# thecasterian/fluca

Measured on AMD Instinct MI355X. Metric: pressure-Poisson Jacobi-PCG iterations/s, 512^3 cells per GPU, higher is better.
Workload: dtype f64

## Files before the change

### fluca_amd/build.py

```python
import hashlib
import json
import os
import subprocess
import sys

HERE = os.path.dirname(os.path.abspath(__file__))
CSRC = os.path.join(HERE, "csrc")
LIBDIR = os.path.join(HERE, "lib")
LIB = os.path.join(LIBDIR, "libflucahip.so")
SOURCES = ["fl_coeff.cpp", "fl_kernels.hip", "fl_api.hip", "fl_knobs.cpp", "fl_place.hip", "fl_halo.hip", "fl_comm.hip", "fl_ksp.hip", "fl_cheb2.hip", "fl_layout.hip", "fl_ibm.hip", "fl_ibm_owner.hip", "fl_ibm_body.hip", "fl_momentum.hip", "fl_mg.hip", "fl_schur_var.hip", "fl_scalar.hip", "fl_buoyancy.hip", "fl_scalar_implicit.hip"]
HEADERS = ["fl_internal.h", "fl_knobs.h", "fl_handle.h", "fl_msg.h", "fl_ibm_device.h", "fl_ibm_handle.h", "fl_ibm_plan.h", "fl_device.h", "fl_stencil.h", "fl_mom_tile.h", "fl_mom_tile3.h", "fl_limiter.h", "fl_scalar_handle.h", os.path.join("..", "..", "include", "fluca_hip.h"),
           os.path.join("..", "..", "include", "fluca_hip_implicit.h"), os.path.join("..", "..", "include", "fluca_hip_implicit_ranks.h"), os.path.join("..", "..", "include", "fluca_hip_ibm_scalar.h")]
HIPCC = os.environ.get("HIPCC", "/opt/rocm/bin/hipcc")
FLAGS = ["--offload-arch=gfx950", "-O3", "-std=c++17", "-fPIC", "-Wall", "-Wno-unused-function", "-Wno-unused-result"]
MANIFEST = os.path.join(LIBDIR, "manifest.json")


def _sha(path):
    h = hashlib.sha256()
    with open(path, "rb") as fh:
        h.update(fh.read())
    return h.hexdigest()


def _load_manifest(path=None):
    try:
        with open(path or MANIFEST) as fh:
            return json.load(fh)
    except (OSError, ValueError):
        return {}


def _fingerprint(deps, cmd_words):
    h = hashlib.sha256()
    for d in deps:
        h.update(os.path.basename(d).encode() + b"\0" + (_sha(d) if os.path.exists(d) else "absent").encode() + b"\0")
    root = os.path.normpath(os.path.join(HERE, ".."))
    real = os.path.realpath(root)
    h.update(" ".join(w.replace(real, "$ROOT").replace(root, "$ROOT") for w in cmd_words).encode())
    return h.hexdigest()


def _stale(target, deps, cmd_words=(), manifest=None):
    if not os.path.exists(target):
        return True
    m = _load_manifest() if manifest is None else manifest
    return m.get(os.path.relpath(target, LIBDIR)) != _fingerprint(deps, cmd_words)


def _record(target, deps, cmd_words=()):
    m = _load_manifest()
    m[os.path.relpath(target, LIBDIR)] = _fingerprint(deps, cmd_words)
    with open(MANIFEST, "w") as fh:
        json.dump(m, fh, indent=0, sort_keys=True)


def _mapped(path):
    try:
        real = os.path.realpath(path)
        with open("/proc/self/maps") as fh:
            return any(line.rstrip().endswith(real) or line.rstrip().endswith(path) for line in fh)
    except OSError:
        return False


def _link(cmd, target):
    if _mapped(target):
        raise RuntimeError(f"{target} is out of date with respect to the sources AND loaded in this process: rebuild it first "
                           "(`python -m fluca_amd.build`, or tests/conftest.py, which builds before anything is loaded); it is not replaced under a live process")
    tmp = target + ".tmp%d" % os.getpid()
    i = cmd.index("-o")
    assert cmd[i + 1] == target
    subprocess.check_call(cmd[:i + 1] + [tmp] + cmd[i + 2:])
    os.replace(tmp, target)


def source_id():
    files = [os.path.join(CSRC, s) for s in SOURCES] + [os.path.normpath(os.path.join(CSRC, h)) for h in HEADERS]
    return _fingerprint(files, FLAGS)[:12]


def build(force=False, verbose=False):
    os.makedirs(LIBDIR, exist_ok=True)
    srcs = [os.path.join(CSRC, s) for s in SOURCES if os.path.exists(os.path.join(CSRC, s))]
    hdrs = [os.path.normpath(os.path.join(CSRC, h)) for h in HEADERS]
    objs = []
    for s in srcs:
        o = os.path.join(LIBDIR, os.path.basename(s) + ".o")
        cmd = [HIPCC] + FLAGS + (["-x", "hip"] if s.endswith(".hip") else []) + ["-c", s, "-o", o]
        if force or _stale(o, [s] + hdrs, cmd):
            if verbose:
                print(" ".join(cmd), flush=True)
            subprocess.check_call(cmd)
            _record(o, [s] + hdrs, cmd)
        objs.append(o)
    sid = source_id()
    idsrc, idobj = os.path.join(LIBDIR, "fl_build_id.cpp"), os.path.join(LIBDIR, "fl_build_id.cpp.o")
    text = f'extern "C" const char *fl_build_id(void) {{ return "{sid}"; }}\n'
    if not os.path.exists(idsrc) or open(idsrc).read() != text:
        with open(idsrc, "w") as fh:
            fh.write(text)
    cmd = [os.environ.get("CXX", "g++"), "-O1", "-fPIC", "-c", idsrc, "-o", idobj]
    if force or _stale(idobj, [idsrc], cmd):
        subprocess.check_call(cmd)
        _record(idobj, [idsrc], cmd)
    objs.append(idobj)
    cmd = [HIPCC, "--offload-arch=gfx950", "-shared", "-fPIC", "-o", LIB] + objs + ["-Wl,-rpath,/opt/rocm/lib", "-ldl"]
    if force or _stale(LIB, objs, cmd):
        if verbose:
            print(" ".join(cmd), flush=True)
        _link(cmd, LIB)
        _record(LIB, objs, cmd)
    build_host(force, verbose)
    return LIB


HOST_LIB = os.path.join(LIBDIR, "libfluca_host.so")


def build_host(force=False, verbose=False):
    src = os.path.join(HERE, "host", "fluca_host.c")
    hdrs = [os.path.normpath(os.path.join(HERE, "..", "include", h)) for h in ("fluca_host.h", "fluca_host_impl.h", "fluca_hip.h", "fluca_hip_implicit.h", "fluca_hip_implicit_ranks.h", "fluca_hip_ibm_scalar.h")]
    cmd = [os.environ.get("CC", "gcc"), "-std=gnu99", "-O2", "-fPIC", "-shared", "-Wall", "-o", HOST_LIB, src,
           "-L" + LIBDIR, "-lflucahip", "-Wl,-rpath,$ORIGIN", "-lm", "-ldl", "-pthread"]
    if force or _stale(HOST_LIB, [src, LIB] + hdrs, cmd):
        if verbose:
            print(" ".join(cmd), flush=True)
        _link(cmd, HOST_LIB)
        _record(HOST_LIB, [src, LIB] + hdrs, cmd)
    build_cgns(force, verbose)
    build_example(force, verbose)
    build_example(force, verbose, name="cavity_flow_3d")
    build_example(force, verbose, name="flow_configs")
    build_example(force, verbose, name="heated_cavity_3d")
    build_example(force, verbose, name="heated_sphere_3d")
    return HOST_LIB


CGNS_LIB = os.path.join(LIBDIR, "libfluca_cgns.so")
HDF5_ROOT = os.environ.get("HDF5_ROOT", "/opt/conda")


def have_hdf5():
    return os.path.exists(os.path.join(HDF5_ROOT, "include", "hdf5.h")) and os.path.exists(os.path.join(HDF5_ROOT, "lib", "libhdf5.so"))


def build_cgns(force=False, verbose=False):
    src = os.path.join(HERE, "host", "fluca_cgns.c")
    if not have_hdf5():
        if verbose:
            print(f"no HDF5 under {HDF5_ROOT}: libfluca_cgns.so not built", flush=True)
        return None
    hdrs = [os.path.normpath(os.path.join(HERE, "..", "include", h)) for h in ("fluca_cgns.h", "fluca_host.h", "fluca_host_impl.h", "fluca_hip.h", "fluca_hip_implicit.h", "fluca_hip_implicit_ranks.h", "fluca_hip_ibm_scalar.h")]
    if True:
        cmd = [os.environ.get("CC", "gcc"), "-std=gnu99", "-O2", "-fPIC", "-shared", "-Wall", "-o", CGNS_LIB, src,
               "-I" + os.path.join(HDF5_ROOT, "include"), "-L" + LIBDIR, "-lfluca_host", "-lflucahip",
               "-L" + os.path.join(HDF5_ROOT, "lib"), "-lhdf5", "-Wl,--enable-new-dtags",
               "-Wl,-rpath,$ORIGIN", "-Wl,-rpath," + os.path.join(HDF5_ROOT, "lib"), "-lm"]
        if force or _stale(CGNS_LIB, [src, HOST_LIB] + hdrs, cmd):
            if verbose:
                print(" ".join(cmd), flush=True)
            _link(cmd, CGNS_LIB)
            _record(CGNS_LIB, [src, HOST_LIB] + hdrs, cmd)
    return CGNS_LIB


EXAMPLE = os.path.join(LIBDIR, "cavity_pressure_step")


def build_example(force=False, verbose=False, name="cavity_pressure_step"):
    root = os.path.normpath(os.path.join(HERE, ".."))
    src = os.path.join(root, "examples", name + ".c")
    EXAMPLE = os.path.join(LIBDIR, name)
    cgns = os.path.exists(CGNS_LIB) and name == "cavity_flow_3d"
    cmd = [os.environ.get("CC", "gcc"), "-std=gnu99", "-O2", "-Wall", "-o", EXAMPLE, src, "-I" + os.path.join(root, "include"),
           "-L" + LIBDIR] + (["-DFLUCA_HAVE_CGNS", "-lfluca_cgns"] if cgns else []) + ["-lfluca_host", "-lflucahip", "-lm",
           "-Wl,-rpath,$ORIGIN", "-Wl,-rpath,/opt/rocm/lib"]
    deps = [src, HOST_LIB, LIB] + ([CGNS_LIB] if cgns else []) + [os.path.join(root, "include", h) for h in ("fluca_host.h", "fluca_hip.h", "fluca_hip_implicit.h", "fluca_hip_implicit_ranks.h", "fluca_hip_ibm_scalar.h", "fluca_cgns.h")]
    if os.path.exists(src) and (force or _stale(EXAMPLE, deps, cmd)):
        if verbose:
            print(" ".join(cmd), flush=True)
        _link(cmd, EXAMPLE)
        _record(EXAMPLE, deps, cmd)
    return EXAMPLE


if __name__ == "__main__":
    print(build(force="--force" in sys.argv, verbose=True))
```

### fluca_amd/capi.py

```python
import ctypes as C
import os

import torch

_HERE = os.path.dirname(os.path.abspath(__file__))
LIB_PATH = os.path.join(os.environ.get("FLUCA_LIB_DIR") or os.path.join(_HERE, "lib"), "libflucahip.so")

if not os.path.exists(LIB_PATH):
    raise ImportError(
        f"{LIB_PATH} is missing: build it with `python -m fluca_amd.build` (hipcc --offload-arch=gfx950). "
        "There is no CPU fallback for the product path.")

lib = C.CDLL(LIB_PATH)

BC_NONE, BC_VELOCITY, BC_PRESSURE_OUTLET, BC_PERIODIC, BC_SYMMETRY = range(5)
KSP_CG, KSP_BCGS, KSP_CHEBYSHEV, KSP_GMRES = range(4)
PC_NONE, PC_JACOBI = range(2)
NORM_PRECONDITIONED, NORM_UNPRECONDITIONED, NORM_NATURAL, NORM_NONE = range(4)
DELTA_PESKIN4, DELTA_ROMA3 = range(2)
SCALAR_DIRICHLET, SCALAR_NEUMANN, SCALAR_PERIODIC = range(3)
LIMITERS = ("superbee", "minmod", "mc", "vanleer", "vanalbada", "barthjesperson", "venkatakrishnan", "koren", "upwind", "sou", "quick")
UNIQUE_ID_BYTES = 128

ERRORS = {0: "FL_SUCCESS", -55: "FL_ERR_MEM", -56: "FL_ERR_SUP", -60: "FL_ERR_ARG_SIZ", -62: "FL_ERR_ARG_WRONG",
          -63: "FL_ERR_ARG_OUTOFRANGE", -73: "FL_ERR_ARG_WRONGSTATE", -76: "FL_ERR_LIB", -85: "FL_ERR_ARG_NULL",
          -91: "FL_ERR_NOT_CONVERGED", -97: "FL_ERR_GPU"}


class FlucaError(RuntimeError):
    def __init__(self, rc, what):
        super().__init__(f"{what} -> {ERRORS.get(rc, rc)} ({rc})")
        self.rc = rc


def check(rc, what="libflucahip"):
    if rc != 0:
        raise FlucaError(rc, what)


class fl_comm_info(C.Structure):
    _fields_ = [("transport", C.c_int), ("rank", C.c_int), ("nranks", C.c_int), ("loopback", C.c_int), ("neighbours", C.c_int), ("messages", C.c_int), ("halo_bytes", C.c_int64)]


class fl_grid(C.Structure):
    _fields_ = [("n", C.c_int64 * 3), ("xf", C.c_void_p * 3), ("xc", C.c_void_p * 3)]


class fl_decomp(C.Structure):
    _fields_ = [("ranks", C.c_int * 3), ("coord", C.c_int * 3), ("lo", C.c_int64 * 3), ("len", C.c_int64 * 3)]


class fl_ksp_opts(C.Structure):
    _fields_ = [("type", C.c_int), ("pc", C.c_int), ("norm_type", C.c_int), ("remove_nullspace", C.c_int),
                ("maxit", C.c_int), ("rtol", C.c_double), ("atol", C.c_double), ("dtol", C.c_double),
                ("emin", C.c_double), ("emax", C.c_double), ("variant", C.c_int), ("check_every", C.c_int),
                ("profile", C.c_int), ("history", C.POINTER(C.c_double)), ("nhistory", C.c_int),
                ("mg_levels", C.c_int), ("mg_smooth_its", C.c_int), ("gmres_restart", C.c_int), ("cg_single_reduction", C.c_int),
                ("initial_guess_nonzero", C.c_int)]


class fl_ksp_stats(C.Structure):
    _fields_ = [("iters", C.c_int), ("reason", C.c_int), ("rnorm0", C.c_double), ("rnorm", C.c_double),
                ("seconds", C.c_double), ("kernel_ms", C.c_double), ("kernel_launches", C.c_int),
                ("kernel2_ms", C.c_double), ("kernel2_launches", C.c_int)]


class fl_dmstag_local(C.Structure):
    _fields_ = [("gstart", C.c_int64 * 3), ("gsize", C.c_int64 * 3), ("start", C.c_int64 * 3), ("entries", C.c_int)]


class fl_scalar_cheb_info(C.Structure):
    _fields_ = [("steps", C.c_int), ("capped", C.c_int), ("emin", C.c_double), ("emax", C.c_double), ("bound", C.c_double)]


class fl_halo_msg(C.Structure):
    _fields_ = [("peer", C.c_int), ("send_boundary", C.c_int), ("recv_boundary", C.c_int), ("sendtag", C.c_int), ("recvtag", C.c_int)]


EXCHANGE_FN = C.CFUNCTYPE(C.c_int, C.c_void_p, C.c_int, C.POINTER(C.c_int), C.POINTER(C.c_int), C.POINTER(C.c_int),
                          C.POINTER(C.c_void_p), C.POINTER(C.c_void_p), C.POINTER(C.c_int64))
ALLREDUCE_FN = C.CFUNCTYPE(C.c_int, C.c_void_p, C.POINTER(C.c_double), C.c_int)

_P = C.c_void_p
PROTOTYPES = {
    "fl_poisson_create": (C.c_int, [C.POINTER(fl_grid), C.POINTER(C.c_int), C.c_double, C.POINTER(fl_decomp), C.c_int, C.POINTER(_P)]),
    "fl_poisson_destroy": (C.c_int, [_P]),
    "fl_poisson_set_stream": (C.c_int, [_P, _P]),
    "fl_poisson_synchronize": (C.c_int, [_P]),
    "fl_poisson_barrier": (C.c_int, [_P]),
    "fl_poisson_sizes": (C.c_int, [_P, C.POINTER(C.c_int64)]),
    "fl_poisson_allreduce_sum": (C.c_int, [_P, C.POINTER(C.c_double), C.c_int]),
    "fl_ksp_opts_default": (None, [C.POINTER(fl_ksp_opts)]),
    "fl_version": (C.c_char_p, []),
    "fl_abi_version": (C.c_int, []),
    "fl_poisson_comm_info": (C.c_int, [_P, C.POINTER(fl_comm_info)]),
    "fl_current_device": (C.c_int, [C.POINTER(C.c_int)]),
    "fl_malloc": (C.c_int, [C.c_int, C.c_size_t, C.POINTER(_P)]),
    "fl_free": (C.c_int, [C.c_int, _P]),
    "fl_memcpy_h2d": (C.c_int, [C.c_int, _P, _P, C.c_size_t]),
    "fl_memcpy_d2h": (C.c_int, [C.c_int, _P, _P, C.c_size_t]),
    "fl_malloc_host": (C.c_int, [C.c_size_t, C.POINTER(C.c_void_p)]),
    "fl_free_host": (C.c_int, [_P]),
    "fl_poisson_upload": (C.c_int, [_P, _P, _P, C.c_size_t]),
    "fl_poisson_upload_fence": (C.c_int, [_P]),
    "fl_tuning_set": (C.c_int, [C.c_char_p, C.c_int]),
    "fl_tuning_get": (C.c_int, [C.c_char_p, C.POINTER(C.c_int)]),
    "fl_poisson_tune_placement": (C.c_int, [_P, C.c_int, C.POINTER(C.c_double)]),
    "fl_poisson_vector_bytes": (C.c_int, [_P, C.POINTER(C.c_int64)]),
    "fl_poisson_apply": (C.c_int, [_P, _P, _P]),
    "fl_poisson_diagonal": (C.c_int, [_P, _P]),
    "fl_poisson_solve": (C.c_int, [_P, _P, _P, C.POINTER(fl_ksp_opts), C.POINTER(fl_ksp_stats)]),
    "fl_poisson_rhs": (C.c_int, [_P, _P, _P, _P, _P, _P]),
    "fl_poisson_project": (C.c_int, [_P, _P, _P, _P, _P, _P, _P, _P]),
    "fl_poisson_gst_bc": (C.c_int, [_P, C.c_int, _P, _P]),
    "fl_pressure_update": (C.c_int, [_P, C.c_int, _P, _P, _P, _P]),
    "fl_layout_from_dmstag_local": (C.c_int, [_P, C.POINTER(fl_dmstag_local), C.c_int, C.c_int, _P, _P]),
    "fl_layout_to_dmstag_local": (C.c_int, [_P, C.POINTER(fl_dmstag_local), C.c_int, C.c_int, _P, _P]),
    "fl_layout_from_dmstag_global": (C.c_int, [_P, C.POINTER(C.c_int), C.c_int, C.c_int, _P, _P]),
    "fl_layout_to_dmstag_global": (C.c_int, [_P, C.POINTER(C.c_int), C.c_int, C.c_int, _P, _P]),
    "fl_dmstag_global_entries": (C.c_int, [_P, C.POINTER(C.c_int), C.POINTER(C.c_int64)]),
    "fl_comm_unique_id": (C.c_int, [_P]),
    "fl_poisson_comm_init_rccl": (C.c_int, [_P, _P, C.c_int, C.c_int]),
    "fl_poisson_comm_init_host": (C.c_int, [_P, EXCHANGE_FN, ALLREDUCE_FN, _P, C.c_int, C.c_int]),
    "fl_poisson_comm_oneshot_handle": (C.c_int, [_P, _P, C.POINTER(_P)]),
    "fl_poisson_comm_oneshot_attach": (C.c_int, [_P, _P, C.POINTER(_P)]),
    "fl_poisson_comm_oneshot_error": (C.c_int, [_P, C.POINTER(C.c_int)]),
    "fl_halo_plan": (C.c_int, [C.POINTER(fl_decomp), C.POINTER(C.c_int), C.POINTER(fl_halo_msg)]),
    "fl_decomp_default": (C.c_int, [C.POINTER(C.c_int64), C.POINTER(C.c_int), C.c_int, C.POINTER(fl_decomp)]),
    "fl_decomp_neighbor": (C.c_int, [C.POINTER(fl_decomp), C.POINTER(C.c_int), C.c_int]),
    "fl_decomp_neighbor_offset": (C.c_int, [C.POINTER(fl_decomp), C.POINTER(C.c_int), C.POINTER(C.c_int)]),
    "fl_momentum_create": (C.c_int, [_P, C.POINTER(_P)]),
    "fl_momentum_destroy": (C.c_int, [_P]),
    "fl_momentum_set_state": (C.c_int, [_P, C.c_double, C.c_double, C.c_double, _P, _P]),
    "fl_momentum_set_state_v0": (C.c_int, [_P, C.c_double, C.c_double, C.c_double, _P, _P, _P]),
    "fl_momentum_set_coefficients": (C.c_int, [_P, C.c_double, C.c_double, C.c_double]),
    "fl_momentum_apply": (C.c_int, [_P, _P, _P]),
    "fl_momentum_diagonal": (C.c_int, [_P, _P]),
    "fl_momentum_rowsum": (C.c_int, [_P, _P]),
    "fl_momentum_gershgorin": (C.c_int, [_P, C.POINTER(C.c_double)]),
    "fl_momentum_chebyshev_interval": (C.c_int, [_P, C.POINTER(C.c_double), C.POINTER(C.c_double)]),
    "fl_abf_set_ainv_types": (C.c_int, [_P, C.c_int, C.c_int]),
    "fl_abf_schur_apply": (C.c_int, [_P, _P, _P]),
    "fl_momentum_solve": (C.c_int, [_P, _P, _P, C.POINTER(fl_ksp_opts), C.POINTER(fl_ksp_stats)]),
    "fl_momentum_face_interp": (C.c_int, [_P, _P, _P, _P]),
    "fl_poisson_gershgorin": (C.c_int, [_P, C.c_int, C.POINTER(C.c_double)]),
    "fl_vec_lincomb": (C.c_int, [_P, C.c_int64, C.c_double, _P, C.c_double, _P, _P]),
    "fl_vec_dot": (C.c_int, [_P, C.c_int64, _P, _P, C.POINTER(C.c_double)]),
    "fl_vec_mdot": (C.c_int, [_P, C.c_int64, _P, C.POINTER(C.c_void_p), C.c_int, C.POINTER(C.c_double)]),
    "fl_vec_maxpy": (C.c_int, [_P, C.c_int64, _P, C.POINTER(C.c_double), C.POINTER(C.c_void_p), C.c_int]),
    "fl_boundary_set_faces": (C.c_int, [_P, C.c_int, C.c_double, _P, _P]),
    "fl_boundary_add_faces": (C.c_int, [_P, C.c_int, C.c_double, _P, _P]),
    "fl_momentum_face_interp_scaled": (C.c_int, [_P, C.c_double, _P, _P, _P]),
    "fl_boundary_add_cells": (C.c_int, [_P, C.c_int, C.c_double, _P, _P]),
    "fl_momentum_rhs": (C.c_int, [_P, C.c_double, C.c_double, C.c_double, _P, _P, _P, _P]),
    "fl_momentum_add_buoyancy": (C.c_int, [_P, C.c_int, C.POINTER(C.c_void_p), C.POINTER(C.c_double), C.POINTER(C.c_double), C.c_double, _P]),
    "fl_momentum_interp_faces": (C.c_int, [_P, _P, _P, _P]),
    "fl_momentum_interp_faces_ends": (C.c_int, [_P, _P, _P, _P]),
    "fl_abf_jacobian_mult": (C.c_int, [_P, _P, _P, _P, _P, _P, _P]),
    "fl_abf_apply": (C.c_int, [_P, C.POINTER(fl_ksp_opts), C.POINTER(fl_ksp_opts), _P, _P, _P, _P, _P, _P, C.POINTER(fl_ksp_stats)]),
    "fl_ibm_create": (C.c_int, [_P, C.c_int, C.c_int64, _P, _P, _P, C.POINTER(_P)]),
    "fl_ibm_update": (C.c_int, [_P, _P, _P, _P]),
    "fl_ibm_interp": (C.c_int, [_P, C.c_int, _P, _P]),
    "fl_ibm_spread": (C.c_int, [_P, C.c_int, _P, _P, _P]),
    "fl_ibm_destroy": (C.c_int, [_P]),
    "fl_ibm_owned_select": (C.c_int, [_P, C.c_int, C.c_int64, _P, _P, _P, _P, C.POINTER(C.c_int64)]),
    "fl_ibm_create_owned": (C.c_int, [_P, C.c_int, C.c_int64, _P, _P, _P, _P, C.POINTER(_P)]),
    "fl_ibm_owned_counts": (C.c_int, [_P, C.POINTER(C.c_int64)]),
    "fl_ibm_migrate": (C.c_int, [_P, _P, _P, _P, C.c_int, _P, C.POINTER(C.c_int64), C.POINTER(C.c_int64)]),
    "fl_ibm_owned_fetch": (C.c_int, [_P, C.c_int64, _P, _P, _P, _P, C.c_int, _P]),
    "fl_ibm_rigid_pose": (C.c_int, [_P, C.c_int64, _P, _P, _P] + [C.POINTER(C.c_double)] * 5 + [_P, _P, _P, _P]),
    "fl_ibm_force": (C.c_int, [_P, _P, _P, _P, C.c_int, C.POINTER(C.c_double), C.POINTER(C.c_double), C.POINTER(C.c_double)]),
    "fl_limiter_from_name": (C.c_int, [C.c_char_p, C.POINTER(C.c_int)]),
    "fl_limiter_eval": (C.c_int, [C.c_int, C.c_double, C.POINTER(C.c_double)]),
    "fl_scalar_create": (C.c_int, [_P, C.POINTER(C.c_int), C.POINTER(_P)]),
    "fl_scalar_create_ranks": (C.c_int, [_P, C.POINTER(C.c_int), C.POINTER(_P)]),
    "fl_scalar_destroy": (C.c_int, [_P]),
    "fl_scalar_set_boundary_value": (C.c_int, [_P, C.c_int, C.c_double]),
    "fl_scalar_set_limiter": (C.c_int, [_P, C.c_int]),
    "fl_scalar_set_diffusivity": (C.c_int, [_P, C.c_double]),
    "fl_scalar_set_velocity": (C.c_int, [_P, _P, _P, _P]),
    "fl_scalar_rhs": (C.c_int, [_P, _P, _P, _P]),
    "fl_scalar_step": (C.c_int, [_P, C.c_double, C.c_int, _P, _P]),
    "fl_scalar_cfl": (C.c_int, [_P, C.c_double, C.POINTER(C.c_double)]),
    "fl_scalar_stats": (C.c_int, [_P, _P, C.POINTER(C.c_double)]),
    "fl_scalar_boundary_flux": (C.c_int, [_P, _P, C.POINTER(C.c_double)]),
}
PROTOTYPES_IMPLICIT = {
    "fl_scalar_cheb_steps": (C.c_int, [C.c_double, C.c_double, C.c_double, C.c_int, C.POINTER(C.c_int), C.POINTER(C.c_double)]),
    "fl_scalar_diffusion_interval": (C.c_int, [_P, C.c_double, C.POINTER(C.c_double), C.POINTER(C.c_double)]),
    "fl_scalar_diffusion_apply": (C.c_int, [_P, C.c_double, _P, _P]),
    "fl_scalar_diffusion_solve": (C.c_int, [_P, C.c_double, C.c_double, C.c_int, _P, _P, C.POINTER(fl_scalar_cheb_info)]),
    "fl_scalar_step_imex": (C.c_int, [_P, C.c_double, C.c_int, C.c_double, C.c_double, C.c_int, _P, _P, C.POINTER(fl_scalar_cheb_info)]),
}
PROTOTYPES_IBM_SCALAR = {
    "fl_ibm_scalar_force": (C.c_int, [_P, C.c_int, _P, _P, C.c_int, C.POINTER(C.c_double), _P, _P, _P]),
    "fl_ibm_scalar_rate": (C.c_int, [_P, _P, _P, _P, C.c_int, C.POINTER(C.c_double)]),
}
PROTOTYPES_IMPLICIT_RANKS = {
    "fl_scalar_diffusion_apply_ranks": PROTOTYPES_IMPLICIT["fl_scalar_diffusion_apply"],
    "fl_scalar_diffusion_solve_ranks": PROTOTYPES_IMPLICIT["fl_scalar_diffusion_solve"],
    "fl_scalar_step_imex_ranks": PROTOTYPES_IMPLICIT["fl_scalar_step_imex"],
}
for _name, (_res, _args) in list(PROTOTYPES.items()) + list(PROTOTYPES_IMPLICIT.items()) + list(PROTOTYPES_IBM_SCALAR.items()) + list(PROTOTYPES_IMPLICIT_RANKS.items()):
    _f = getattr(lib, _name)
    _f.restype = _res
    _f.argtypes = _args
```

### fluca_amd/csrc/fl_momentum.hip

```cpp
#include <new>

#include "fl_handle.h"
#include "fl_device.h"

namespace fl {

struct MomP {
  const double *tab[3];
  const double *stab[3];
  const double *bw[3];
  int           len[3];
  double        cI, cC, cL;
};

struct FaceT {
  const double *w0[3][3], *w1[3][3];
  const int    *c0[3][3];
};

__device__ __forceinline__ double recip(double d)
{
  double r = __builtin_amdgcn_rcp(d);
  r        = fma(r, fma(-d, r, 1.), r);
  r        = fma(r, fma(-d, r, 1.), r);
  return r;
}

}
#include "fl_stencil.h"
#include "fl_mom_tile.h"
#include "fl_mom_tile3.h"
namespace fl {

template <int OP>
__global__ void __launch_bounds__(512) k_mom_pw3(GridP g, int64_t cs, const double *__restrict__ a0, const double *__restrict__ a1, const double *__restrict__ a2, const double *__restrict__ a3, double *__restrict__ w0,
                                                 double *__restrict__ w1, const KspScal *__restrict__ s, double *__restrict__ partial, int pstride, int pairs, int tiles_x, int nchunk, int zc)
{
  __shared__ double red[3 * 8];
  if (OP != 3 && s->reason != 0) return;
  const double alpha = s->alpha, omega = s->omega, beta = s->beta, ob = s->omega_old * s->beta;
  const int    nb = gridDim.x, tiles = nb / nchunk, b = xcd_remap(blockIdx.x, nb), chunk = b / tiles, tile = b % tiles;
  const int    lane = threadIdx.x & 63, w = threadIdx.x >> 6;
  const int    i = (tile % tiles_x) * 128 + 2 * lane, j = (tile / tiles_x) * 8 + w;
  const int    k0 = chunk * zc, k1 = min(k0 + zc, g.nz);
  const int64_t ncell = (int64_t)g.nx * g.ny * g.nz;
  double       acc[3] = {0., 0., 0.};
  if (i < g.nx && j < g.ny) {
    const bool two = i + 1 < g.nx;
    auto       ldp = [&](const double *p, int64_t q) { return two ? ld2<1>(p + q) : make_double2(p[q], 0.); };
    auto       ldk = [&](const double *p, int64_t q) { return two ? ld2<0>(p + q) : make_double2(p[q], 0.); };
    auto       stp = [&](double *p, int64_t q, double2 v) {
      if (two) st2<0>(p + q, v);
      else p[q] = v.x;
    };
    for (int k = k0; k < k1; ++k) {
      const int64_t idx = g.off0 + (int64_t)k * g.sxy + (int64_t)j * g.sx + i, ub = ((int64_t)k * g.ny + j) * g.nx + i;
#pragma unroll
      for (int c = 0; c < 3; ++c) {
        const int64_t q = c * cs + idx;
        if (OP == 0) {
          const double2 r = ldk(a0, q), v = ldp(a1, q), p = ldp(w0, q);
          stp(w0, q, make_double2(r.x - ob * v.x + beta * p.x, r.y - ob * v.y + beta * p.y));
        } else if (OP == 4) {
          stp(w0, q, ldk(a0, q));
        } else if (OP == 1) {
          const double2 r = ldp(a0, q), v = ldp(a1, q);
          stp(w0, q, make_double2(r.x - alpha * v.x, r.y - alpha * v.y));
        } else if (OP == 6) {
          const double2 xk = ldp(a0, q), ax = ldp(a1, q), bb = ldp(a2, q), xo = ldp(w0, q);
          const double2 rr = make_double2(bb.x - ax.x, bb.y - ax.y);
          double2       zz = rr;
          if (a3) {
            const double2 d = ldk(a3, q);
            zz.x = rr.x * recip(d.x);
            zz.y = two ? rr.y * recip(d.y) : 0.;
          }
          stp(w0, q, make_double2(fma(s->cheb_c, zz.x, fma(s->cheb_rho, xk.x - xo.x, xk.x)), fma(s->cheb_c, zz.y, fma(s->cheb_rho, xk.y - xo.y, xk.y))));
          acc[0] += zz.x + (two ? zz.y : 0.);
          acc[1] += zz.x * zz.x + (two ? zz.y * zz.y : 0.);
          acc[2] += rr.x * rr.x + (two ? rr.y * rr.y : 0.);
        } else if (OP == 2 || OP == 5) {
          const double2 P = ldp(a0, q), S = ldp(a1, q), T = ldp(a2, q), RP = ldk(a3, q), X = OP == 5 ? make_double2(0., 0.) : ldp(w0, q);
          const double2 rn = make_double2(S.x - omega * T.x, S.y - omega * T.y);
          double2       xn = X;
          xn.x += alpha * P.x + omega * S.x;
          xn.y += alpha * P.y + omega * S.y;
          if (two) st2<1>(w0 + q, xn);
          else w0[q] = xn.x;
          stp(w1, q, rn);
          acc[0] += rn.x * rn.x + (two ? rn.y * rn.y : 0.);
          acc[1] += rn.x * RP.x + (two ? rn.y * RP.y : 0.);
          acc[2] += rn.x + (two ? rn.y : 0.);
        } else {
          const int64_t u = c * ncell + ub;
          double2       bb;
          if (two && pairs) bb = ld2<1>(a0 + u);
          else bb = make_double2(a0[u], two ? a0[u + 1] : 0.);
          double2 r = bb;
          if (a1) {
            const double2 d = ldp(a1, q);
            r.x = bb.x / d.x;
            if (two) r.y = bb.y / d.y;
          }
          stp(w0, q, r);
          stp(w1, q, r);
          acc[0] += r.x + (two ? r.y : 0.);
          acc[1] += r.x * r.x + (two ? r.y * r.y : 0.);
        }
      }
    }
  }
  if (OP == 2 || OP == 3 || OP == 5 || OP == 6) {
#pragma unroll
    for (int a = 0; a < 3; ++a) {
      const double v = wave_sum(acc[a]);
      if (lane == 0) red[a * 8 + w] = v;
    }
    __syncthreads();
    if (threadIdx.x < 3) {
      double v = 0.;
#pragma unroll
      for (int q = 0; q < 8; ++q) v += red[threadIdx.x * 8 + q];
      partial[(int64_t)threadIdx.x * pstride + blockIdx.x] = v;
    }
  }
}

__global__ void __launch_bounds__(256) k_fill(int64_t n, double v, double *__restrict__ out)
{
  for (int64_t q = (int64_t)blockIdx.x * blockDim.x + threadIdx.x; q < n; q += (int64_t)gridDim.x * blockDim.x) out[q] = v;
}
__global__ void __launch_bounds__(256) k_recip(int64_t n, const double *__restrict__ in, double *__restrict__ out)
{
  for (int64_t q = (int64_t)blockIdx.x * blockDim.x + threadIdx.x; q < n; q += (int64_t)gridDim.x * blockDim.x) out[q] = 1. / in[q];
}
__global__ void __launch_bounds__(256) k_scale_by(int64_t n, const double *__restrict__ w, double shift, const double *x, double *y, int add)
{
  for (int64_t q = (int64_t)blockIdx.x * blockDim.x + threadIdx.x; q < n; q += (int64_t)gridDim.x * blockDim.x) {
    const double t = (w[q] - shift) * x[q];
    y[q]           = add ? y[q] + t : t;
  }
}
__global__ void __launch_bounds__(256) k_max_sum_owned(GridP g, int64_t cs, const double *__restrict__ a, const double *__restrict__ b, double *__restrict__ partial)
{
  __shared__ double red[2][4];
  const int64_t plane = (int64_t)g.nz * g.ny, rows = 3 * plane;
  double        mx = 0., sm = 0.;
  for (int64_t r0 = (int64_t)blockIdx.x * 4; r0 < rows; r0 += (int64_t)gridDim.x * 4) {
    int64_t base[4];
#pragma unroll
    for (int u = 0; u < 4; ++u) {
      const int64_t r = min(r0 + u, rows - 1);
      const int     c = (int)(r / plane), kj = (int)(r % plane), k = kj / g.ny, j = kj % g.ny;
      base[u] = (int64_t)c * cs + g.off0 + (int64_t)k * g.sxy + (int64_t)j * g.sx;
    }
    for (int i = 2 * threadIdx.x; i < g.nx; i += 512) {
      const bool two = i + 1 < g.nx;
      double2    va[4], vb[4];
#pragma unroll
      for (int u = 0; u < 4; ++u) {
        va[u] = a ? (two ? *reinterpret_cast<const double2 *>(a + base[u] + i) : make_double2(a[base[u] + i], 0.)) : make_double2(0., 0.);
        vb[u] = b ? (two ? *reinterpret_cast<const double2 *>(b + base[u] + i) : make_double2(b[base[u] + i], 0.)) : make_double2(0., 0.);
      }
#pragma unroll
      for (int u = 0; u < 4; ++u) {
        mx = fmax(mx, fmax(va[u].x, va[u].y));
        if (r0 + u < rows) sm += vb[u].x + vb[u].y;
      }
    }
  }
  for (int off = 32; off > 0; off >>= 1) {
    mx = fmax(mx, __shfl_down(mx, off, 64));
    sm += __shfl_down(sm, off, 64);
  }
  if ((threadIdx.x & 63) == 0) {
    red[0][threadIdx.x >> 6] = mx;
    red[1][threadIdx.x >> 6] = sm;
  }
  __syncthreads();
  if (threadIdx.x == 0) {
    partial[2 * blockIdx.x]     = fmax(fmax(red[0][0], red[0][1]), fmax(red[0][2], red[0][3]));
    partial[2 * blockIdx.x + 1] = (red[1][0] + red[1][1]) + (red[1][2] + red[1][3]);
  }
}

struct Vec8 {
  const double *p[8];
};
struct Coef8 {
  double a[8];
};
__global__ void __launch_bounds__(256) k_mdot8(int64_t n, const double *__restrict__ x, Vec8 Y, int k, double *__restrict__ partial, int stride)
{
  __shared__ double red[8 * 4];
  double            acc[8] = {0., 0., 0., 0., 0., 0., 0., 0.};
  for (int64_t q = (int64_t)blockIdx.x * blockDim.x + threadIdx.x; q < n; q += (int64_t)gridDim.x * blockDim.x) {
    const double xv = x[q];
#pragma unroll
    for (int i = 0; i < 8; ++i)
      if (i < k) acc[i] += xv * Y.p[i][q];
  }
  block_sum<8>(acc, red);
  if (threadIdx.x == 0)
#pragma unroll
    for (int i = 0; i < 8; ++i) partial[(int64_t)i * stride + blockIdx.x] = acc[i];
}
__global__ void __launch_bounds__(256) k_maxpy8(int64_t n, double *__restrict__ x, Coef8 A, Vec8 Y, int k)
{
  for (int64_t q = (int64_t)blockIdx.x * blockDim.x + threadIdx.x; q < n; q += (int64_t)gridDim.x * blockDim.x) {
    double t = x[q];
#pragma unroll
    for (int i = 0; i < 8; ++i)
      if (i < k) t += A.a[i] * Y.p[i][q];
    x[q] = t;
  }
}
__global__ void __launch_bounds__(256) k_lincomb(int64_t n, double a, const double *x, double b, const double *z, double *y)
{
  const bool ux = a != 0., uz = z && b != 0.;
  for (int64_t q = (int64_t)blockIdx.x * blockDim.x + threadIdx.x; q < n; q += (int64_t)gridDim.x * blockDim.x) y[q] = (ux ? a * x[q] : 0.) + (uz ? b * z[q] : 0.);
}

__global__ void __launch_bounds__(256) k_dot(int64_t n, const double *__restrict__ x, const double *__restrict__ y, double *__restrict__ partial)
{
  __shared__ double red[4];
  double            v[1] = {0.};
  for (int64_t q = (int64_t)blockIdx.x * blockDim.x + threadIdx.x; q < n; q += (int64_t)gridDim.x * blockDim.x) v[0] += x[q] * y[q];
  block_sum<1>(v, red);
  if (threadIdx.x == 0) partial[blockIdx.x] = v[0];
}

__global__ void __launch_bounds__(256) k_pad_copy_ext(GridP g, const double *__restrict__ src, double *__restrict__ dst, int ex, int ey, int ez)
{
  const int64_t n = (int64_t)ex * ey * ez;
  for (int64_t q = (int64_t)blockIdx.x * blockDim.x + threadIdx.x; q < n; q += (int64_t)gridDim.x * blockDim.x) {
    const int     i = (int)(q % ex);
    const int64_t r = q / ex;
    const int     j = (int)(r % ey), k = (int)(r / ey);
    dst[g.off0 + (int64_t)k * g.sxy + (int64_t)j * g.sx + i] = src[q];
  }
}

__global__ void __launch_bounds__(256) k_pad_copy_ends(GridP g, const double *__restrict__ src, double *__restrict__ dst, int ex, int ey, int ez, int d)
{
  const int     nd = d == 0 ? g.nx : (d == 1 ? g.ny : g.nz), ed = d == 0 ? ex : (d == 1 ? ey : ez);
  const int     na = d == 0 ? ey : ex, nb = d == 2 ? ey : ez;
  const int     nend = ed > nd ? 2 : 1;
  const int64_t n = (int64_t)na * nb * nend;
  for (int64_t q = (int64_t)blockIdx.x * blockDim.x + threadIdx.x; q < n; q += (int64_t)gridDim.x * blockDim.x) {
    const int a = (int)(q % na), b = (int)((q / na) % nb), f = (q / ((int64_t)na * nb)) ? nd : 0;
    const int i = d == 0 ? f : a, j = d == 1 ? f : (d == 0 ? a : b), k = d == 2 ? f : b;
    dst[g.off0 + (int64_t)k * g.sxy + (int64_t)j * g.sx + i] = src[((int64_t)k * ey + j) * ex + i];
  }
}

__global__ void __launch_bounds__(256) k_face_interp(GridP g, FaceT t, int kind, int d, double alpha, const double *__restrict__ vpad, const double *rhs, double *V)
{
  const int     ex = d == 0 ? g.fx : g.nx, ey = d == 1 ? g.fy : g.ny, ez = d == 2 ? g.fz : g.nz;
  const int64_t str = d == 0 ? 1 : (d == 1 ? (int64_t)g.sx : g.sxy);
  const int     lane = threadIdx.x & 63, w = __builtin_amdgcn_readfirstlane(threadIdx.x >> 6), nw = blockDim.x >> 6;
  const int     nseg = (ex + 63) / 64;
  const int64_t nitem = (int64_t)nseg * ey * ez;
  for (int64_t it = (int64_t)blockIdx.x * nw + w; it < nitem; it += (int64_t)gridDim.x * nw) {
    const int seg = (int)(it % nseg), row = (int)(it / nseg);
    const int j = row % ey, k = row / ey, i = seg * 64 + lane;
    if (i >= ex) continue;
    const int     f = d == 0 ? i : (d == 1 ? j : k);
    const int     c0 = t.c0[kind][d][f];
    const int64_t q = ((int64_t)k * ey + j) * ex + i;
    const int64_t base = g.off0 + (int64_t)k * g.sxy + (int64_t)j * g.sx + i + (int64_t)(c0 - f) * str;
    const double  w0 = alpha * t.w0[kind][d][f], w1 = alpha * t.w1[kind][d][f];
    double        s = rhs ? rhs[q] : 0.;
    if (w0 != 0.) s += w0 * vpad[base];
    if (w1 != 0.) s += w1 * vpad[base + str];
    V[q] = s;
  }
}

__global__ void __launch_bounds__(256) k_face_interp_ends(GridP g, FaceT t, int kind, int d, const double *__restrict__ vpad, const double *rhs, double *V)
{
  const int     ex = d == 0 ? g.fx : g.nx, ey = d == 1 ? g.fy : g.ny, ez = d == 2 ? g.fz : g.nz;
  const int     nd = d == 0 ? g.nx : (d == 1 ? g.ny : g.nz), ed = d == 0 ? ex : (d == 1 ? ey : ez);
  const int     na = d == 0 ? ey : ex, nb = d == 2 ? ey : ez;
  const int64_t n = (int64_t)na * nb * (ed > nd ? 2 : 1);
  const int64_t str = d == 0 ? 1 : (d == 1 ? (int64_t)g.sx : g.sxy);
  for (int64_t q = (int64_t)blockIdx.x * blockDim.x + threadIdx.x; q < n; q += (int64_t)gridDim.x * blockDim.x) {
    const int     a = (int)(q % na), b = (int)((q / na) % nb), f = (q / ((int64_t)na * nb)) ? nd : 0;
    const int     i = d == 0 ? f : a, j = d == 1 ? f : (d == 0 ? a : b), k = d == 2 ? f : b;
    const int64_t u = ((int64_t)k * ey + j) * ex + i;
    const int     c0 = t.c0[kind][d][f];
    const int64_t base = g.off0 + (int64_t)k * g.sxy + (int64_t)j * g.sx + i + (int64_t)(c0 - f) * str;
    const double  w0 = t.w0[kind][d][f], w1 = t.w1[kind][d][f];
    double        s = rhs ? rhs[u] : 0.;
    if (w0 != 0.) s += w0 * vpad[base];
    if (w1 != 0.) s += w1 * vpad[base + str];
    V[u] = s;
  }
}

}

using namespace fl;


struct fl_momentum {
  fl_poisson *p = nullptr;
  MomP        mp;
  FaceT       ft;
  void       *tabs[3] = {nullptr, nullptr, nullptr};
  double     *bws[3] = {nullptr, nullptr, nullptr};
  double     *stabs[2][3] = {{nullptr, nullptr, nullptr}, {nullptr, nullptr, nullptr}};
  std::vector<void *> ttabs;
  double     *srhs = nullptr;
  double     *gr = nullptr, *gd = nullptr;
  double     *tmpv = nullptr;
  double     *F = nullptr;
  double     *dg = nullptr;
  double     *v0p = nullptr;
  bool        fly = false;
  double     *vec[8] = {nullptr, nullptr, nullptr, nullptr, nullptr, nullptr, nullptr, nullptr};
  int                   schur_ainv = FL_ABF_AINV_ID, upper_ainv = FL_ABF_AINV_ID;
  double               *ainv[2] = {nullptr, nullptr}, *zV[3] = {nullptr, nullptr, nullptr}, *gv = nullptr;
  std::vector<double *> gm;
  std::vector<double *> kb;
  bool        have_state = false;
  double      dmean = 1.;
  double      gersh = -1.;
  int         t2x = 1, t2chunk = 1, t2zc = 1, t2blocks = 1;
};

namespace {

int mom_vec(fl_momentum *m, int slot)
{
  if (m->vec[slot]) return 0;
  return fl_dev_alloc(m->p, (void **)&m->vec[slot], sizeof(double) * 3 * m->p->padlen, true);
}

int mom_ghosts(fl_momentum *m, double *v3)
{
  fl_poisson *h = m->p;
  if (!fl_any_ghost_exchange(h)) return 0;
  if (!h->multi) {
    for (int d = 0; d < 3; ++d)
      if (h->wrap_local[d]) launch_wrap(h->stream, h->g, v3, d, 3, (int64_t)h->padlen);
    return 0;
  }
  for (int c = 0; c < 3; ++c) FL_CHK(fl_fill_ghosts(h, v3 + (size_t)c * h->padlen));
  return 0;
}

constexpr int MOM_XCD_ORDER = 1;

bool mom3_grid(const GridP &g) { return g.ny > 8; }

template <int DOT, bool JAC, int OUT>
void mom_apply_t(fl_momentum *m, const double *x, double *y, const double *o, const KspScal *s, const MomP *coeffs = nullptr)
{
  fl_poisson *h = m->p;
  int         flags = MOM_XCD_ORDER;
  if (OUT == 1 && (h->g.nx & 1) == 0 && (reinterpret_cast<uintptr_t>(y) & 15) == 0) flags |= 2;
  if (m->fly && mom3_grid(h->g))
    hipLaunchKernelGGL((k_mom3<8, DOT, JAC, OUT, 1>), dim3(m->t2blocks), dim3(512), 0, h->stream, h->g, coeffs ? *coeffs : m->mp, x, y, m->F, (const double *)m->v0p, (int64_t)h->padlen, o, s, h->partial,
                       h->partial_stride, m->t2x, m->t2chunk, m->t2zc, flags);
  else
    hipLaunchKernelGGL((k_mom2<8, DOT, JAC, OUT, 1>), dim3(m->t2blocks), dim3(512), 0, h->stream, h->g, coeffs ? *coeffs : m->mp, x, y, m->F, (int64_t)h->padlen, o, s, h->partial, h->partial_stride, m->t2x, m->t2chunk,
                       m->t2zc, flags);
}
int mom_scale_tables(fl_momentum *m, int slot, MomP &p)
{
  fl_poisson *h = m->p;
  for (int d = 0; d < 3; ++d) {
    const int len = m->mp.len[d], n = len * MOM_STAB;
    hipLaunchKernelGGL(k_mom_scale_tab, dim3((n + 255) / 256), dim3(256), 0, h->stream, (const double *)m->tabs[d], len, p.cC, p.cL, m->stabs[slot][d]);
    p.stab[d] = m->stabs[slot][d];
  }
  FL_HIP(hipGetLastError());
  return 0;
}

template <int OP>
void mom_pw(fl_momentum *m, const double *a0, const double *a1, const double *a2, const double *a3, double *w0, double *w1)
{
  fl_poisson *h = m->p;
  const int   pairs = (h->g.nx & 1) == 0 && (reinterpret_cast<uintptr_t>(a0) & 15) == 0;
  hipLaunchKernelGGL((k_mom_pw3<OP>), dim3(m->t2blocks), dim3(512), 0, h->stream, h->g, (int64_t)h->padlen, a0, a1, a2, a3, w0, w1, h->scal, h->partial, h->partial_stride, pairs, m->t2x, m->t2chunk, m->t2zc);
}

}

MomPlan fl::mom_plan(const GridP &g)
{
  MomPlan p;
  p.t2x           = (g.nx + 127) / 128;
  const int tiles = p.t2x * ((g.ny + 7) / 8);
  int       nc    = z_chunk_count(tiles, g.nz, 1024);
  if (tiles * nc > MAX_PARTIAL_BLOCKS) nc = std::max(1, MAX_PARTIAL_BLOCKS / tiles);
  const ZChunks z = z_chunks(g.nz, nc);
  p.t2zc     = z.zc;
  p.t2chunk  = z.nchunk;
  p.t2blocks = tiles * p.t2chunk;
  return p;
}

namespace {

int mom_init(fl_momentum *m, fl_poisson *h)
{
  m->p = h;
  const GridP &g = h->g;
  if (g.nx < 2 || g.ny < 2 || g.nz < 2) return FL_ERR_SUP;
  const int64_t lo[3] = {h->dec.lo[0], h->dec.lo[1], h->dec.lo[2]};
  const int     len[3] = {g.nx, g.ny, g.nz};
  for (int d = 0; d < 3; ++d) {
    std::vector<double> tab, loc;
    FL_CHK(build_axis_momentum(h->ax[d], tab));
    const int64_t n = h->ax[d].n;
    loc.resize((size_t)MOM_NTAB * len[d]);
    for (int a = 0; a < MOM_NTAB; ++a)
      for (int i = 0; i < len[d]; ++i) loc[(size_t)a * len[d] + i] = tab[(size_t)a * n + (size_t)(lo[d] + i)];
    FL_HIP(hipMalloc(&m->tabs[d], sizeof(double) * loc.size()));
    FL_HIP(hipMemcpy(m->tabs[d], loc.data(), sizeof(double) * loc.size(), hipMemcpyHostToDevice));
    m->mp.tab[d] = (const double *)m->tabs[d];
    m->mp.len[d] = len[d];
    for (int slot = 0; slot < 2; ++slot) FL_HIP(hipMalloc((void **)&m->stabs[slot][d], sizeof(double) * (size_t)MOM_STAB * len[d]));
    m->mp.stab[d] = m->stabs[0][d];
    const int nfl = d == 0 ? g.fx : (d == 1 ? g.fy : g.fz);
    std::vector<double> bw((size_t)4 * nfl, 0.);
    for (int kind = 0; kind < 3; ++kind) {
      std::vector<double> w0, w1;
      std::vector<int>    c0;
      FL_CHK(build_axis_faceinterp(h->ax[d], kind, w0, w1, c0));
      std::vector<double> l0(nfl), l1(nfl);
      std::vector<int>    lc(nfl);
      for (int f = 0; f < nfl; ++f) {
        l0[f] = w0[(size_t)(lo[d] + f)];
        l1[f] = w1[(size_t)(lo[d] + f)];
        lc[f] = (int)(c0[(size_t)(lo[d] + f)] - lo[d]);
        if (kind >= 1) {
          bw[(size_t)4 * f + 2 * (kind - 1)]     = l0[f];
          bw[(size_t)4 * f + 2 * (kind - 1) + 1] = l1[f];
        }
      }
      const void  *src[3] = {l0.data(), l1.data(), lc.data()};
      const size_t by[3] = {sizeof(double) * nfl, sizeof(double) * nfl, sizeof(int) * nfl};
      void        *dv[3];
      for (int a = 0; a < 3; ++a) {
        FL_HIP(hipMalloc(&dv[a], std::max<size_t>(by[a], 8)));
        m->ttabs.push_back(dv[a]);
        FL_HIP(hipMemcpy(dv[a], src[a], by[a], hipMemcpyHostToDevice));
      }
      m->ft.w0[kind][d] = (const double *)dv[0];
      m->ft.w1[kind][d] = (const double *)dv[1];
      m->ft.c0[kind][d] = (const int *)dv[2];
    }
    FL_HIP(hipMalloc((void **)&m->bws[d], sizeof(double) * std::max<size_t>(bw.size(), 4)));
    FL_HIP(hipMemcpy(m->bws[d], bw.data(), sizeof(double) * bw.size(), hipMemcpyHostToDevice));
    m->mp.bw[d] = m->bws[d];
  }
  m->mp.cI = 1.;
  m->mp.cC = 0.;
  m->mp.cL = 0.;
  const MomPlan pl = mom_plan(g);
  if (pl.t2blocks > MAX_PARTIAL_BLOCKS) return FL_ERR_SUP;
  m->t2x      = pl.t2x;
  m->t2chunk  = pl.t2chunk;
  m->t2zc     = pl.t2zc;
  m->t2blocks = pl.t2blocks;
  FL_CHK(fl_ensure_partials(h, m->t2blocks));
  FL_CHK(fl_dev_alloc(h, (void **)&m->F, sizeof(double) * 12 * h->padlen, true));
  FL_CHK(fl_dev_alloc(h, (void **)&m->dg, sizeof(double) * 3 * h->padlen, true));
  return fl_momentum_set_coefficients(m, 1., 0., 0.);
}

}

extern "C" int fl_momentum_create(fl_poisson *grid_from, fl_momentum **out)
{
  if (!grid_from || !out) return FL_ERR_ARG_NULL;
  *out = nullptr;
  FL_HIP(hipSetDevice(grid_from->device));
  fl_momentum *m = new (std::nothrow) fl_momentum;
  if (!m) return FL_ERR_MEM;
  const int rc = mom_init(m, grid_from);
  if (rc != 0) {
    fl_momentum_destroy(m);
    return rc;
  }
  *out = m;
  return FL_SUCCESS;
}

extern "C" int fl_momentum_destroy(fl_momentum *m)
{
  if (!m) return FL_SUCCESS;
  if (m->p) {
    (void)hipSetDevice(m->p->device);
    (void)hipStreamSynchronize(m->p->stream);
  }
  for (void *t : m->tabs)
    if (t) (void)hipFree(t);
  for (void *t : m->ttabs)
    if (t) (void)hipFree(t);
  for (double *t : m->bws)
    if (t) (void)hipFree(t);
  for (auto &sl : m->stabs)
    for (double *t : sl)
      if (t) (void)hipFree(t);
  if (m->srhs) (void)hipFree(m->srhs);
  if (m->gr) (void)hipFree(m->gr);
  if (m->gd) (void)hipFree(m->gd);
  if (m->tmpv) (void)hipFree(m->tmpv);
  if (m->F) (void)hipFree(m->F);
  if (m->dg) (void)hipFree(m->dg);
  if (m->v0p) (void)hipFree(m->v0p);
  for (double *v : m->vec)
    if (v) (void)hipFree(v);
  for (double *v : {m->ainv[0], m->ainv[1], m->zV[0], m->zV[1], m->zV[2], m->gv})
    if (v) (void)hipFree(v);
  for (double *v : m->gm)
    if (v) (void)hipFree(v);
  for (double *v : m->kb)
    if (v) (void)hipFree(v);
  delete m;
  return FL_SUCCESS;
}

extern "C" int fl_momentum_set_coefficients(fl_momentum *m, double cI, double cC, double cL)
{
  if (!m) return FL_ERR_ARG_NULL;
  m->mp.cI = cI;
  m->mp.cC = cC;
  m->mp.cL = cL;
  m->gersh = -1.;
  fl_poisson *h = m->p;
  FL_HIP(hipSetDevice(h->device));
  FL_CHK(mom_scale_tables(m, 0, m->mp));
  mom_apply_t<0, false, 2>(m, m->F, m->dg, nullptr, nullptr);
  FL_HIP(hipGetLastError());
  return FL_SUCCESS;
}

namespace {
int mom_set_state(fl_momentum *m, double dt, double rho, double mu, const double *const V0_dev[3], const double *const v0interp_dev[9], const double *v0_dev)
{
  if (!m || !V0_dev || !v0interp_dev) return FL_ERR_ARG_NULL;
  if (!(rho > 0.)) return FL_ERR_ARG_OUTOFRANGE;
  fl_poisson  *h = m->p;
  const GridP &g = h->g;
  FL_HIP(hipSetDevice(h->device));
  for (int d = 0; d < 3; ++d) {
    if (!V0_dev[d]) return FL_ERR_ARG_NULL;
    for (int c = 0; c < 3; ++c)
      if (!v0interp_dev[c * 3 + d]) return FL_ERR_ARG_NULL;
  }
  const int ext[3][3] = {{g.fx, g.ny, g.nz}, {g.nx, g.fy, g.nz}, {g.nx, g.ny, g.fz}};
  const bool ends_only = v0_dev && mom3_grid(g);
  for (int f = 0; f < 12; ++f) {
    const int     d = f < 3 ? f : (f - 3) % 3;
    const double *src = f < 3 ? V0_dev[f] : v0interp_dev[f - 3];
    double       *dst = m->F + (size_t)f * h->padlen;
    const int64_t n = (int64_t)ext[d][0] * ext[d][1] * ext[d][2];
    const int     nb = (int)std::min<int64_t>((n + 255) / 256, 8192);
    if (f >= 3 && ends_only) {
      const int64_t ne = 2 * n / std::max(ext[d][d], 1);
      hipLaunchKernelGGL(k_pad_copy_ends, dim3((unsigned)std::max<int64_t>(1, std::min<int64_t>((ne + 255) / 256, 8192))), dim3(256), 0, h->stream, g, src, dst, ext[d][0], ext[d][1], ext[d][2], d);
    } else hipLaunchKernelGGL(k_pad_copy_ext, dim3(std::max(nb, 1)), dim3(256), 0, h->stream, g, src, dst, ext[d][0], ext[d][1], ext[d][2]);
    if (fl_any_ghost_exchange(h)) FL_CHK(fl_fill_ghosts(h, dst));
  }
  m->fly = false;
  if (v0_dev) {
    if (!m->v0p) FL_CHK(fl_dev_alloc(h, (void **)&m->v0p, sizeof(double) * 3 * h->padlen, true));
    for (int c = 0; c < 3; ++c) launch_pad_copy(h->stream, g, v0_dev + (size_t)c * h->ncell, m->v0p + (size_t)c * h->padlen);
    FL_CHK(mom_ghosts(m, m->v0p));
    m->fly = true;
  }
  m->have_state = true;
  return fl_momentum_set_coefficients(m, 1., dt, -0.5 * mu * dt / rho);
}
}

extern "C" int fl_momentum_set_state(fl_momentum *m, double dt, double rho, double mu, const double *const V0_dev[3], const double *const v0interp_dev[9])
{
  return mom_set_state(m, dt, rho, mu, V0_dev, v0interp_dev, nullptr);
}

extern "C" int fl_momentum_set_state_v0(fl_momentum *m, double dt, double rho, double mu, const double *const V0_dev[3], const double *const v0interp_dev[9], const double *v0_dev)
{
  if (!v0_dev) return FL_ERR_ARG_NULL;
  return mom_set_state(m, dt, rho, mu, V0_dev, v0interp_dev, v0_dev);
}

extern "C" int fl_momentum_apply(fl_momentum *m, const double *v_dev, double *y_dev)
{
  if (!m || !v_dev || !y_dev) return FL_ERR_ARG_NULL;
  if (!m->have_state && m->mp.cC != 0.) return FL_ERR_ARG_WRONGSTATE;
  fl_poisson *h = m->p;
  FL_HIP(hipSetDevice(h->device));
  FL_CHK(mom_vec(m, 7));
  for (int c = 0; c < 3; ++c) launch_pad_copy(h->stream, h->g, v_dev + (size_t)c * h->ncell, m->vec[7] + (size_t)c * h->padlen);
  FL_CHK(mom_ghosts(m, m->vec[7]));
  mom_apply_t<0, false, 1>(m, m->vec[7], y_dev, nullptr, nullptr);
  FL_HIP(hipGetLastError());
  return FL_SUCCESS;
}

extern "C" int fl_momentum_diagonal(fl_momentum *m, double *d_dev)
{
  if (!m || !d_dev) return FL_ERR_ARG_NULL;
  if (!m->have_state && m->mp.cC != 0.) return FL_ERR_ARG_WRONGSTATE;
  fl_poisson *h = m->p;
  FL_HIP(hipSetDevice(h->device));
  mom_apply_t<0, false, 2>(m, m->F, m->dg, nullptr, nullptr);
  for (int c = 0; c < 3; ++c) launch_unpad_copy(h->stream, h->g, m->dg + (size_t)c * h->padlen, d_dev + (size_t)c * h->ncell, nullptr);
  FL_HIP(hipGetLastError());
  return FL_SUCCESS;
}

static int max_sum_owned(fl_momentum *m, const double *a3, const double *b3, double *mx_out, double *sum_out)
{
  fl_poisson   *h = m->p;
  const int64_t rows = (int64_t)3 * h->g.nz * h->g.ny;
  const int     nb = (int)std::max<int64_t>(1, std::min<int64_t>((rows + 3) / 4, 2048));
  FL_CHK(fl_ensure_partials(h, 2 * nb));
  hipLaunchKernelGGL(k_max_sum_owned, dim3(nb), dim3(256), 0, h->stream, h->g, (int64_t)h->padlen, a3, b3, h->partial);
  FL_HIP(hipGetLastError());
  std::vector<double> part((size_t)(2 * nb));
  FL_HIP(hipMemcpyAsync(part.data(), h->partial, sizeof(double) * (size_t)(2 * nb), hipMemcpyDeviceToHost, h->stream));
  FL_HIP(hipStreamSynchronize(h->stream));
  double mx = 0., sm = 0.;
  for (int q = 0; q < nb; ++q) {
    mx = std::max(mx, part[(size_t)(2 * q)]);
    sm += part[(size_t)(2 * q + 1)];
  }
  FL_CHK(fl_allreduce_max(h, &mx));
  FL_CHK(fl_allreduce_sum(h, &sm));
  if (mx_out) *mx_out = mx;
  if (sum_out) *sum_out = sm;
  return 0;
}

extern "C" int fl_momentum_gershgorin(fl_momentum *m, double *radius)
{
  if (!m || !radius) return FL_ERR_ARG_NULL;
  if (!m->have_state && m->mp.cC != 0.) return FL_ERR_ARG_WRONGSTATE;
  fl_poisson *h = m->p;
  FL_HIP(hipSetDevice(h->device));
  if (m->gersh < 0.) {
    FL_CHK(mom_vec(m, 7));
    mom_apply_t<0, false, 3>(m, m->F, m->vec[7], nullptr, nullptr);
    double dsum = 0.;
    FL_CHK(max_sum_owned(m, m->vec[7], m->dg, &m->gersh, &dsum));
    m->dmean = dsum / (3. * (double)h->ax[0].n * (double)h->ax[1].n * (double)h->ax[2].n);
  }
  *radius = m->gersh;
  return FL_SUCCESS;
}

extern "C" int fl_momentum_chebyshev_interval(fl_momentum *m, double *emin, double *emax)
{
  if (!m || !emin || !emax) return FL_ERR_ARG_NULL;
  double g = 0.;
  FL_CHK(fl_momentum_gershgorin(m, &g));
  *emax = 1. + g;
  *emin = std::max(1. - g, 0.9 / m->dmean);
  return FL_SUCCESS;
}

static int momentum_cheb(fl_momentum *m, const double *b_dev, double *x_dev, const fl_ksp_opts *opts, fl_ksp_stats *stats, bool from_guess = false)
{
  if (opts->pc != FL_PC_JACOBI && opts->pc != FL_PC_NONE) return FL_ERR_SUP;
  if (opts->norm_type == FL_NORM_NATURAL) return FL_ERR_SUP;
  if (opts->maxit < 0) return FL_ERR_ARG_OUTOFRANGE;
  fl_poisson *h = m->p;
  FL_HIP(hipSetDevice(h->device));
  std::memset(stats, 0, sizeof(*stats));
  const bool jac = opts->pc == FL_PC_JACOBI;
  double     emin = opts->emin, emax = opts->emax;
  bool       default_interval = false;
  if (emin == 0. && emax == 0.) {
    if (!jac) return FL_ERR_SUP;
    FL_CHK(fl_momentum_chebyshev_interval(m, &emin, &emax));
    default_interval = true;
  }
  if (!(emax > emin) || !(emin > 0.)) return FL_ERR_ARG_OUTOFRANGE;
  const bool fused = m->fly && mom3_grid(h->g);
  for (int a : {0, 2, 4}) FL_CHK(mom_vec(m, a));
  if (!fused) FL_CHK(mom_vec(m, 3));
  double *B = m->vec[0], *X0 = m->vec[4], *X1 = m->vec[2], *AX = m->vec[3];
  const int nhist = opts->maxit + 2;
  FL_CHK(fl_ensure_hist(h, nhist));
  FL_CHK(fl_ensure_partials(h, m->t2blocks));
  fl_ksp_opts o = *opts;
  o.remove_nullspace = 0;
  const bool watched = default_interval && o.norm_type == FL_NORM_NONE;
  if (watched) {
    o.norm_type = FL_NORM_PRECONDITIONED;
    o.rtol      = 0.;
    o.atol      = 0.;
  }
  FL_CHK(fl_cheb_begin(h, &o, emin, emax));
  const size_t bytes = sizeof(double) * 3 * h->padlen;
  for (double *v : {X0, X1}) FL_HIP(hipMemsetAsync(v, 0, bytes, h->stream));
  for (int c = 0; c < 3; ++c) launch_pad_copy(h->stream, h->g, b_dev + (size_t)c * h->ncell, B + (size_t)c * h->padlen);
  if (from_guess)
    for (int c = 0; c < 3; ++c) launch_pad_copy(h->stream, h->g, x_dev + (size_t)c * h->ncell, X0 + (size_t)c * h->padlen);
  const int every = o.check_every > 0 ? o.check_every : 8;
  const int total = o.norm_type == FL_NORM_NONE ? o.maxit : o.maxit + 1;
  int       j = 0, hostcur = 0;
  bool      done = total <= 0;
  const int flags = MOM_XCD_ORDER;
  while (!done) {
    const int stop = std::min(total, j + every);
    for (; j < stop; ++j) {
      double *xin = hostcur ? X1 : X0, *xout = hostcur ? X0 : X1;
      if (j > 0 || from_guess) FL_CHK(mom_ghosts(m, xin));
      if (fused) {
        if (jac) hipLaunchKernelGGL((k_mom3<8, 0, true, 4, 1>), dim3(m->t2blocks), dim3(512), 0, h->stream, h->g, m->mp, (const double *)xin, xout, m->F, (const double *)m->v0p, (int64_t)h->padlen, (const double *)B,
                                    (const KspScal *)h->scal, h->partial, h->partial_stride, m->t2x, m->t2chunk, m->t2zc, flags);
        else hipLaunchKernelGGL((k_mom3<8, 0, false, 4, 1>), dim3(m->t2blocks), dim3(512), 0, h->stream, h->g, m->mp, (const double *)xin, xout, m->F, (const double *)m->v0p, (int64_t)h->padlen, (const double *)B,
                                (const KspScal *)h->scal, h->partial, h->partial_stride, m->t2x, m->t2chunk, m->t2zc, flags);
        FL_CHK(fl_cheb_fin_step(h, m->t2blocks, nhist));
      } else {
        mom_apply_t<0, false, 0>(m, xin, AX, nullptr, h->scal);
        mom_pw<6>(m, xin, AX, B, jac ? m->dg : nullptr, xout, nullptr);
        FL_CHK(fl_cheb_fin_step(h, m->t2blocks, nhist));
      }
      hostcur ^= 1;
    }
    FL_HIP(hipGetLastError());
    FL_CHK(fl_poll_scal(h));
    if (h->scal_host->reason != 0 || j >= total) done = true;
  }
  FL_CHK(fl_poll_scal(h));
  const double *ans = h->scal_host->cur ? X1 : X0;
  for (int c = 0; c < 3; ++c) launch_unpad_copy(h->stream, h->g, ans + (size_t)c * h->padlen, x_dev + (size_t)c * h->ncell, nullptr);
  FL_CHK(fl_ksp_finish(h, &o, stats));
  if (watched && stats->reason == FL_DIVERGED_ITS) stats->reason = FL_CONVERGED_ITS;
  return 0;
}

static int momentum_gmres(fl_momentum *m, const double *b_dev, double *x_dev, const fl_ksp_opts *opts, fl_ksp_stats *stats);

namespace {
void lincomb(fl_poisson *h, int64_t n, double a, const double *x, double b, const double *z, double *y);
}
static int momentum_solve_from_guess(fl_momentum *m, const double *b_dev, double *x_dev, const fl_ksp_opts *opts, fl_ksp_stats *stats)
{
  fl_poisson *h = m->p;
  FL_HIP(hipSetDevice(h->device));
  const int64_t n3 = 3 * h->ncell;
  const bool scaled = opts->pc == FL_PC_JACOBI && opts->norm_type != FL_NORM_UNPRECONDITIONED;
  for (int a = 0; a < 2; ++a) FL_CHK(mom_vec(m, a));
  FL_CHK(fl_ensure_partials(h, m->t2blocks));
  mom_pw<3>(m, b_dev, scaled ? m->dg : nullptr, nullptr, nullptr, m->vec[0], m->vec[1]);
  launch_reduce(h->stream, h->partial, m->t2blocks, h->partial_stride, 3, h->sums);
  if (h->multi) FL_CHK(h->comm.allreduce(h->stream, h->sums, NSLOT));
  double sums[NSLOT];
  FL_HIP(hipMemcpyAsync(sums, h->sums, sizeof(sums), hipMemcpyDeviceToHost, h->stream));
  FL_HIP(hipStreamSynchronize(h->stream));
  const double bnorm = std::sqrt(sums[1] > 0. ? sums[1] : 0.);
  if (opts->type == FL_KSP_CHEBYSHEV) {
    fl_ksp_opts o = *opts;
    o.initial_guess_nonzero = 0;
    o.rtol = 0.;
    o.atol = std::max(opts->rtol * bnorm, opts->atol);
    FL_CHK(momentum_cheb(m, b_dev, x_dev, &o, stats, true));
    if (stats->reason == FL_CONVERGED_ATOL && !(stats->rnorm < opts->atol)) stats->reason = FL_CONVERGED_RTOL;
    stats->rnorm0 = bnorm;
    return FL_SUCCESS;
  }
  if (!m->gr) FL_CHK(fl_dev_alloc(h, (void **)&m->gr, sizeof(double) * (size_t)n3, false));
  if (!m->gd) FL_CHK(fl_dev_alloc(h, (void **)&m->gd, sizeof(double) * (size_t)n3, false));
  FL_CHK(fl_momentum_apply(m, x_dev, m->gr));
  lincomb(h, n3, 1., b_dev, -1., m->gr, m->gr);
  fl_ksp_opts o = *opts;
  o.initial_guess_nonzero = 0;
  o.rtol = 0.;
  o.atol = std::max(opts->rtol * bnorm, opts->atol);
  FL_CHK(fl_momentum_solve(m, m->gr, m->gd, &o, stats));
  lincomb(h, n3, 1., x_dev, 1., m->gd, x_dev);
  FL_HIP(hipGetLastError());
  if (stats->reason == FL_CONVERGED_ATOL && !(stats->rnorm < opts->atol)) stats->reason = FL_CONVERGED_RTOL;
  stats->rnorm0 = bnorm;
  return FL_SUCCESS;
}

extern "C" int fl_momentum_solve(fl_momentum *m, const double *b_dev, double *x_dev, const fl_ksp_opts *opts, fl_ksp_stats *stats)
{
  if (!m || !b_dev || !x_dev || !opts || !stats) return FL_ERR_ARG_NULL;
  if (!m->have_state && m->mp.cC != 0.) return FL_ERR_ARG_WRONGSTATE;
  if (opts->initial_guess_nonzero) return momentum_solve_from_guess(m, b_dev, x_dev, opts, stats);
  if (opts->type == FL_KSP_GMRES) return momentum_gmres(m, b_dev, x_dev, opts, stats);
  if (opts->type == FL_KSP_CHEBYSHEV) return momentum_cheb(m, b_dev, x_dev, opts, stats);
  if (opts->type != FL_KSP_BCGS) return FL_ERR_SUP;
  if (opts->pc != FL_PC_JACOBI && opts->pc != FL_PC_NONE) return FL_ERR_SUP;
  if (opts->norm_type != FL_NORM_PRECONDITIONED) return FL_ERR_SUP;
  if (opts->maxit < 0) return FL_ERR_ARG_OUTOFRANGE;
  fl_poisson *h = m->p;
  FL_HIP(hipSetDevice(h->device));
  std::memset(stats, 0, sizeof(*stats));
  const bool jac = opts->pc == FL_PC_JACOBI;
  for (int a = 0; a < 7; ++a) FL_CHK(mom_vec(m, a));
  double *R = m->vec[0], *RP = m->vec[1], *P = m->vec[2], *V = m->vec[3], *X = m->vec[4], *S = m->vec[5], *T = m->vec[6];
  const int nhist = opts->maxit + 1;
  FL_CHK(fl_ensure_hist(h, nhist));
  FL_CHK(fl_ensure_partials(h, m->t2blocks));
  fl_ksp_opts o = *opts;
  o.remove_nullspace = 0;
  FL_CHK(fl_ksp_begin(h, &o));
  const size_t bytes = sizeof(double) * 3 * h->padlen;
  mom_pw<3>(m, b_dev, jac ? m->dg : nullptr, nullptr, nullptr, R, RP);
  FL_CHK(fl_bcgs_fin_step(h, 0, m->t2blocks, 3, nhist));
  const int every = o.check_every > 0 ? o.check_every : 4;
  int       it = 0;
  bool      done = false;
  while (!done) {
    const int stop = std::min(o.maxit, it + every);
    for (; it < stop; ++it) {
      if (it == 0) mom_pw<4>(m, R, nullptr, nullptr, nullptr, P, nullptr);
      else mom_pw<0>(m, R, V, nullptr, nullptr, P, nullptr);
      FL_CHK(mom_ghosts(m, P));
      if (jac) mom_apply_t<1, true, 0>(m, P, V, RP, h->scal);
      else mom_apply_t<1, false, 0>(m, P, V, RP, h->scal);
      FL_CHK(fl_bcgs_fin_step(h, 1, m->t2blocks, 4, nhist));
      mom_pw<1>(m, R, V, nullptr, nullptr, S, nullptr);
      FL_CHK(mom_ghosts(m, S));
      if (jac) mom_apply_t<2, true, 0>(m, S, T, nullptr, h->scal);
      else mom_apply_t<2, false, 0>(m, S, T, nullptr, h->scal);
      FL_CHK(fl_bcgs_fin_step(h, 3, m->t2blocks, 4, nhist));
      if (it == 0) mom_pw<5>(m, P, S, T, RP, X, R);
      else mom_pw<2>(m, P, S, T, RP, X, R);
      FL_CHK(fl_bcgs_fin_step(h, 4, m->t2blocks, 3, nhist));
    }
    FL_CHK(fl_poll_scal(h));
    if (h->scal_host->reason != 0 || it >= o.maxit) done = true;
  }
  if (h->scal_host->it == 0) FL_HIP(hipMemsetAsync(X, 0, bytes, h->stream));
  for (int c = 0; c < 3; ++c) launch_unpad_copy(h->stream, h->g, X + (size_t)c * h->padlen, x_dev + (size_t)c * h->ncell, nullptr);
  return fl_ksp_finish(h, &o, stats);
}

namespace {
int face_interp(fl_momentum *m, double alpha, const double *v_dev, const double *const rhs_dev[3], double *const V_dev[3])
{
  fl_poisson *h = m->p;
  FL_CHK(mom_vec(m, 7));
  for (int c = 0; c < 3; ++c) launch_pad_copy(h->stream, h->g, v_dev + (size_t)c * h->ncell, m->vec[7] + (size_t)c * h->padlen);
  FL_CHK(mom_ghosts(m, m->vec[7]));
  for (int d = 0; d < 3; ++d) {
    if (!V_dev[d]) return FL_ERR_ARG_NULL;
    const int64_t n = h->nface[d];
    const int     nb = (int)std::min<int64_t>((n + 255) / 256, 8192);
    hipLaunchKernelGGL(k_face_interp, dim3(std::max(nb, 1)), dim3(256), 0, h->stream, h->g, m->ft, 0, d, alpha, m->vec[7] + (size_t)d * h->padlen, rhs_dev ? rhs_dev[d] : nullptr, V_dev[d]);
  }
  FL_HIP(hipGetLastError());
  return 0;
}
void lincomb(fl_poisson *h, int64_t n, double a, const double *x, double b, const double *z, double *y)
{
  const int nb = (int)std::min<int64_t>((n + 255) / 256, 8192);
  hipLaunchKernelGGL(k_lincomb, dim3(std::max(nb, 1)), dim3(256), 0, h->stream, n, a, x, b, z, y);
}
}

extern "C" int fl_momentum_face_interp(fl_momentum *m, const double *v_dev, const double *const rhs_dev[3], double *const V_dev[3])
{
  if (!m || !v_dev || !V_dev) return FL_ERR_ARG_NULL;
  FL_HIP(hipSetDevice(m->p->device));
  return face_interp(m, 1., v_dev, rhs_dev, V_dev);
}

extern "C" int fl_momentum_face_interp_scaled(fl_momentum *m, double alpha, const double *v_dev, const double *const rhs_dev[3], double *const V_dev[3])
{
  if (!m || !v_dev || !V_dev) return FL_ERR_ARG_NULL;
  FL_HIP(hipSetDevice(m->p->device));
  return face_interp(m, alpha, v_dev, rhs_dev, V_dev);
}

extern "C" int fl_momentum_rhs(fl_momentum *m, double dt, double rho, double mu, const double *v0_dev, const double *p_dev, const double *vbc_dev, double *momrhs_dev)
{
  if (!m || !v0_dev || !momrhs_dev) return FL_ERR_ARG_NULL;
  if (!(rho > 0.)) return FL_ERR_ARG_OUTOFRANGE;
  fl_poisson *h = m->p;
  FL_HIP(hipSetDevice(h->device));
  const size_t N = (size_t)h->ncell;
  FL_CHK(mom_vec(m, 7));
  for (int c = 0; c < 3; ++c) launch_pad_copy(h->stream, h->g, v0_dev + c * N, m->vec[7] + (size_t)c * h->padlen);
  FL_CHK(mom_ghosts(m, m->vec[7]));
  MomP co = m->mp;
  co.cI   = 1.;
  co.cC   = 0.;
  co.cL   = 0.5 * mu * dt / rho;
  FL_CHK(mom_scale_tables(m, 1, co));
  mom_apply_t<0, false, 1>(m, m->vec[7], momrhs_dev, nullptr, nullptr, &co);
  if (p_dev) FL_CHK(fl_poisson_project(h, p_dev, momrhs_dev, momrhs_dev + N, momrhs_dev + 2 * N, nullptr, nullptr, nullptr));
  if (vbc_dev) lincomb(h, (int64_t)(3 * N), 1., momrhs_dev, 1., vbc_dev, momrhs_dev);
  FL_HIP(hipGetLastError());
  return FL_SUCCESS;
}

extern "C" int fl_momentum_interp_faces(fl_momentum *m, const double *v_dev, const double *const vbc_dev[9], double *const out_dev[9])
{
  if (!m || !v_dev || !out_dev) return FL_ERR_ARG_NULL;
  fl_poisson *h = m->p;
  FL_HIP(hipSetDevice(h->device));
  FL_CHK(mom_vec(m, 7));
  for (int c = 0; c < 3; ++c) launch_pad_copy(h->stream, h->g, v_dev + (size_t)c * h->ncell, m->vec[7] + (size_t)c * h->padlen);
  FL_CHK(mom_ghosts(m, m->vec[7]));
  for (int c = 0; c < 3; ++c)
    for (int d = 0; d < 3; ++d) {
      if (!out_dev[c * 3 + d]) return FL_ERR_ARG_NULL;
      const int64_t n = h->nface[d];
      const int     nb = (int)std::min<int64_t>((n + 255) / 256, 8192);
      hipLaunchKernelGGL(k_face_interp, dim3(std::max(nb, 1)), dim3(256), 0, h->stream, h->g, m->ft, c == d ? 1 : 2, d, 1., m->vec[7] + (size_t)c * h->padlen, vbc_dev ? vbc_dev[c * 3 + d] : nullptr,
                         out_dev[c * 3 + d]);
    }
  FL_HIP(hipGetLastError());
  return FL_SUCCESS;
}

extern "C" int fl_momentum_interp_faces_ends(fl_momentum *m, const double *v_dev, const double *const vbc_dev[9], double *const out_dev[9])
{
  if (!m || !v_dev || !out_dev) return FL_ERR_ARG_NULL;
  fl_poisson *h = m->p;
  const GridP &g = h->g;
  if (!mom3_grid(g)) return fl_momentum_interp_faces(m, v_dev, vbc_dev, out_dev);
  FL_HIP(hipSetDevice(h->device));
  FL_CHK(mom_vec(m, 7));
  for (int c = 0; c < 3; ++c) launch_pad_copy(h->stream, h->g, v_dev + (size_t)c * h->ncell, m->vec[7] + (size_t)c * h->padlen);
  FL_CHK(mom_ghosts(m, m->vec[7]));
  for (int c = 0; c < 3; ++c)
    for (int d = 0; d < 3; ++d) {
      if (!out_dev[c * 3 + d]) return FL_ERR_ARG_NULL;
      const int64_t n = 2 * h->nface[d] / std::max(d == 0 ? g.fx : (d == 1 ? g.fy : g.fz), 1);
      const int     nb = (int)std::max<int64_t>(1, std::min<int64_t>((n + 255) / 256, 8192));
      hipLaunchKernelGGL(k_face_interp_ends, dim3(nb), dim3(256), 0, h->stream, g, m->ft, c == d ? 1 : 2, d, m->vec[7] + (size_t)c * h->padlen, vbc_dev ? vbc_dev[c * 3 + d] : nullptr, out_dev[c * 3 + d]);
    }
  FL_HIP(hipGetLastError());
  return FL_SUCCESS;
}

extern "C" int fl_abf_jacobian_mult(fl_momentum *m, const double *v_dev, const double *const V_dev[3], const double *p_dev, double *fv_dev, double *const fV_dev[3], double *fp_dev)
{
  if (!m || !v_dev || !V_dev || !p_dev || !fv_dev || !fV_dev || !fp_dev) return FL_ERR_ARG_NULL;
  fl_poisson *h = m->p;
  FL_HIP(hipSetDevice(h->device));
  const int64_t N = h->ncell;
  if (!m->tmpv) FL_CHK(fl_dev_alloc(h, (void **)&m->tmpv, sizeof(double) * 3 * (size_t)N, true));
  if (!m->srhs) FL_CHK(fl_dev_alloc(h, (void **)&m->srhs, sizeof(double) * (size_t)N, true));
  for (int d = 0; d < 3; ++d)
    if (!V_dev[d] || !fV_dev[d]) return FL_ERR_ARG_NULL;
  FL_CHK(fl_momentum_apply(m, v_dev, fv_dev));
  lincomb(h, N, -1., p_dev, 0., nullptr, m->srhs);
  lincomb(h, 3 * N, 1., v_dev, 0., nullptr, m->tmpv);
  for (int d = 0; d < 3; ++d) lincomb(h, h->nface[d], 1., V_dev[d], 0., nullptr, fV_dev[d]);
  FL_CHK(fl_poisson_project(h, m->srhs, m->tmpv, m->tmpv + N, m->tmpv + 2 * N, fV_dev[0], fV_dev[1], fV_dev[2]));
  lincomb(h, 3 * N, 1., fv_dev, 1., m->tmpv, fv_dev);
  lincomb(h, 3 * N, 1., fv_dev, -1., v_dev, fv_dev);
  FL_CHK(face_interp(m, -1., m->tmpv, fV_dev, fV_dev));
  FL_CHK(fl_poisson_rhs(h, V_dev[0], V_dev[1], V_dev[2], nullptr, fp_dev));
  lincomb(h, N, -1., fp_dev, 0., nullptr, fp_dev);
  FL_HIP(hipGetLastError());
  return FL_SUCCESS;
}

namespace {

int nblk_flat(int64_t n) { return (int)std::max<int64_t>(1, std::min<int64_t>((n + 255) / 256, 8192)); }

int compute_ainv(fl_momentum *m, int type, double **out)
{
  fl_poisson   *h = m->p;
  const int64_t n3 = 3 * h->ncell;
  if (!*out) FL_CHK(fl_dev_alloc(h, (void **)out, sizeof(double) * (size_t)n3, true));
  if (type == FL_ABF_AINV_DIAG) FL_CHK(fl_momentum_diagonal(m, *out));
  else FL_CHK(fl_momentum_rowsum(m, *out));
  hipLaunchKernelGGL(k_recip, dim3(nblk_flat(n3)), dim3(256), 0, h->stream, n3, (const double *)*out, *out);
  return 0;
}

int ensure_ainv_scratch(fl_momentum *m)
{
  fl_poisson *h = m->p;
  if (!m->gv) FL_CHK(fl_dev_alloc(h, (void **)&m->gv, sizeof(double) * 3 * (size_t)h->ncell, true));
  for (int d = 0; d < 3; ++d)
    if (!m->zV[d]) FL_CHK(fl_dev_alloc(h, (void **)&m->zV[d], sizeof(double) * (size_t)std::max<int64_t>(h->nface[d], 1), true));
  return 0;
}

int schur_apply_var(fl_momentum *m, const double *p, double *y)
{
  fl_poisson   *h = m->p;
  const int64_t N = h->ncell, n3 = 3 * N;
  if (knob(K_schur_var_fused) != 0 && fl_schur_var_usable(h)) {
    FL_CHK(fl_ensure_vec(h, &h->w0));
    launch_pad_copy(h->stream, h->g, p, h->w0);
    FL_CHK(fl_schur_var_fill_ghosts(h, h->w0));
    SchurVarT t;
    for (int d = 0; d < 3; ++d) {
      t.w0[d] = m->ft.w0[0][d];
      t.w1[d] = m->ft.w1[0][d];
      t.c0[d] = m->ft.c0[0][d];
    }
    return fl_schur_var_apply_fused(h, t, m->ainv[0], h->w0, y);
  }
  FL_CHK(ensure_ainv_scratch(m));
  FL_HIP(hipMemsetAsync(m->gv, 0, sizeof(double) * (size_t)n3, h->stream));
  for (int d = 0; d < 3; ++d) FL_HIP(hipMemsetAsync(m->zV[d], 0, sizeof(double) * (size_t)h->nface[d], h->stream));
  FL_CHK(fl_poisson_project(h, p, m->gv, m->gv + N, m->gv + 2 * N, m->zV[0], m->zV[1], m->zV[2]));
  hipLaunchKernelGGL(k_scale_by, dim3(nblk_flat(n3)), dim3(256), 0, h->stream, n3, (const double *)m->ainv[0], 1., (const double *)m->gv, m->gv, 0);
  FL_CHK(face_interp(m, 1., m->gv, m->zV, m->zV));
  FL_CHK(fl_poisson_rhs(h, m->zV[0], m->zV[1], m->zV[2], nullptr, y));
  lincomb(h, N, -1., y, 0., nullptr, y);
  return 0;
}

int dot_cells(fl_poisson *h, const double *x, const double *y, double *out)
{
  const int64_t n = h->ncell;
  FL_CHK(fl_ensure_partials(h, 1024));
  const int nb = (int)std::max<int64_t>(1, std::min<int64_t>((n + 255) / 256, 1024));
  hipLaunchKernelGGL(k_dot, dim3(nb), dim3(256), 0, h->stream, n, x, y, h->partial);
  launch_reduce(h->stream, h->partial, nb, h->partial_stride, 1, h->sums);
  if (h->multi) FL_CHK(h->comm.allreduce(h->stream, h->sums, NSLOT));
  FL_HIP(hipMemcpyAsync(out, h->sums, sizeof(double), hipMemcpyDeviceToHost, h->stream));
  FL_HIP(hipStreamSynchronize(h->stream));
  return 0;
}

int schur_solve_var(fl_momentum *m, const double *b, double *x, const fl_ksp_opts *o, fl_ksp_stats *st)
{
  fl_poisson   *h = m->p;
  const int64_t N = h->ncell;
  constexpr int M = 20;
  while ((int)m->gm.size() < 2 * M + 2) {
    double *v = nullptr;
    FL_CHK(fl_dev_alloc(h, (void **)&v, sizeof(double) * (size_t)N, true));
    m->gm.push_back(v);
  }
  double **V = m->gm.data(), **Z = m->gm.data() + M + 1, *w = m->gm[2 * M + 1];
  fl_ksp_opts inner = *o;
  inner.rtol        = std::max(o->rtol, 1e-2);
  inner.history     = nullptr;
  inner.nhistory    = 0;
  fl_ksp_stats ist;
  struct Events {
    hipEvent_t a = nullptr, b = nullptr;
    ~Events()
    {
      if (a) (void)hipEventDestroy(a);
      if (b) (void)hipEventDestroy(b);
    }
  } ev;
  FL_HIP(hipEventCreate(&ev.a));
  FL_HIP(hipEventCreate(&ev.b));
  hipEvent_t e0 = ev.a, e1 = ev.b;
  FL_HIP(hipEventRecord(e0, h->stream));
  double H[(M + 1) * M], cs[M], sn[M], g[M + 1], y[M];
  double bnorm = 0., beta = 0.;
  FL_CHK(dot_cells(h, b, b, &bnorm));
  bnorm = std::sqrt(bnorm);
  const double ttol = std::max(o->rtol * bnorm, o->atol);
  FL_HIP(hipMemsetAsync(x, 0, sizeof(double) * (size_t)N, h->stream));
  int    its = 0, reason = 0, nh = 0;
  double rnorm = bnorm;
  if (o->history && o->nhistory > 0) o->history[nh++] = bnorm;
  bool first = true;
  while (!reason) {
    if (first) lincomb(h, N, 1., b, 0., nullptr, w);
    else {
      FL_CHK(schur_apply_var(m, x, w));
      lincomb(h, N, -1., w, 1., b, w);
    }
    first = false;
    FL_CHK(dot_cells(h, w, w, &beta));
    beta  = std::sqrt(beta);
    rnorm = beta;
    if (std::isnan(beta)) { reason = FL_DIVERGED_NANORINF; break; }
    if (beta <= ttol) { reason = beta < o->atol ? FL_CONVERGED_ATOL : FL_CONVERGED_RTOL; break; }
    if (its >= o->maxit) { reason = FL_DIVERGED_ITS; break; }
    lincomb(h, N, 1. / beta, w, 0., nullptr, V[0]);
    std::fill(g, g + M + 1, 0.);
    g[0] = beta;
    int j = 0;
    for (; j < M && its < o->maxit; ++j) {
      FL_CHK(fl_poisson_solve(h, V[j], Z[j], &inner, &ist));
      if (ist.reason < 0 && ist.reason != FL_DIVERGED_ITS) { reason = ist.reason; break; }
      FL_CHK(schur_apply_var(m, Z[j], w));
      for (int i = 0; i <= j; ++i) {
        double hij;
        FL_CHK(dot_cells(h, w, V[i], &hij));
        H[i * M + j] = hij;
        lincomb(h, N, 1., w, -hij, V[i], w);
      }
      double hn;
      FL_CHK(dot_cells(h, w, w, &hn));
      hn = std::sqrt(hn);
      H[(j + 1) * M + j] = hn;
      for (int i = 0; i < j; ++i) {
        const double a = H[i * M + j], c = H[(i + 1) * M + j];
        H[i * M + j]       = cs[i] * a + sn[i] * c;
        H[(i + 1) * M + j] = -sn[i] * a + cs[i] * c;
      }
      {
        const double a = H[j * M + j], c = H[(j + 1) * M + j], r = std::hypot(a, c);
        cs[j] = r > 0. ? a / r : 1.;
        sn[j] = r > 0. ? c / r : 0.;
        H[j * M + j]       = r;
        H[(j + 1) * M + j] = 0.;
        g[j + 1]           = -sn[j] * g[j];
        g[j]               = cs[j] * g[j];
      }
      ++its;
      rnorm = std::fabs(g[j + 1]);
      if (o->history && nh < o->nhistory) o->history[nh++] = rnorm;
      if (rnorm <= ttol || hn == 0.) {
        ++j;
        break;
      }
      lincomb(h, N, 1. / hn, w, 0., nullptr, V[j + 1]);
    }
    for (int i = j - 1; i >= 0; --i) {
      double acc = g[i];
      for (int k = i + 1; k < j; ++k) acc -= H[i * M + k] * y[k];
      y[i] = acc / H[i * M + i];
    }
    for (int i = 0; i < j; ++i) lincomb(h, N, 1., x, y[i], Z[i], x);
    if (reason) break;
  }
  FL_HIP(hipEventRecord(e1, h->stream));
  FL_HIP(hipStreamSynchronize(h->stream));
  float ms = 0.f;
  FL_HIP(hipEventElapsedTime(&ms, e0, e1));
  st->iters   = its;
  st->reason  = reason;
  st->rnorm0  = bnorm;
  st->rnorm   = rnorm;
  st->seconds = ms * 1e-3;
  return 0;
}

}

extern "C" int fl_momentum_rowsum(fl_momentum *m, double *out_dev)
{
  if (!m || !out_dev) return FL_ERR_ARG_NULL;
  if (!m->have_state && m->mp.cC != 0.) return FL_ERR_ARG_WRONGSTATE;
  fl_poisson   *h = m->p;
  const int64_t n3 = 3 * h->ncell;
  FL_HIP(hipSetDevice(h->device));
  if (!m->tmpv) FL_CHK(fl_dev_alloc(h, (void **)&m->tmpv, sizeof(double) * (size_t)n3, true));
  hipLaunchKernelGGL(k_fill, dim3(nblk_flat(n3)), dim3(256), 0, h->stream, n3, 1., m->tmpv);
  return fl_momentum_apply(m, m->tmpv, out_dev);
}

extern "C" int fl_abf_set_ainv_types(fl_momentum *m, int schur_type, int upper_type)
{
  if (!m) return FL_ERR_ARG_NULL;
  for (int t : {schur_type, upper_type})
    if (t != FL_ABF_AINV_ID && t != FL_ABF_AINV_DIAG && t != FL_ABF_AINV_ROWSUM) return FL_ERR_SUP;
  m->schur_ainv = schur_type;
  m->upper_ainv = upper_type;
  return FL_SUCCESS;
}

extern "C" int fl_abf_schur_apply(fl_momentum *m, const double *p_dev, double *y_dev)
{
  if (!m || !p_dev || !y_dev) return FL_ERR_ARG_NULL;
  fl_poisson *h = m->p;
  FL_HIP(hipSetDevice(h->device));
  if (m->schur_ainv == FL_ABF_AINV_ID) return fl_poisson_apply(h, p_dev, y_dev);
  if (!m->have_state && m->mp.cC != 0.) return FL_ERR_ARG_WRONGSTATE;
  FL_CHK(compute_ainv(m, m->schur_ainv, &m->ainv[0]));
  FL_CHK(schur_apply_var(m, p_dev, y_dev));
  FL_HIP(hipGetLastError());
  return FL_SUCCESS;
}

extern "C" int fl_abf_apply(fl_momentum *m, const fl_ksp_opts *momentum_opts, const fl_ksp_opts *schur_opts, const double *momrhs_dev, const double *const interprhs_dev[3], const double *contrhs_dev,
                            double *v_dev, double *const V_dev[3], double *p_dev, fl_ksp_stats stats[2])
{
  if (!m || !momentum_opts || !schur_opts || !momrhs_dev || !v_dev || !V_dev || !p_dev || !stats) return FL_ERR_ARG_NULL;
  fl_poisson *h = m->p;
  FL_HIP(hipSetDevice(h->device));
  if (!m->srhs) FL_CHK(fl_dev_alloc(h, (void **)&m->srhs, sizeof(double) * (size_t)h->ncell, true));
  FL_CHK(fl_momentum_solve(m, momrhs_dev, v_dev, momentum_opts, &stats[0]));
  FL_CHK(fl_momentum_face_interp(m, v_dev, interprhs_dev, V_dev));
  FL_CHK(fl_poisson_rhs(h, V_dev[0], V_dev[1], V_dev[2], contrhs_dev, m->srhs));
  const size_t N = (size_t)h->ncell;
  if (m->schur_ainv == FL_ABF_AINV_ID) FL_CHK(fl_poisson_solve(h, m->srhs, p_dev, schur_opts, &stats[1]));
  else {
    FL_CHK(compute_ainv(m, m->schur_ainv, &m->ainv[0]));
    FL_CHK(schur_solve_var(m, m->srhs, p_dev, schur_opts, &stats[1]));
  }
  if (m->upper_ainv == FL_ABF_AINV_ID) return fl_poisson_project(h, p_dev, v_dev, v_dev + N, v_dev + 2 * N, V_dev[0], V_dev[1], V_dev[2]);
  FL_CHK(compute_ainv(m, m->upper_ainv, &m->ainv[1]));
  FL_CHK(ensure_ainv_scratch(m));
  const int64_t n3 = 3 * (int64_t)N;
  FL_HIP(hipMemsetAsync(m->gv, 0, sizeof(double) * (size_t)n3, h->stream));
  FL_CHK(fl_poisson_project(h, p_dev, m->gv, m->gv + N, m->gv + 2 * N, V_dev[0], V_dev[1], V_dev[2]));
  hipLaunchKernelGGL(k_scale_by, dim3(nblk_flat(n3)), dim3(256), 0, h->stream, n3, (const double *)m->ainv[1], 0., (const double *)m->gv, v_dev, 1);
  hipLaunchKernelGGL(k_scale_by, dim3(nblk_flat(n3)), dim3(256), 0, h->stream, n3, (const double *)m->ainv[1], 1., (const double *)m->gv, m->gv, 0);
  FL_CHK(face_interp(m, 1., m->gv, V_dev, V_dev));
  FL_HIP(hipGetLastError());
  return FL_SUCCESS;
}


extern "C" int fl_vec_lincomb(fl_poisson *h, int64_t n, double a, const double *x_dev, double b, const double *z_dev, double *y_dev)
{
  if (!h || !x_dev || !y_dev) return FL_ERR_ARG_NULL;
  if (n < 0) return FL_ERR_ARG_OUTOFRANGE;
  FL_HIP(hipSetDevice(h->device));
  if (n > 0) lincomb(h, n, a, x_dev, b, z_dev, y_dev);
  FL_HIP(hipGetLastError());
  return FL_SUCCESS;
}

extern "C" int fl_vec_dot(fl_poisson *h, int64_t n, const double *x_dev, const double *y_dev, double *result)
{
  if (!h || !x_dev || !y_dev || !result) return FL_ERR_ARG_NULL;
  if (n < 0) return FL_ERR_ARG_OUTOFRANGE;
  FL_HIP(hipSetDevice(h->device));
  FL_CHK(fl_ensure_partials(h, 1024));
  const int nb = (int)std::max<int64_t>(1, std::min<int64_t>((n + 255) / 256, 1024));
  hipLaunchKernelGGL(k_dot, dim3(nb), dim3(256), 0, h->stream, n, x_dev, y_dev, h->partial);
  launch_reduce(h->stream, h->partial, nb, h->partial_stride, 1, h->sums);
  if (h->multi) FL_CHK(h->comm.allreduce(h->stream, h->sums, NSLOT));
  FL_HIP(hipMemcpyAsync(result, h->sums, sizeof(double), hipMemcpyDeviceToHost, h->stream));
  FL_HIP(hipStreamSynchronize(h->stream));
  return FL_SUCCESS;
}

extern "C" int fl_vec_mdot(fl_poisson *h, int64_t n, const double *x_dev, const double *const *ys_dev, int k, double *out)
{
  if (!h || !x_dev || !ys_dev || !out) return FL_ERR_ARG_NULL;
  if (n < 0 || k < 0) return FL_ERR_ARG_OUTOFRANGE;
  FL_HIP(hipSetDevice(h->device));
  FL_CHK(fl_ensure_partials(h, 1024));
  const int nb = (int)std::max<int64_t>(1, std::min<int64_t>((n + 255) / 256, 1024));
  for (int i0 = 0; i0 < k; i0 += 8) {
    const int kk = std::min(8, k - i0);
    Vec8      Y;
    for (int i = 0; i < 8; ++i) {
      Y.p[i] = i < kk ? ys_dev[i0 + i] : x_dev;
      if (!Y.p[i]) return FL_ERR_ARG_NULL;
    }
    hipLaunchKernelGGL(k_mdot8, dim3(nb), dim3(256), 0, h->stream, n, x_dev, Y, kk, h->partial, h->partial_stride);
    launch_reduce(h->stream, h->partial, nb, h->partial_stride, 8, h->sums);
    if (h->multi) FL_CHK(h->comm.allreduce(h->stream, h->sums, NSLOT));
    FL_HIP(hipMemcpyAsync(out + i0, h->sums, sizeof(double) * kk, hipMemcpyDeviceToHost, h->stream));
  }
  FL_HIP(hipStreamSynchronize(h->stream));
  return FL_SUCCESS;
}

extern "C" int fl_vec_maxpy(fl_poisson *h, int64_t n, double *x_dev, const double *alphas, const double *const *ys_dev, int k)
{
  if (!h || !x_dev || !ys_dev || !alphas) return FL_ERR_ARG_NULL;
  if (n < 0 || k < 0) return FL_ERR_ARG_OUTOFRANGE;
  FL_HIP(hipSetDevice(h->device));
  const int nb = (int)std::max<int64_t>(1, std::min<int64_t>((n + 255) / 256, 8192));
  for (int i0 = 0; i0 < k && n > 0; i0 += 8) {
    const int kk = std::min(8, k - i0);
    Vec8      Y;
    Coef8     A;
    for (int i = 0; i < 8; ++i) {
      Y.p[i] = i < kk ? ys_dev[i0 + i] : x_dev;
      A.a[i] = i < kk ? alphas[i0 + i] : 0.;
      if (!Y.p[i]) return FL_ERR_ARG_NULL;
    }
    hipLaunchKernelGGL(k_maxpy8, dim3(nb), dim3(256), 0, h->stream, n, x_dev, A, Y, kk);
  }
  FL_HIP(hipGetLastError());
  return FL_SUCCESS;
}


extern "C" int fldbg_mom_apply(fl_momentum *m, int mode, int reps, double *ms_out)
{
  fl_poisson *h = m->p;
  FL_HIP(hipSetDevice(h->device));
  FL_CHK(mom_vec(m, 5));
  FL_CHK(mom_vec(m, 6));
  FL_CHK(mom_vec(m, 7));
  auto go = [&]() {
    switch (mode & 3) {
      case 0: mom_apply_t<0, false, 0>(m, m->vec[7], m->vec[6], nullptr, nullptr); break;
      case 1: mom_apply_t<0, true, 0>(m, m->vec[7], m->vec[6], nullptr, nullptr); break;
      case 2: mom_apply_t<1, true, 0>(m, m->vec[7], m->vec[6], m->vec[5], nullptr); break;
      default: mom_apply_t<2, true, 0>(m, m->vec[7], m->vec[6], nullptr, nullptr); break;
    }
  };
  go();
  FL_HIP(hipEventRecord(h->ev0, h->stream));
  for (int r = 0; r < reps; ++r) go();
  FL_HIP(hipEventRecord(h->ev1, h->stream));
  FL_HIP(hipStreamSynchronize(h->stream));
  FL_HIP(hipGetLastError());
  float ms = 0.f;
  FL_HIP(hipEventElapsedTime(&ms, h->ev0, h->ev1));
  *ms_out = ms / reps;
  return 0;
}

__global__ void __launch_bounds__(256) k_div(int64_t n, const double *__restrict__ a, const double *__restrict__ d, double *__restrict__ out)
{
  for (int64_t i = (int64_t)blockIdx.x * 256 + threadIdx.x; i < n; i += (int64_t)gridDim.x * 256) out[i] = a[i] / d[i];
}

static int momentum_gmres(fl_momentum *m, const double *b_dev, double *x_dev, const fl_ksp_opts *opts, fl_ksp_stats *stats)
{
  if (opts->pc != FL_PC_JACOBI && opts->pc != FL_PC_NONE) return FL_ERR_SUP;
  if (opts->norm_type != FL_NORM_PRECONDITIONED) return FL_ERR_SUP;
  if (opts->maxit < 0) return FL_ERR_ARG_OUTOFRANGE;
  const int restart = opts->gmres_restart > 0 ? opts->gmres_restart : 30;
  if (restart > 1000) return FL_ERR_ARG_OUTOFRANGE;
  fl_poisson *h = m->p;
  FL_HIP(hipSetDevice(h->device));
  std::memset(stats, 0, sizeof(*stats));
  const bool    jac = opts->pc == FL_PC_JACOBI;
  const int64_t n = 3 * (int64_t)h->ncell;
  hipStream_t   s = h->stream;
  FL_CHK(mom_vec(m, 7));
  auto kvec = [&](size_t i) -> int {
    if (m->kb.size() <= i) m->kb.resize(i + 1, nullptr);
    if (!m->kb[i]) FL_CHK(fl_dev_alloc(h, (void **)&m->kb[i], sizeof(double) * (size_t)n, true));
    return 0;
  };
  for (size_t i = 0; i < 4; ++i) FL_CHK(kvec(i));
  double *W = m->kb[0], *X = m->kb[1], *R = m->kb[2];
  auto apply = [&](const double *xin, double *yout) -> int {
    for (int c = 0; c < 3; ++c) launch_pad_copy(s, h->g, xin + (size_t)c * h->ncell, m->vec[7] + (size_t)c * h->padlen);
    FL_CHK(mom_ghosts(m, m->vec[7]));
    if (jac) mom_apply_t<0, true, 1>(m, m->vec[7], yout, nullptr, nullptr);
    else mom_apply_t<0, false, 1>(m, m->vec[7], yout, nullptr, nullptr);
    return 0;
  };
  double *MB = m->kb[3];
  if (jac) {
    FL_CHK(fl_momentum_diagonal(m, W));
    hipLaunchKernelGGL(k_div, dim3(nblk_flat(n)), dim3(256), 0, s, n, b_dev, (const double *)W, MB);
  } else lincomb(h, n, 1., b_dev, 0., nullptr, MB);
  hipEvent_t e0 = h->ev0, e1 = h->ev1;
  FL_HIP(hipEventRecord(e0, s));
  std::vector<double> hist, H((size_t)(restart + 1) * restart, 0.), cs(restart, 0.), sn(restart, 0.), g(restart + 1, 0.), hcol(restart + 1, 0.), y(restart, 0.);
  std::vector<const double *> basis(restart + 1, nullptr);
  FL_HIP(hipMemsetAsync(X, 0, sizeof(double) * (size_t)n, s));
  lincomb(h, n, 1., MB, 0., nullptr, R);
  double beta = 0.;
  FL_CHK(fl_vec_dot(h, n, R, R, &beta));
  beta = std::sqrt(beta);
  const double rnorm0 = beta, ttol = std::max(opts->rtol * rnorm0, opts->atol);
  auto converged = [&](double v) {
    if (std::isnan(v) || std::isinf(v)) return (int)FL_DIVERGED_NANORINF;
    if (v <= ttol) return v < opts->atol ? (int)FL_CONVERGED_ATOL : (int)FL_CONVERGED_RTOL;
    if (v >= opts->dtol * rnorm0) return (int)FL_DIVERGED_DTOL;
    return 0;
  };
  hist.push_back(beta);
  int    it = 0, reason = converged(beta);
  double res = beta;
  if (!reason && opts->maxit == 0) reason = FL_DIVERGED_ITS;
  while (!reason) {
    FL_CHK(kvec(4));
    lincomb(h, n, 1. / beta, R, 0., nullptr, m->kb[4]);
    std::fill(g.begin(), g.end(), 0.);
    g[0] = beta;
    int k = 0;
    for (; k < restart && !reason; ++k) {
      FL_CHK(kvec(4 + (size_t)k + 1));
      for (int i = 0; i <= k; ++i) basis[i] = m->kb[4 + (size_t)i];
      FL_CHK(apply(m->kb[4 + (size_t)k], W));
      FL_CHK(fl_vec_mdot(h, n, W, basis.data(), k + 1, hcol.data()));
      for (int i = 0; i <= k; ++i) y[i] = -hcol[i];
      FL_CHK(fl_vec_maxpy(h, n, W, y.data(), basis.data(), k + 1));
      double hk1 = 0.;
      FL_CHK(fl_vec_dot(h, n, W, W, &hk1));
      hk1 = std::sqrt(hk1);
      hcol[k + 1] = hk1;
      const bool happy = !(hk1 > 1e-30 * rnorm0);
      if (!happy) lincomb(h, n, 1. / hk1, W, 0., nullptr, m->kb[4 + (size_t)k + 1]);
      for (int i = 0; i < k; ++i) {
        const double t = cs[i] * hcol[i] + sn[i] * hcol[i + 1];
        hcol[i + 1]    = -sn[i] * hcol[i] + cs[i] * hcol[i + 1];
        hcol[i]        = t;
      }
      const double d = std::hypot(hcol[k], hcol[k + 1]);
      cs[k] = d > 0. ? hcol[k] / d : 1.;
      sn[k] = d > 0. ? hcol[k + 1] / d : 0.;
      hcol[k]     = d;
      hcol[k + 1] = 0.;
      g[k + 1]    = -sn[k] * g[k];
      g[k]        = cs[k] * g[k];
      for (int i = 0; i <= k; ++i) H[(size_t)i * restart + k] = hcol[i];
      res = std::fabs(g[k + 1]);
      ++it;
      hist.push_back(res);
      reason = converged(res);
      if (!reason && happy) reason = FL_CONVERGED_RTOL;
      if (!reason && it >= opts->maxit) reason = FL_DIVERGED_ITS;
    }
    for (int i = k - 1; i >= 0; --i) {
      double t = g[i];
      for (int j = i + 1; j < k; ++j) t -= H[(size_t)i * restart + j] * y[j];
      y[i] = t / H[(size_t)i * restart + i];
    }
    for (int i = 0; i < k; ++i) basis[i] = m->kb[4 + (size_t)i];
    FL_CHK(fl_vec_maxpy(h, n, X, y.data(), basis.data(), k));
    if (reason) break;
    FL_CHK(apply(X, W));
    lincomb(h, n, 1., MB, -1., W, R);
    FL_CHK(fl_vec_dot(h, n, R, R, &beta));
    beta = std::sqrt(beta);
    if (!(beta > 0.)) {
      reason = std::isnan(beta) ? FL_DIVERGED_NANORINF : FL_CONVERGED_ATOL;
      break;
    }
  }
  lincomb(h, n, 1., X, 0., nullptr, x_dev);
  FL_HIP(hipEventRecord(e1, s));
  FL_HIP(hipStreamSynchronize(s));
  FL_HIP(hipGetLastError());
  float ms = 0.f;
  FL_HIP(hipEventElapsedTime(&ms, e0, e1));
  stats->iters   = it;
  stats->reason  = reason;
  stats->rnorm0  = rnorm0;
  stats->rnorm   = res;
  stats->seconds = ms * 1e-3;
  if (opts->history && opts->nhistory > 0) std::memcpy(opts->history, hist.data(), sizeof(double) * std::min<size_t>((size_t)opts->nhistory, hist.size()));
  return FL_SUCCESS;
}
```

### fluca_amd/host/fluca_host.c

```c
#include "../../include/fluca_host_impl.h"

#include <math.h>
#include <pthread.h>
#include <stdio.h>
#include <stdlib.h>
#include <string.h>
#include <strings.h>

enum { E_MEM = 55, E_SUP = 56, E_ARG_WRONG = 62, E_FILE_OPEN = 65, E_FILE_WRITE = 67 , E_ARG_OUTOFRANGE = 63, E_ARG_WRONGSTATE = 73, E_ARG_NULL = 85, E_ARG_UNKNOWN_TYPE = 86, E_ARG_TYPENOTSET = 89 };

#define FLCHK(call)             \
  do {                          \
    FlErrorCode e_ = (call);    \
    if (e_) return e_;          \
  } while (0)
#define FLABI(call)             \
  do {                          \
    int r_ = (call);            \
    if (r_) return -r_;         \
  } while (0)

#define FLABI_T(call)           \
  do {                          \
    int r_ = (call);            \
    if (r_) {                   \
      trace_end();              \
      return -r_;               \
    }                           \
  } while (0)
#define FLCHK_T(call)           \
  do {                          \
    FlErrorCode e_ = (call);    \
    if (e_) {                   \
      trace_end();              \
      return e_;                \
    }                           \
  } while (0)
static void trace_end(void);
static void trace_begin(const char *name);
static int    step_timing(void);
static double step_clock(NS ns);
static FlErrorCode ns_jacobian(NS ns);
static FlErrorCode ibm_force_monitor_destroy(void **ctx);
static FlErrorCode ibm_body_to_ref(NS ns);
static FlErrorCode ibm_body_from_ref(NS ns, int64_t Ln);


#define MAXTYPES 16
typedef struct {
  char name[32];
  void *create;
} TypeEntry;
static TypeEntry MeshList[MAXTYPES], NSList[MAXTYPES];
static int       nMeshTypes = 0, nNSTypes = 0;
static pthread_once_t  register_once = PTHREAD_ONCE_INIT;
static pthread_mutex_t register_lock = PTHREAD_MUTEX_INITIALIZER;

static void RegisterBuiltins(void)
{
  MeshRegister(MESHCART, MeshCreate_Cart);
  NSRegister(NSCNLINEAR, NSCreate_CNLinear);
}
static void RegisterAll(void) { pthread_once(&register_once, RegisterBuiltins); }

static const char *opt_find(int argc, char **argv, const char *name)
{
  for (int i = 1; i + 1 < argc; ++i)
    if (argv[i] && !strcmp(argv[i], name)) return argv[i + 1];
  return NULL;
}
static int opt_flag(int argc, char **argv, const char *name, int *v)
{
  for (int i = 1; i < argc; ++i) {
    if (!argv[i] || strcmp(argv[i], name)) continue;
    const char *s = i + 1 < argc ? argv[i + 1] : NULL;
    if (!s || (s[0] == '-' && !(s[1] >= '0' && s[1] <= '9'))) {
      *v = 1;
      return 1;
    }
    if (!strcasecmp(s, "true") || !strcasecmp(s, "yes") || !strcasecmp(s, "on") || !strcmp(s, "1")) *v = 1;
    else if (!strcasecmp(s, "false") || !strcasecmp(s, "no") || !strcasecmp(s, "off") || !strcmp(s, "0")) *v = 0;
    else return -1;
    return 1;
  }
  return 0;
}
static int opt_int64(int argc, char **argv, const char *name, int64_t *v)
{
  const char *s = opt_find(argc, argv, name);
  if (!s) return 0;
  *v = strtoll(s, NULL, 10);
  return 1;
}
static int opt_real(int argc, char **argv, const char *name, double *v)
{
  const char *s = opt_find(argc, argv, name);
  if (!s) return 0;
  *v = strtod(s, NULL);
  return 1;
}


FlErrorCode FlucaViewerCreate(FlucaViewerType type, char mode, FlucaViewer *viewer)
{
  if (!type || !viewer) return E_ARG_NULL;
  FlucaViewer v = (FlucaViewer)calloc(1, sizeof(*v));
  if (!v) return E_MEM;
  v->type   = type;
  v->mode   = mode;
  v->seqnum = -1;
  *viewer   = v;
  return 0;
}
static FlErrorCode ViewerVPrintf_ASCII(FlucaViewer v, const char *fmt, va_list ap)
{
  FILE *f = (FILE *)v->data;
  for (int i = 0; i < v->tab; ++i) fputs("  ", f);
  return vfprintf(f, fmt, ap) < 0 ? E_FILE_WRITE : 0;
}
static FlErrorCode ViewerDestroy_ASCII(FlucaViewer v)
{
  FILE *f = (FILE *)v->data;
  if (f && f != stdout) fclose(f);
  else if (f) fflush(f);
  return 0;
}
FlErrorCode FlucaViewerASCIIOpen(const char *filename, FlucaViewer *viewer)
{
  if (!viewer) return E_ARG_NULL;
  FILE *f = !filename || !strcmp(filename, "stdout") ? stdout : fopen(filename, "w");
  if (!f) return E_FILE_OPEN;
  const FlErrorCode rc = FlucaViewerCreate(FLUCAVIEWERASCII, 'w', viewer);
  if (rc) {
    if (f != stdout) fclose(f);
    return rc;
  }
  (*viewer)->data         = f;
  (*viewer)->ops->vprintf = ViewerVPrintf_ASCII;
  (*viewer)->ops->destroy = ViewerDestroy_ASCII;
  return 0;
}
FlErrorCode FlucaViewerASCIIPrintf(FlucaViewer viewer, const char *fmt, ...)
{
  if (!viewer || !fmt) return E_ARG_NULL;
  if (!viewer->ops->vprintf) return E_SUP;
  va_list ap;
  va_start(ap, fmt);
  const FlErrorCode rc = viewer->ops->vprintf(viewer, fmt, ap);
  va_end(ap);
  return rc;
}
FlErrorCode FlucaViewerASCIIPushTab(FlucaViewer viewer) { if (!viewer) return E_ARG_NULL; ++viewer->tab; return 0; }
FlErrorCode FlucaViewerASCIIPopTab(FlucaViewer viewer)
{
  if (!viewer) return E_ARG_NULL;
  if (viewer->tab <= 0) return E_ARG_WRONGSTATE;
  --viewer->tab;
  return 0;
}
FlErrorCode FlucaViewerGetType(FlucaViewer viewer, FlucaViewerType *type)
{
  if (!viewer || !type) return E_ARG_NULL;
  *type = viewer->type;
  return 0;
}
FlErrorCode FlucaViewerDestroy(FlucaViewer *viewer)
{
  if (!viewer || !*viewer) return 0;
  const FlErrorCode rc = (*viewer)->ops->destroy ? (*viewer)->ops->destroy(*viewer) : 0;
  free(*viewer);
  *viewer = NULL;
  return rc;
}
static int viewer_is(FlucaViewer v, const char *type) { return v && v->type && !strcmp(v->type, type); }
#define WITH_STDOUT_VIEWER(viewer, body)                          \
  do {                                                            \
    FlucaViewer own_ = NULL;                                      \
    if (!(viewer)) {                                              \
      FLCHK(FlucaViewerASCIIOpen(NULL, &own_));                   \
      (viewer) = own_;                                            \
    }                                                             \
    FlErrorCode rc_ = (body);                                     \
    if (own_) FlucaViewerDestroy(&own_);                          \
    return rc_;                                                   \
  } while (0)


FlErrorCode MeshRegister(const char name[], FlErrorCode (*create)(Mesh))
{
  pthread_mutex_lock(&register_lock);
  if (nMeshTypes >= MAXTYPES) {
    pthread_mutex_unlock(&register_lock);
    return E_MEM;
  }
  snprintf(MeshList[nMeshTypes].name, sizeof(MeshList[0].name), "%s", name);
  MeshList[nMeshTypes].create = (void *)create;
  __atomic_store_n(&nMeshTypes, nMeshTypes + 1, __ATOMIC_RELEASE);
  pthread_mutex_unlock(&register_lock);
  return 0;
}

FlErrorCode MeshCreate(Mesh *mesh)
{
  if (!mesh) return E_ARG_NULL;
  RegisterAll();
  Mesh m = (Mesh)calloc(1, sizeof(*m));
  if (!m) return E_MEM;
  m->dim  = 3;
  m->size = 1;
  *mesh   = m;
  return 0;
}

FlErrorCode MeshSetType(Mesh mesh, MeshType type)
{
  if (!mesh || !type) return E_ARG_NULL;
  for (int i = 0, nt = __atomic_load_n(&nMeshTypes, __ATOMIC_ACQUIRE); i < nt; ++i)
    if (!strcmp(MeshList[i].name, type)) {
      if (mesh->ops->destroy) FLCHK(mesh->ops->destroy(mesh));
      memset(mesh->ops, 0, sizeof(mesh->ops));
      snprintf(mesh->type_name, sizeof(mesh->type_name), "%s", type);
      return ((FlErrorCode(*)(Mesh))MeshList[i].create)(mesh);
    }
  return E_ARG_UNKNOWN_TYPE;
}

FlErrorCode MeshSetRank(Mesh mesh, int rank, int size)
{
  if (!mesh) return E_ARG_NULL;
  if (mesh->setupcalled) return E_ARG_WRONGSTATE;
  if (size < 1 || rank < 0 || rank >= size) return E_ARG_OUTOFRANGE;
  mesh->rank = rank;
  mesh->size = size;
  return 0;
}

static FlErrorCode MeshSetFromOptions_Cart(Mesh mesh, int argc, char **argv)
{
  Mesh_Cart *cart = (Mesh_Cart *)mesh->data;
  char       opt[64];
  for (int d = 0; d < 3; ++d) {
    int64_t v;
    snprintf(opt, sizeof(opt), "-cart_grid_%c", 'x' + d);
    if (opt_int64(argc, argv, opt, &v)) {
      if (v < 1) return E_ARG_OUTOFRANGE;
      cart->N[d] = v;
    }
    snprintf(opt, sizeof(opt), "-cart_ranks_%c", 'x' + d);
    if (opt_int64(argc, argv, opt, &v)) cart->nRanks[d] = (int)v;
    snprintf(opt, sizeof(opt), "-cart_boundary_type_%c", 'x' + d);
    const char *s = opt_find(argc, argv, opt);
    if (s) {
      if (!strcasecmp(s, "none")) cart->bndTypes[d] = MESHCART_BOUNDARY_NONE;
      else if (!strcasecmp(s, "periodic")) cart->bndTypes[d] = MESHCART_BOUNDARY_PERIODIC;
      else return E_ARG_WRONG;
    }
    snprintf(opt, sizeof(opt), "-cart_refine_%c", 'x' + d);
    if (opt_int64(argc, argv, opt, &v)) {
      if (v < 1) return E_ARG_OUTOFRANGE;
      cart->refineFactor[d] = v;
    }
  }
  int64_t nRefine = 0;
  if (opt_int64(argc, argv, "-cart_refine", &nRefine)) {
    if (nRefine < 0) return E_ARG_OUTOFRANGE;
    for (int d = 0; d < 3; ++d) {
      int64_t total = 1;
      for (int64_t i = 0; i < nRefine; ++i) total *= cart->refineFactor[d];
      cart->N[d] *= total;
      if (cart->l[d])
        for (int i = 0; i < cart->nRanks[d]; ++i) cart->l[d][i] *= total;
    }
  }
  return 0;
}

FlErrorCode MeshCartSetRefinementFactor(Mesh mesh, int64_t refine_x, int64_t refine_y, int64_t refine_z)
{
  if (!mesh) return E_ARG_NULL;
  if (mesh->setupcalled) return E_ARG_WRONGSTATE;
  Mesh_Cart *cart = (Mesh_Cart *)mesh->data;
  if (refine_x > 0) cart->refineFactor[0] = refine_x;
  if (refine_y > 0) cart->refineFactor[1] = refine_y;
  if (refine_z > 0) cart->refineFactor[2] = refine_z;
  return 0;
}
FlErrorCode MeshCartGetRefinementFactor(Mesh mesh, int64_t *refine_x, int64_t *refine_y, int64_t *refine_z)
{
  if (!mesh) return E_ARG_NULL;
  Mesh_Cart *cart = (Mesh_Cart *)mesh->data;
  if (refine_x) *refine_x = cart->refineFactor[0];
  if (refine_y) *refine_y = cart->refineFactor[1];
  if (refine_z) *refine_z = cart->refineFactor[2];
  return 0;
}

static void decide_ranks(int size, const int64_t N[3], int ranks[3])
{
  int fixed = 1, nfree = 0;
  for (int d = 0; d < 3; ++d)
    if (ranks[d] > 0) fixed *= ranks[d];
    else ++nfree;
  int rest = size / (fixed > 0 ? fixed : 1);
// ... 1867 lines not shown
  if (!ns) return E_ARG_NULL;
  if (!ns->setupcalled || !ns->data) return E_ARG_WRONGSTATE;
  NS_CNLinear *c = (NS_CNLinear *)ns->data;
  if (v) *v = c->sol_v;
  if (p) *p = c->sol_p;
  if (V)
    for (int d = 0; d < 3; ++d) V[d] = c->sol_V[d];
  return 0;
}

static FlErrorCode cnl_eval_velocity(NS ns, int b, double t, const double *out[3])
{
  NS_CNLinear     *c = (NS_CNLinear *)ns->data;
  Mesh_Cart       *cart = (Mesh_Cart *)ns->mesh->data;
  const fl_decomp *D    = &ns->mesh->decomp;
  const int        ax = b / 2, side = b % 2, a1 = ax == 0 ? 1 : 0, a2 = ax == 2 ? 1 : 2;
  const int64_t    n1 = D->len[a1], n2 = D->len[a2];
  if (!ns->bcs[b].velocity) return E_ARG_WRONGSTATE;
  for (int k = 0; k < 2; ++k)
    if (c->bc_have[b][k] && c->bc_time[b][k] == t && c->bc_fn[b][k] == ns->bcs[b].velocity && c->bc_ctx[b][k] == ns->bcs[b].ctx_velocity) {
      for (int q = 0; q < 3; ++q) out[q] = c->bc_plane[b][k][q];
      c->bc_old[b] = 1 - k;
      return 0;
    }
  const int k = c->bc_old[b];
  FLABI(fl_poisson_upload_fence(ns->poisson));
  c->bc_have[b][k] = 0;
  for (int q = 0; q < 3; ++q)
    if (!c->bc_plane[b][k][q]) FLABI(fl_malloc_host(sizeof(double) * (size_t)c->plane_cap, (void **)&c->bc_plane[b][k][q]));
  double *p0 = c->bc_plane[b][k][0], *p1 = c->bc_plane[b][k][1], *p2 = c->bc_plane[b][k][2];
  for (int64_t j = 0; j < n2; ++j)
    for (int64_t i = 0; i < n1; ++i) {
      double xb[3], val[3] = {0., 0., 0.};
      xb[ax] = cart->xf[ax][side ? cart->N[ax] : 0];
      xb[a1] = cart->xc[a1][D->lo[a1] + i];
      xb[a2] = cart->xc[a2][D->lo[a2] + j];
      FLCHK(ns->bcs[b].velocity(3, t, xb, val, ns->bcs[b].ctx_velocity));
      p0[j * n1 + i] = val[0];
      p1[j * n1 + i] = val[1];
      p2[j * n1 + i] = val[2];
    }
  c->bc_have[b][k] = 1;
  c->bc_time[b][k] = t;
  c->bc_fn[b][k]   = ns->bcs[b].velocity;
  c->bc_ctx[b][k]  = ns->bcs[b].ctx_velocity;
  c->bc_old[b]     = 1 - k;
  for (int q = 0; q < 3; ++q) out[q] = c->bc_plane[b][k][q];
  return 0;
}

static int cnl_touches(NS ns, int b)
{
  const fl_decomp *D = &ns->mesh->decomp;
  return b % 2 ? D->coord[b / 2] == D->ranks[b / 2] - 1 : D->coord[b / 2] == 0;
}

static FlErrorCode cnl_upload(NS ns, const double *host, int64_t n)
{
  NS_CNLinear *c = (NS_CNLinear *)ns->data;
  FLABI(fl_poisson_upload(ns->poisson, c->plane_dev, host, sizeof(double) * (size_t)n));
  return 0;
}
static FlErrorCode cnl_scratch(NS ns, double **plane)
{
  NS_CNLinear *c = (NS_CNLinear *)ns->data;
  if (c->plane_next == 7) {
    FLABI(fl_poisson_upload_fence(ns->poisson));
    c->plane_next = 0;
  }
  *plane = c->plane_host[c->plane_next++];
  return 0;
}

static FlErrorCode cnl_residual(NS ns, double *rnorm)
{
  NS_CNLinear *c = (NS_CNLinear *)ns->data;
  fl_poisson  *h = ns->poisson;
  const double *xV[3] = {c->x_V[0], c->x_V[1], c->x_V[2]};
  FLABI(fl_abf_jacobian_mult(ns->momentum, c->x_v, xV, c->x_p, c->r_v, c->r_V, c->r_p));
  double s = 0., part;
  FLABI(fl_vec_lincomb(h, 3 * c->sz[0], -1., c->r_v, 1., c->f_v, c->r_v));
  FLABI(fl_vec_dot(h, 3 * c->sz[0], c->r_v, c->r_v, &part));
  s += part;
  for (int d = 0; d < 3; ++d) {
    FLABI(fl_vec_lincomb(h, c->sz[1 + d], -1., c->r_V[d], 1., c->f_V[d], c->r_V[d]));
    FLABI(fl_vec_dot(h, c->sz[1 + d], c->r_V[d], c->r_V[d], &part));
    s += part;
  }
  FLABI(fl_vec_lincomb(h, c->sz[0], -1., c->r_p, 1., c->f_p, c->r_p));
  FLABI(fl_vec_dot(h, c->sz[0], c->r_p, c->r_p, &part));
  s += part;
  *rnorm = sqrt(s);
  return 0;
}

static FlErrorCode cv_alloc(NS ns, NSVec *a)
{
  NS_CNLinear *c = (NS_CNLinear *)ns->data;
  FLCHK(cnl_alloc(ns, &a->v, 3 * c->sz[0]));
  FLCHK(cnl_alloc(ns, &a->p, c->sz[0]));
  for (int d = 0; d < 3; ++d) FLCHK(cnl_alloc(ns, &a->V[d], c->sz[1 + d]));
  return 0;
}
static FlErrorCode cv_lincomb(NS ns, double a, const NSVec *x, double b, const NSVec *z, NSVec *y)
{
  NS_CNLinear *c = (NS_CNLinear *)ns->data;
  fl_poisson  *h = ns->poisson;
  FLABI(fl_vec_lincomb(h, 3 * c->sz[0], a, x->v, b, z ? z->v : NULL, y->v));
  FLABI(fl_vec_lincomb(h, c->sz[0], a, x->p, b, z ? z->p : NULL, y->p));
  for (int d = 0; d < 3; ++d) FLABI(fl_vec_lincomb(h, c->sz[1 + d], a, x->V[d], b, z ? z->V[d] : NULL, y->V[d]));
  return 0;
}
static FlErrorCode cv_dot(NS ns, const NSVec *x, const NSVec *y, double *out)
{
  NS_CNLinear *c = (NS_CNLinear *)ns->data;
  fl_poisson  *h = ns->poisson;
  double       s = 0., part;
  FLABI(fl_vec_dot(h, 3 * c->sz[0], x->v, y->v, &part));
  s += part;
  FLABI(fl_vec_dot(h, c->sz[0], x->p, y->p, &part));
  s += part;
  for (int d = 0; d < 3; ++d) {
    FLABI(fl_vec_dot(h, c->sz[1 + d], x->V[d], y->V[d], &part));
    s += part;
  }
  *out = s;
  return 0;
}
#define CV_MAXK 208
static FlErrorCode cv_mdot(NS ns, const NSVec *x, const NSVec *Y, int k, double *out)
{
  NS_CNLinear  *c = (NS_CNLinear *)ns->data;
  fl_poisson   *h = ns->poisson;
  const double *ys[CV_MAXK];
  double        part[CV_MAXK];
  if (k > CV_MAXK) return E_ARG_OUTOFRANGE;
  for (int i = 0; i < k; ++i) out[i] = 0.;
  for (int a = 0; a < 5; ++a) {
    const int64_t n  = a == 0 ? 3 * c->sz[0] : a == 1 ? c->sz[0] : c->sz[a - 1];
    const double *xa = a == 0 ? x->v : a == 1 ? x->p : x->V[a - 2];
    for (int i = 0; i < k; ++i) ys[i] = a == 0 ? Y[i].v : a == 1 ? Y[i].p : Y[i].V[a - 2];
    FLABI(fl_vec_mdot(h, n, xa, ys, k, part));
    for (int i = 0; i < k; ++i) out[i] += part[i];
  }
  return 0;
}
static FlErrorCode cv_msub(NS ns, NSVec *x, const double *coef, const NSVec *Y, int k)
{
  NS_CNLinear  *c = (NS_CNLinear *)ns->data;
  fl_poisson   *h = ns->poisson;
  const double *ys[CV_MAXK];
  double        neg[CV_MAXK];
  if (k > CV_MAXK) return E_ARG_OUTOFRANGE;
  for (int i = 0; i < k; ++i) neg[i] = -coef[i];
  for (int a = 0; a < 5; ++a) {
    const int64_t n  = a == 0 ? 3 * c->sz[0] : a == 1 ? c->sz[0] : c->sz[a - 1];
    double       *xa = a == 0 ? x->v : a == 1 ? x->p : x->V[a - 2];
    for (int i = 0; i < k; ++i) ys[i] = a == 0 ? Y[i].v : a == 1 ? Y[i].p : Y[i].V[a - 2];
    FLABI(fl_vec_maxpy(h, n, xa, neg, ys, k));
  }
  return 0;
}
static FlErrorCode cv_pcapply(NS ns, const NSVec *r, NSVec *z)
{
  fl_ksp_stats  st[2];
  const double *rV[3] = {r->V[0], r->V[1], r->V[2]};
  FLABI(fl_abf_apply(ns->momentum, &ns->mom, &ns->schur, r->v, rV, r->p, z->v, z->V, z->p, st));
  ns->mom_its += st[0].iters;
  ns->schur_its += st[1].iters;
  if (st[0].reason == FL_DIVERGED_NANORINF || st[1].reason == FL_DIVERGED_NANORINF) ns->reason = -1;
  return 0;
}
static FlErrorCode cv_jmult(NS ns, const NSVec *x, NSVec *y)
{
  const double *xV[3] = {x->V[0], x->V[1], x->V[2]};
  FLABI(fl_abf_jacobian_mult(ns->momentum, x->v, xV, x->p, y->v, y->V, y->p));
  return 0;
}

static FlErrorCode cnl_gmres(NS ns, const NSVec *f, NSVec *x)
{
  const int    m = ns->gmres_restart;
  NS_CNLinear *c = (NS_CNLinear *)ns->data;
  if (c->gm_cap < m + 1) {
    NSVec *nv = (NSVec *)calloc((size_t)m + 1, sizeof(NSVec));
    if (!nv) return E_MEM;
    if (c->gm_V) memcpy(nv, c->gm_V, sizeof(NSVec) * (size_t)c->gm_nalloc);
    free(c->gm_V);
    c->gm_V   = nv;
    c->gm_cap = m + 1;
  }
  NSVec     *Vk = c->gm_V;
  NSVec     *w = &c->gm_w, *t = &c->gm_t;
  double   *H = (double *)calloc((size_t)(m + 1) * m, sizeof(double)), *cs = (double *)calloc(m, sizeof(double)), *sn = (double *)calloc(m, sizeof(double)),
           *g = (double *)calloc((size_t)m + 1, sizeof(double)), *y = (double *)calloc(m, sizeof(double));
  FlErrorCode rc = 0;
#define GM(call)          \
  do {                    \
    rc = (call);          \
    if (rc) goto done;    \
  } while (0)
  if (!H || !cs || !sn || !g || !y) {
    rc = E_MEM;
    goto done;
  }
  if (!w->v) GM(cv_alloc(ns, w));
  if (!t->v) GM(cv_alloc(ns, t));
  double fnorm, beta;
  GM(cv_dot(ns, f, f, &fnorm));
  fnorm = sqrt(fnorm);
  const double ttol = ns->ksp_rtol * fnorm > ns->ksp_atol ? ns->ksp_rtol * fnorm : ns->ksp_atol;
  GM(cv_lincomb(ns, 0., f, 0., NULL, x));
  ns->ksp_its    = 0;
  ns->ksp_rnorm  = fnorm;
  ns->ksp_rnorm0 = fnorm;
  int first = 1;
  while (ns->reason >= 0) {
    if (first) GM(cv_lincomb(ns, 1., f, 0., NULL, w));
    else {
      GM(cv_jmult(ns, x, w));
      GM(cv_lincomb(ns, -1., w, 1., f, w));
    }
    first = 0;
    GM(cv_dot(ns, w, w, &beta));
    beta          = sqrt(beta);
    ns->ksp_rnorm = beta;
    if (!(beta == beta)) { ns->reason = -1; break; }
    if (beta <= ttol || ns->ksp_its >= ns->ksp_max_it) break;
    if (c->gm_nalloc < 1) { GM(cv_alloc(ns, &Vk[0])); c->gm_nalloc = 1; }
    GM(cv_lincomb(ns, 1. / beta, w, 0., NULL, &Vk[0]));
    memset(g, 0, sizeof(double) * ((size_t)m + 1));
    g[0] = beta;
    int j = 0, conv = 0;
    for (; j < m && ns->ksp_its < ns->ksp_max_it; ++j) {
      GM(cv_pcapply(ns, &Vk[j], t));
      if (ns->reason < 0) break;
      GM(cv_jmult(ns, t, w));
      {
        double hcol[CV_MAXK];
        GM(cv_mdot(ns, w, Vk, j + 1, hcol));
        for (int i = 0; i <= j; ++i) H[i * m + j] = hcol[i];
        GM(cv_msub(ns, w, hcol, Vk, j + 1));
      }
      double hn;
      GM(cv_dot(ns, w, w, &hn));
      hn = sqrt(hn);
      H[(j + 1) * m + j] = hn;
      for (int i = 0; i < j; ++i) {
        const double a = H[i * m + j], b = H[(i + 1) * m + j];
        H[i * m + j]       = cs[i] * a + sn[i] * b;
        H[(i + 1) * m + j] = -sn[i] * a + cs[i] * b;
      }
      {
        const double a = H[j * m + j], b = H[(j + 1) * m + j], r = hypot(a, b);
        cs[j] = r > 0. ? a / r : 1.;
        sn[j] = r > 0. ? b / r : 0.;
        H[j * m + j]       = r;
        H[(j + 1) * m + j] = 0.;
        g[j + 1]           = -sn[j] * g[j];
        g[j]               = cs[j] * g[j];
      }
      ++ns->ksp_its;
      ns->ksp_rnorm = fabs(g[j + 1]);
      if (ns->ksp_rnorm <= ttol || hn == 0.) {
        conv = 1;
        ++j;
        break;
      }
      if (j + 1 < m || 1) {
        if (c->gm_nalloc < j + 2) { GM(cv_alloc(ns, &Vk[j + 1])); c->gm_nalloc = j + 2; }
        GM(cv_lincomb(ns, 1. / hn, w, 0., NULL, &Vk[j + 1]));
      }
    }
    for (int i = j - 1; i >= 0; --i) {
      double sacc = g[i];
      for (int k = i + 1; k < j; ++k) sacc -= H[i * m + k] * y[k];
      y[i] = sacc / H[i * m + i];
    }
    if (j > 0) {
      GM(cv_lincomb(ns, y[0], &Vk[0], 0., NULL, w));
      for (int i = 1; i < j; ++i) GM(cv_lincomb(ns, 1., w, y[i], &Vk[i], w));
      GM(cv_pcapply(ns, w, t));
      GM(cv_lincomb(ns, 1., x, 1., t, x));
    }
    if (conv || ns->reason < 0) break;
  }
  if (ns->reason >= 0 && ns->ksp_rnorm > ttol && ns->ksp_its >= ns->ksp_max_it) ns->reason = -1;
done:
#undef GM
  free(H); free(cs); free(sn); free(g); free(y);
  return rc;
}

static FlErrorCode NSFormFunction_CNLinear(NS ns, const NSVec *x, NSVec *f)
{
  NS_CNLinear *c = (NS_CNLinear *)ns->data;
  (void)x;
  if (!c || !f || !f->v || !f->p) return E_ARG_NULL;
  if (!c->have_sol0 || !ns->momentum) return E_ARG_WRONGSTATE;
  Mesh_Cart    *cart = (Mesh_Cart *)ns->mesh->data;
  fl_poisson   *h = ns->poisson;
  const int64_t N = c->sz[0];
  const double  dt = ns->dt, t = ns->t, cv = 0.5 * ns->mu * dt / ns->rho;
  FLABI(fl_momentum_rhs(ns->momentum, dt, ns->rho, ns->mu, c->sol0_v, ns->step == 0 ? c->sol0_p : c->phalf, NULL, f->v));
  for (int d = 0; d < 3; ++d) FLABI(fl_vec_lincomb(h, c->sz[1 + d], 0., f->V[d], 0., NULL, f->V[d]));
  FLABI(fl_vec_lincomb(h, N, 0., f->p, 0., NULL, f->p));
  for (int b = 0; b < 6; ++b) {
    if (ns->bcs[b].type != NS_BC_VELOCITY || !cnl_touches(ns, b)) continue;
    const int        ax = b / 2, side = b % 2, a1 = ax == 0 ? 1 : 0, a2 = ax == 2 ? 1 : 2;
    const fl_decomp *D = &ns->mesh->decomp;
    const int64_t    np = D->len[a1] * D->len[a2], n = cart->N[ax];
    const double    *xf = cart->xf[ax], *xc = cart->xc[ax];
    const double    *vb0[3], *vb1[3];
    FLCHK(cnl_eval_velocity(ns, b, t, vb0));
    FLCHK(cnl_eval_velocity(ns, b, t + dt, vb1));
    double h1, h2, h3, hcell;
    if (n < 3) return E_SUP;
    if (!side) {
      h1 = xc[0] - xf[0]; h2 = xc[1] - xc[0]; h3 = xc[2] - xc[0]; hcell = xf[1] - xf[0];
    } else {
      h1 = xf[n] - xc[n - 1]; h2 = xc[n - 1] - xc[n - 2]; h3 = xc[n - 1] - xc[n - 3]; hcell = xf[n] - xf[n - 1];
    }
    const double cl = 2. * (h2 + h3) / (h1 * (h1 + h2) * (h1 + h3)), sgn = side ? 0.5 : -0.5;
    for (int q = 0; q < 3; ++q) {
      double *tmp;
      FLCHK(cnl_scratch(ns, &tmp));
      for (int64_t a = 0; a < np; ++a) tmp[a] = cv * cl * (vb0[q][a] + vb1[q][a]) - dt * sgn * (vb1[q][a] * vb0[ax][a] + vb0[q][a] * vb1[ax][a]) / hcell;
      FLCHK(cnl_upload(ns, tmp, np));
      FLABI(fl_boundary_add_cells(h, b, 1., c->plane_dev, f->v + q * N));
    }
    FLCHK(cnl_upload(ns, vb1[ax], np));
    FLABI(fl_boundary_set_faces(h, b, 1., c->plane_dev, f->V[ax]));
  }
  if (ns->ibm) {
    FLABI(fl_ibm_interp(ns->ibm, 3, c->sol0_v, ns->ibm_U));
    FLABI(fl_vec_lincomb(h, 3 * ns->ibm_L, -1., ns->ibm_U, 1., ns->ibm_Ut, ns->ibm_U));
    FLABI(fl_ibm_spread(ns->ibm, 3, ns->ibm_U, ns->ibm_dV, f->v));
  }
  FLCHK(buoyancy_add(ns, f->v));
  {
    int     rhiechow = 0;
    double *w = c->d_v;
    const double tq = ns->step == 0 ? t : t - 0.5 * dt, tp = t + 0.5 * dt, kappa = dt / ns->rho;
    for (int b = 0; b < 6; ++b) {
      if (ns->bcs[b].type != NS_BC_PRESSURE_OUTLET || !cnl_touches(ns, b)) continue;
      const int        ax = b / 2, side = b % 2, a1 = ax == 0 ? 1 : 0, a2 = ax == 2 ? 1 : 2;
      const fl_decomp *D = &ns->mesh->decomp;
      const int64_t    n1 = D->len[a1], n2 = D->len[a2], np = n1 * n2, n = cart->N[ax];
      const double    *xf = cart->xf[ax], *xc = cart->xc[ax];
      if (!ns->bcs[b].pressure || n < 2) return !ns->bcs[b].pressure ? E_ARG_WRONGSTATE : E_SUP;
      double *pq, *pp, *tmp;
      FLCHK(cnl_scratch(ns, &pq));
      FLCHK(cnl_scratch(ns, &pp));
      FLCHK(cnl_scratch(ns, &tmp));
      int     differs = 0;
      for (int64_t j = 0; j < n2; ++j)
        for (int64_t i = 0; i < n1; ++i) {
          double xb[3], vq = 0., vp = 0.;
          xb[ax] = xf[side ? n : 0];
          xb[a1] = cart->xc[a1][D->lo[a1] + i];
          xb[a2] = cart->xc[a2][D->lo[a2] + j];
          FLCHK(ns->bcs[b].pressure(3, tq, xb, &vq, ns->bcs[b].ctx_pressure));
          FLCHK(ns->bcs[b].pressure(3, tp, xb, &vp, ns->bcs[b].ctx_pressure));
          pq[j * n1 + i] = vq;
          pp[j * n1 + i] = vp;
          differs |= vq != vp;
        }
      const double h1 = side ? xf[n] - xc[n - 1] : xc[0] - xf[0], h2 = side ? xc[n - 1] - xc[n - 2] : xc[1] - xc[0];
      const double cg = (side ? 1. : -1.) * h2 / (h1 * (h1 + h2));
      FLCHK(cnl_upload(ns, pq, np));
      FLABI(fl_boundary_add_cells(h, b, -cg, c->plane_dev, f->v + ax * N));
      if (differs) {
        const double g1 = side ? xf[n] - xc[n - 1] : xc[0] - xf[0], g2 = side ? xf[n] - xc[n - 2] : xc[1] - xf[0];
        const double cgst = (side ? 1. : -1.) * (g1 + g2) / (g1 * g2);
        if (!rhiechow) FLABI(fl_vec_lincomb(h, 3 * N, 0., w, 0., NULL, w));
        rhiechow = 1;
        for (int64_t a = 0; a < np; ++a) tmp[a] = pq[a] - pp[a];
        FLCHK(cnl_upload(ns, tmp, np));
        FLABI(fl_boundary_add_cells(h, b, kappa * cg, c->plane_dev, w + ax * N));
        FLABI(fl_boundary_add_faces(h, b, kappa * cgst, c->plane_dev, f->V[ax]));
      }
    }
    int any_outlet = 0;
    for (int b = 0; b < 6; ++b) any_outlet |= ns->bcs[b].type == NS_BC_PRESSURE_OUTLET;
    if (any_outlet && ns->mesh->size > 1) {
      double flag = (double)rhiechow;
      FLABI(fl_poisson_allreduce_sum(h, &flag, 1));
      if (flag > 0. && !rhiechow) FLABI(fl_vec_lincomb(h, 3 * N, 0., w, 0., NULL, w));
      rhiechow = flag > 0.;
    }
    if (rhiechow) {
      const double *rhs[3] = {f->V[0], f->V[1], f->V[2]};
      FLABI(fl_momentum_face_interp_scaled(ns->momentum, -1., w, rhs, f->V));
    }
  }
  return 0;
}

static FlErrorCode NSFormJacobian_CNLinear(NS ns, const NSVec *x, NSMat J, NSFormJacobianType type)
{
  NS_CNLinear *c = (NS_CNLinear *)ns->data;
  (void)x;
  if (!J) return E_ARG_NULL;
  if (type == NS_INIT_JACOBIAN) FLABI(fl_abf_set_ainv_types(J, ns->schur_ainv, ns->upper_ainv));
  if (c && c->have_sol0) {
    const double *V0[3] = {c->sol0_V[0], c->sol0_V[1], c->sol0_V[2]};
    const double *W[9];
    for (int q = 0; q < 9; ++q) W[q] = c->W[q];
    FLABI(fl_momentum_set_state_v0(J, ns->dt, ns->rho, ns->mu, V0, W, c->sol0_v));
  }
  return 0;
}

#include <time.h>
static int step_timing(void)
{
  static int on = -1;
  if (on < 0) {
    const char *e = getenv("FLUCA_STEP_TIMING");
    on = e && atoi(e) != 0;
  }
  return on;
}
static double step_clock(NS ns)
{
  struct timespec ts;
  if (ns->poisson) (void)fl_poisson_synchronize(ns->poisson);
  clock_gettime(CLOCK_MONOTONIC, &ts);
  return ts.tv_sec + 1e-9 * ts.tv_nsec;
}

static FlErrorCode ns_jacobian(NS ns)
{
  if (ns->momentum) return 0;
  if (!ns->poisson) return E_ARG_WRONGSTATE;
  FLABI(fl_momentum_create(ns->poisson, &ns->momentum));
  return NSFormJacobian(ns, NULL, ns->momentum, NS_INIT_JACOBIAN);
}

static FlErrorCode NSStep_CNLinear(NS ns)
{
  NS_CNLinear *c = (NS_CNLinear *)ns->data;
  if (!c) return E_ARG_WRONGSTATE;
  fl_poisson   *h = ns->poisson;
  const int64_t N = c->sz[0];
  FLCHK(ns_jacobian(ns));
  if (!ns->bc_keep)
    for (int b = 0; b < 6; ++b) c->bc_have[b][0] = c->bc_have[b][1] = 0;
  const int timing = step_timing();
  double    tm[6] = {0., 0., 0., 0., 0., 0.};
  if (timing) tm[0] = step_clock(ns);
  const int guess = ns->ksp_type != 2 ? ns->mom_guess_previous : 0;
  if (guess == 2 && c->have_sol0) FLABI(fl_vec_lincomb(h, 3 * N, 2., c->sol_v, -1., c->sol0_v, c->x_v));
  else if (guess) FLABI(fl_vec_lincomb(h, 3 * N, 1., c->sol_v, 0., NULL, c->x_v));
  FLABI(fl_vec_lincomb(h, 3 * N, 1., c->sol_v, 0., NULL, c->sol0_v));
  FLABI(fl_vec_lincomb(h, N, 1., c->sol_p, 0., NULL, c->sol0_p));
  for (int d = 0; d < 3; ++d) FLABI(fl_vec_lincomb(h, c->sz[1 + d], 1., c->sol_V[d], 0., NULL, c->sol0_V[d]));
  c->have_sol0 = 1;

  FLABI(fl_momentum_interp_faces_ends(ns->momentum, c->sol0_v, NULL, c->W));
  for (int b = 0; b < 6; ++b) {
    if (ns->bcs[b].type != NS_BC_VELOCITY || !cnl_touches(ns, b)) continue;
    const int        ax = b / 2, a1 = ax == 0 ? 1 : 0, a2 = ax == 2 ? 1 : 2;
    const fl_decomp *D = &ns->mesh->decomp;
    const int64_t    np = D->len[a1] * D->len[a2];
    const double    *vb0[3];
    FLCHK(cnl_eval_velocity(ns, b, ns->t, vb0));
    for (int q = 0; q < 3; ++q) {
      FLCHK(cnl_upload(ns, vb0[q], np));
      FLABI(fl_boundary_set_faces(h, b, 1., c->plane_dev, c->W[q * 3 + ax]));
    }
  }
  NSVec x = {c->x_v, {c->x_V[0], c->x_V[1], c->x_V[2]}, c->x_p}, f = {c->f_v, {c->f_V[0], c->f_V[1], c->f_V[2]}, c->f_p};
  if (timing) tm[1] = step_clock(ns);
  FLCHK(NSFormFunction(ns, &x, &f));
  if (timing) tm[2] = step_clock(ns);
  FLCHK(NSFormJacobian(ns, &x, ns->momentum, NS_UPDATE_JACOBIAN));
  if (timing) tm[3] = step_clock(ns);
  fl_ksp_stats  st[2];
  const double *fV[3] = {c->f_V[0], c->f_V[1], c->f_V[2]};
  if (ns->ksp_type == 2) {
    ns->reason  = 0;
    ns->mom_its = ns->schur_its = 0;
    FLCHK(cnl_gmres(ns, &f, &x));
  } else {
    fl_ksp_opts mom1 = ns->mom;
    if (guess) mom1.initial_guess_nonzero = 1;
    FLABI(fl_abf_apply(ns->momentum, &mom1, &ns->schur, c->f_v, fV, c->f_p, c->x_v, c->x_V, c->x_p, st));
  }
  if (ns->ksp_type != 2) {
    ns->ksp_its   = 1;
    ns->reason    = 0;
    ns->mom_its   = st[0].iters;
    ns->schur_its = st[1].iters;
  }
  if (ns->ksp_type != 2 && (st[0].reason == FL_DIVERGED_NANORINF || st[1].reason == FL_DIVERGED_NANORINF)) ns->reason = -1;
  if (ns->ksp_type == 0 && ns->reason >= 0) {
    double fnorm, rnorm = 0., part;
    FLABI(fl_vec_dot(h, 3 * N, c->f_v, c->f_v, &fnorm));
    for (int d = 0; d < 3; ++d) {
      FLABI(fl_vec_dot(h, c->sz[1 + d], c->f_V[d], c->f_V[d], &part));
      fnorm += part;
    }
    FLABI(fl_vec_dot(h, N, c->f_p, c->f_p, &part));
    fnorm += part;
    fnorm = sqrt(fnorm);
    ns->ksp_rnorm0 = fnorm;
    const double ttol = ns->ksp_rtol * fnorm > ns->ksp_atol ? ns->ksp_rtol * fnorm : ns->ksp_atol;
    for (;;) {
      FLCHK(cnl_residual(ns, &rnorm));
      ns->ksp_rnorm = rnorm;
      if (!(rnorm == rnorm)) { ns->reason = -1; break; }
      if (rnorm <= ttol) break;
      if (ns->ksp_its >= ns->ksp_max_it) { ns->reason = -1; break; }
      const double *rV[3] = {c->r_V[0], c->r_V[1], c->r_V[2]};
      FLABI(fl_abf_apply(ns->momentum, &ns->mom, &ns->schur, c->r_v, rV, c->r_p, c->d_v, c->d_V, c->d_p, st));
      ns->mom_its += st[0].iters;
      ns->schur_its += st[1].iters;
      if (st[0].reason == FL_DIVERGED_NANORINF || st[1].reason == FL_DIVERGED_NANORINF) { ns->reason = -1; break; }
      FLABI(fl_vec_lincomb(h, 3 * N, 1., c->x_v, 1., c->d_v, c->x_v));
      FLABI(fl_vec_lincomb(h, N, 1., c->x_p, 1., c->d_p, c->x_p));
      for (int d = 0; d < 3; ++d) FLABI(fl_vec_lincomb(h, c->sz[1 + d], 1., c->x_V[d], 1., c->d_V[d], c->x_V[d]));
      ++ns->ksp_its;
    }
  }
  if (timing) tm[4] = step_clock(ns);
  if (ns->reason < 0) return 0;
  FLABI(fl_vec_lincomb(h, 3 * N, 1., c->x_v, 0., NULL, c->sol_v));
  for (int d = 0; d < 3; ++d) FLABI(fl_vec_lincomb(h, c->sz[1 + d], 1., c->x_V[d], 0., NULL, c->sol_V[d]));
  FLABI(fl_pressure_update(h, ns->step == 0, c->x_p, c->sol0_p, c->phalf, c->sol_p));
  FLABI(fl_poisson_synchronize(h));
  if (timing) {
    tm[5] = step_clock(ns);
    fprintf(stderr, "[fluca step %lld] copy sol0 + v0interp ends %.4f s | NSFormFunction %.4f | NSFormJacobian %.4f | KSPSolve (PCApply_ABF: kspA %d its, kspS %d its) %.4f | update %.4f\n",
            (long long)ns->step + 1, tm[1] - tm[0], tm[2] - tm[1], tm[3] - tm[2], ns->mom_its, ns->schur_its, tm[4] - tm[3], tm[5] - tm[4]);
  }
  return 0;
}
static FlErrorCode NSView_CNLinear(NS ns, FlucaViewer viewer)
{
  (void)ns;
  (void)viewer;
  return 0;
}
static FlErrorCode NSViewSolution_CNLinear(NS ns, FlucaViewer viewer)
{
  NS_CNLinear *c = (NS_CNLinear *)ns->data;
  if (!c) return E_ARG_WRONGSTATE;
  return viewer->ops->cellfield(viewer, ns, "PressureHalfStep", 1, c->phalf);
}
static FlErrorCode NSLoadSolution_CNLinear(NS ns, FlucaViewer viewer)
{
  NS_CNLinear *c = (NS_CNLinear *)ns->data;
  if (!c) return E_ARG_WRONGSTATE;
  return viewer->ops->cellfield(viewer, ns, "PressureHalfStep", 1, c->phalf);
}
FlErrorCode NSGetSolverVectors(NS ns, NSVec *x, NSVec *r)
{
  if (!ns) return E_ARG_NULL;
  if (!ns->setupcalled || !ns->data) return E_ARG_WRONGSTATE;
  NS_CNLinear *c = (NS_CNLinear *)ns->data;
  if (x) {
    x->v = c->x_v;
    x->p = c->x_p;
    for (int d = 0; d < 3; ++d) x->V[d] = c->x_V[d];
  }
  if (r) {
    r->v = c->f_v;
    r->p = c->f_p;
    for (int d = 0; d < 3; ++d) r->V[d] = c->f_V[d];
  }
  return 0;
}

FlErrorCode NSCreate_CNLinear(NS ns)
{
  ns->ops->setfromoptions = NULL;
  ns->ops->setup          = NSSetUp_CNLinear;
  ns->ops->step           = NSStep_CNLinear;
  ns->ops->formjacobian   = NSFormJacobian_CNLinear;
  ns->ops->formfunction   = NSFormFunction_CNLinear;
  ns->ops->destroy        = NSDestroy_CNLinear;
  ns->ops->view           = NSView_CNLinear;
  ns->ops->viewsolution   = NSViewSolution_CNLinear;
  ns->ops->loadsolution   = NSLoadSolution_CNLinear;
  return 0;
}
```

### include/fluca_host_impl.h

```cpp
#ifndef FLUCA_HOST_IMPL_H
#define FLUCA_HOST_IMPL_H

#include <stdarg.h>
#include "fluca_host.h"

#ifdef __cplusplus
extern "C" {
#endif

struct _FlucaViewerOps {
  FlErrorCode (*vprintf)(FlucaViewer, const char *fmt, va_list ap);
  FlErrorCode (*viewmesh)(FlucaViewer, Mesh);
  FlErrorCode (*loadmesh)(FlucaViewer, int64_t N[3], double *xf[3]);
  FlErrorCode (*solutionbegin)(FlucaViewer, NS, int write);
  FlErrorCode (*cellfield)(FlucaViewer, NS, const char *name, int ncomp, double *dev);
  FlErrorCode (*facefield)(FlucaViewer, NS, const char *name, double *const dev[3]);
  FlErrorCode (*solutionend)(FlucaViewer, NS);
  FlErrorCode (*destroy)(FlucaViewer);
};
struct _p_FlucaViewer {
  struct _FlucaViewerOps ops[1];
  FlucaViewerType        type;
  char                   mode;
  int                    tab;
  int64_t seqnum;
  double  seqval;
  void   *data;
};
FlErrorCode FlucaViewerCreate(FlucaViewerType type, char mode, FlucaViewer *viewer);
FlErrorCode FlucaViewerASCIIPrintf(FlucaViewer viewer, const char *fmt, ...);
FlErrorCode FlucaViewerASCIIPushTab(FlucaViewer viewer);
FlErrorCode FlucaViewerASCIIPopTab(FlucaViewer viewer);

typedef struct {
  int64_t              N[3];
  int                  nRanks[3];
  int64_t             *l[3];
  MeshCartBoundaryType bndTypes[3];
  int64_t              refineFactor[3];
  double              *xf[3], *xc[3];
  double              *coordLoaded[3];
} Mesh_Cart;

struct _p_Mesh {
  struct _MeshOps ops[1];
  char            type_name[32];
  int             dim, rank, size, setupcalled;
  fl_decomp       decomp;
  void           *data;
};
FlErrorCode MeshCreate_Cart(Mesh mesh);

#define MAXNSMONITORS 10
struct _p_NS {
  struct _NSOps        ops[1];
  char                 type_name[32];
  double               rho, mu, dt, t;
  int64_t              step, max_steps;
  double               max_time;
  int                  errorifstepfailed;
  int                  mom_guess_previous;
  int                  bc_keep;
  Mesh                 mesh;
  NSBoundaryCondition *bcs;
  int                  nb, device, setupcalled;
  fl_poisson          *poisson;
  fl_momentum         *momentum;
  fl_ibm              *ibm;
  int64_t              ibm_L;
  const double        *ibm_dV, *ibm_Ut;
  double              *ibm_U;
  int                  ibm_owner;
  void                *ibm_own[6];
  const double        *ibm_X[3];
  FlErrorCode        (*ibm_motion)(double, double *, double *, double *, double *, void *);
  void                *ibm_motion_ctx;
  double               ibm_centre0[3];
  double              *ibm_ref, *ibm_mv;
  int64_t              ibm_cap, ibm_Ucap;
  fl_ksp_opts          schur;
  fl_ksp_opts          mom;
  int                  schur_ainv, upper_ainv;
  int                  ksp_type;
  int                  gmres_restart;
  double               ksp_rtol, ksp_atol;
  int                  ksp_max_it;
  int                  ksp_its, reason;
  int                  mom_its, schur_its;
  double               ksp_rnorm;
  double               ksp_rnorm0;
  int                  nmon;
  FlErrorCode (*mon[MAXNSMONITORS])(NS, void *);
  void *monctx[MAXNSMONITORS];
  FlErrorCode (*mondestroy[MAXNSMONITORS])(void **);
  void                *data;
  int                  ibm_force_ready;
  int                  ibm_have_centre, ibm_have_centre0;
  double               ibm_centre[3];
  int64_t              ibm_Lglobal;
  int                  ibm_nbody;
  const int32_t       *ibm_body;
  void                *ibm_body_own;
  int64_t              ibm_body_cap;
  int64_t              ibm_mon_step;
  int                  nscalar;
  struct NSScalar     *scalars;
  int                  scalar_stages;
  int                  scalar_limiter;
  double               gravity[3];
  double               scalar_theta, scalar_rtol;
  int                  scalar_implicit_ranks;
  int                  scalar_ibm_passes;
  double              *ibm_Q;
  int64_t              ibm_Qcap;
};
struct NSScalar {
  char          name[32];
  fl_scalar    *h;
  double        gamma, val[6];
  int           limiter, substeps, kind[6];
  double       *phi;
  const double *src;
  double        beta, phi_ref;
  double        theta, rtol;
  int           cheb_steps;
  double        cheb_bound;
  int           ibm_npass;
  double        ibm_value[64];
  double        ibm_sum[64];
  double        ibm_sum_dt;
  int           ibm_sum_ready;
};

typedef struct {
  int64_t sz[4];
  double *sol_v, *sol_V[3], *sol_p;
  double *sol0_v, *sol0_V[3], *sol0_p;
  double *phalf;
  double *x_v, *x_V[3], *x_p;
  double *f_v, *f_V[3], *f_p;
  int     have_sol0;
  double *W[9];
  double *r_v, *r_V[3], *r_p, *d_v, *d_V[3], *d_p;
  double *plane_dev, *plane_host[7];
  int64_t plane_cap;
  int     plane_next;
  double     *bc_plane[6][2][3];
  double      bc_time[6][2];
  int         bc_have[6][2], bc_old[6];
  void       *bc_ctx[6][2];
  NSBoundaryConditionFunction bc_fn[6][2];
  NSVec gm_w, gm_t, *gm_V;
  int   gm_nalloc, gm_cap;
} NS_CNLinear;
FlErrorCode NSCreate_CNLinear(NS ns);

#ifdef __cplusplus
}
#endif
#endif
```

Measured before the change: 719.0.

## Share padded v0 across momentum RHS, face interp and state; skip redundant copies

```diff
diff --git a/fluca_amd/build.py b/fluca_amd/build.py
--- a/fluca_amd/build.py
+++ b/fluca_amd/build.py
@@ -10,7 +10,8 @@
 LIB = os.path.join(LIBDIR, "libflucahip.so")
 SOURCES = ["fl_coeff.cpp", "fl_kernels.hip", "fl_api.hip", "fl_knobs.cpp", "fl_place.hip", "fl_halo.hip", "fl_comm.hip", "fl_ksp.hip", "fl_cheb2.hip", "fl_layout.hip", "fl_ibm.hip", "fl_ibm_owner.hip", "fl_ibm_body.hip", "fl_momentum.hip", "fl_mg.hip", "fl_schur_var.hip", "fl_scalar.hip", "fl_buoyancy.hip", "fl_scalar_implicit.hip"]
 HEADERS = ["fl_internal.h", "fl_knobs.h", "fl_handle.h", "fl_msg.h", "fl_ibm_device.h", "fl_ibm_handle.h", "fl_ibm_plan.h", "fl_device.h", "fl_stencil.h", "fl_mom_tile.h", "fl_mom_tile3.h", "fl_limiter.h", "fl_scalar_handle.h", os.path.join("..", "..", "include", "fluca_hip.h"),
-           os.path.join("..", "..", "include", "fluca_hip_implicit.h"), os.path.join("..", "..", "include", "fluca_hip_implicit_ranks.h"), os.path.join("..", "..", "include", "fluca_hip_ibm_scalar.h")]
+           os.path.join("..", "..", "include", "fluca_hip_implicit.h"), os.path.join("..", "..", "include", "fluca_hip_implicit_ranks.h"), os.path.join("..", "..", "include", "fluca_hip_ibm_scalar.h"),
+           os.path.join("..", "..", "include", "fluca_hip_momentum_v0.h")]
 HIPCC = os.environ.get("HIPCC", "/opt/rocm/bin/hipcc")
 FLAGS = ["--offload-arch=gfx950", "-O3", "-std=c++17", "-fPIC", "-Wall", "-Wno-unused-function", "-Wno-unused-result"]
 MANIFEST = os.path.join(LIBDIR, "manifest.json")
@@ -120,7 +121,7 @@
 
 def build_host(force=False, verbose=False):
     src = os.path.join(HERE, "host", "fluca_host.c")
-    hdrs = [os.path.normpath(os.path.join(HERE, "..", "include", h)) for h in ("fluca_host.h", "fluca_host_impl.h", "fluca_hip.h", "fluca_hip_implicit.h", "fluca_hip_implicit_ranks.h", "fluca_hip_ibm_scalar.h")]
+    hdrs = [os.path.normpath(os.path.join(HERE, "..", "include", h)) for h in ("fluca_host.h", "fluca_host_impl.h", "fluca_hip.h", "fluca_hip_implicit.h", "fluca_hip_implicit_ranks.h", "fluca_hip_ibm_scalar.h", "fluca_hip_momentum_v0.h")]
     cmd = [os.environ.get("CC", "gcc"), "-std=gnu99", "-O2", "-fPIC", "-shared", "-Wall", "-o", HOST_LIB, src,
            "-L" + LIBDIR, "-lflucahip", "-Wl,-rpath,$ORIGIN", "-lm", "-ldl", "-pthread"]
     if force or _stale(HOST_LIB, [src, LIB] + hdrs, cmd):
@@ -151,7 +152,7 @@
         if verbose:
             print(f"no HDF5 under {HDF5_ROOT}: libfluca_cgns.so not built", flush=True)
         return None
-    hdrs = [os.path.normpath(os.path.join(HERE, "..", "include", h)) for h in ("fluca_cgns.h", "fluca_host.h", "fluca_host_impl.h", "fluca_hip.h", "fluca_hip_implicit.h", "fluca_hip_implicit_ranks.h", "fluca_hip_ibm_scalar.h")]
+    hdrs = [os.path.normpath(os.path.join(HERE, "..", "include", h)) for h in ("fluca_cgns.h", "fluca_host.h", "fluca_host_impl.h", "fluca_hip.h", "fluca_hip_implicit.h", "fluca_hip_implicit_ranks.h", "fluca_hip_ibm_scalar.h", "fluca_hip_momentum_v0.h")]
     if True:
         cmd = [os.environ.get("CC", "gcc"), "-std=gnu99", "-O2", "-fPIC", "-shared", "-Wall", "-o", CGNS_LIB, src,
                "-I" + os.path.join(HDF5_ROOT, "include"), "-L" + LIBDIR, "-lfluca_host", "-lflucahip",
@@ -176,7 +177,7 @@
     cmd = [os.environ.get("CC", "gcc"), "-std=gnu99", "-O2", "-Wall", "-o", EXAMPLE, src, "-I" + os.path.join(root, "include"),
            "-L" + LIBDIR] + (["-DFLUCA_HAVE_CGNS", "-lfluca_cgns"] if cgns else []) + ["-lfluca_host", "-lflucahip", "-lm",
            "-Wl,-rpath,$ORIGIN", "-Wl,-rpath,/opt/rocm/lib"]
-    deps = [src, HOST_LIB, LIB] + ([CGNS_LIB] if cgns else []) + [os.path.join(root, "include", h) for h in ("fluca_host.h", "fluca_hip.h", "fluca_hip_implicit.h", "fluca_hip_implicit_ranks.h", "fluca_hip_ibm_scalar.h", "fluca_cgns.h")]
+    deps = [src, HOST_LIB, LIB] + ([CGNS_LIB] if cgns else []) + [os.path.join(root, "include", h) for h in ("fluca_host.h", "fluca_hip.h", "fluca_hip_implicit.h", "fluca_hip_implicit_ranks.h", "fluca_hip_ibm_scalar.h", "fluca_hip_momentum_v0.h", "fluca_cgns.h")]
     if os.path.exists(src) and (force or _stale(EXAMPLE, deps, cmd)):
         if verbose:
             print(" ".join(cmd), flush=True)
diff --git a/fluca_amd/capi.py b/fluca_amd/capi.py
--- a/fluca_amd/capi.py
+++ b/fluca_amd/capi.py
@@ -201,7 +201,14 @@
     "fl_scalar_diffusion_solve_ranks": PROTOTYPES_IMPLICIT["fl_scalar_diffusion_solve"],
     "fl_scalar_step_imex_ranks": PROTOTYPES_IMPLICIT["fl_scalar_step_imex"],
 }
-for _name, (_res, _args) in list(PROTOTYPES.items()) + list(PROTOTYPES_IMPLICIT.items()) + list(PROTOTYPES_IBM_SCALAR.items()) + list(PROTOTYPES_IMPLICIT_RANKS.items()):
+PROTOTYPES_MOMENTUM_V0 = {
+    "fl_momentum_set_v0": (C.c_int, [_P, _P]),
+    "fl_momentum_interp_faces_ends_v0": (C.c_int, [_P, _P, _P]),
+    "fl_momentum_rhs_v0": (C.c_int, [_P, C.c_double, C.c_double, C.c_double, _P, _P, _P]),
+    "fl_momentum_set_state_shared_v0": (C.c_int, [_P, C.c_double, C.c_double, C.c_double, _P, _P]),
+}
+for _name, (_res, _args) in (list(PROTOTYPES.items()) + list(PROTOTYPES_IMPLICIT.items()) + list(PROTOTYPES_IBM_SCALAR.items()) + list(PROTOTYPES_IMPLICIT_RANKS.items()) +
+                             list(PROTOTYPES_MOMENTUM_V0.items())):
     _f = getattr(lib, _name)
     _f.restype = _res
     _f.argtypes = _args
diff --git a/fluca_amd/csrc/fl_momentum.hip b/fluca_amd/csrc/fl_momentum.hip
--- a/fluca_amd/csrc/fl_momentum.hip
+++ b/fluca_amd/csrc/fl_momentum.hip
@@ -2,6 +2,7 @@
 
 #include "fl_handle.h"
 #include "fl_device.h"
+#include "../../include/fluca_hip_momentum_v0.h"
 
 namespace fl {
 
@@ -317,6 +318,7 @@
   double     *F = nullptr;
   double     *dg = nullptr;
   double     *v0p = nullptr;
+  bool        have_v0 = false;
   bool        fly = false;
   double     *vec[8] = {nullptr, nullptr, nullptr, nullptr, nullptr, nullptr, nullptr, nullptr};
   int                   schur_ainv = FL_ABF_AINV_ID, upper_ainv = FL_ABF_AINV_ID;
@@ -324,6 +326,7 @@
   std::vector<double *> gm;
   std::vector<double *> kb;
   bool        have_state = false;
+  bool        poisoned = false;
   double      dmean = 1.;
   double      gersh = -1.;
   int         t2x = 1, t2chunk = 1, t2zc = 1, t2blocks = 1;
@@ -542,7 +545,17 @@
 }
 
 namespace {
-int mom_set_state(fl_momentum *m, double dt, double rho, double mu, const double *const V0_dev[3], const double *const v0interp_dev[9], const double *v0_dev)
+int mom_pad_v0(fl_momentum *m, const double *v0_dev)
+{
+  fl_poisson *h = m->p;
+  if (!m->v0p) FL_CHK(fl_dev_alloc(h, (void **)&m->v0p, sizeof(double) * 3 * h->padlen, true));
+  for (int c = 0; c < 3; ++c) launch_pad_copy(h->stream, h->g, v0_dev + (size_t)c * h->ncell, m->v0p + (size_t)c * h->padlen);
+  FL_CHK(mom_ghosts(m, m->v0p));
+  m->have_v0 = true;
+  return 0;
+}
+
+int mom_set_state(fl_momentum *m, double dt, double rho, double mu, const double *const V0_dev[3], const double *const v0interp_dev[9], const double *v0_dev, bool shared_v0 = false)
 {
   if (!m || !V0_dev || !v0interp_dev) return FL_ERR_ARG_NULL;
   if (!(rho > 0.)) return FL_ERR_ARG_OUTOFRANGE;
@@ -555,7 +568,7 @@
       if (!v0interp_dev[c * 3 + d]) return FL_ERR_ARG_NULL;
   }
   const int ext[3][3] = {{g.fx, g.ny, g.nz}, {g.nx, g.fy, g.nz}, {g.nx, g.ny, g.fz}};
-  const bool ends_only = v0_dev && mom3_grid(g);
+  const bool ends_only = (v0_dev || shared_v0) && mom3_grid(g);
   for (int f = 0; f < 12; ++f) {
     const int     d = f < 3 ? f : (f - 3) % 3;
     const double *src = f < 3 ? V0_dev[f] : v0interp_dev[f - 3];
@@ -569,12 +582,8 @@
     if (fl_any_ghost_exchange(h)) FL_CHK(fl_fill_ghosts(h, dst));
   }
   m->fly = false;
-  if (v0_dev) {
-    if (!m->v0p) FL_CHK(fl_dev_alloc(h, (void **)&m->v0p, sizeof(double) * 3 * h->padlen, true));
-    for (int c = 0; c < 3; ++c) launch_pad_copy(h->stream, g, v0_dev + (size_t)c * h->ncell, m->v0p + (size_t)c * h->padlen);
-    FL_CHK(mom_ghosts(m, m->v0p));
-    m->fly = true;
-  }
+  if (v0_dev) FL_CHK(mom_pad_v0(m, v0_dev));
+  if (v0_dev || shared_v0) m->fly = true;
   m->have_state = true;
   return fl_momentum_set_coefficients(m, 1., dt, -0.5 * mu * dt / rho);
 }
@@ -667,7 +676,12 @@
   return FL_SUCCESS;
 }
 
-static int momentum_cheb(fl_momentum *m, const double *b_dev, double *x_dev, const fl_ksp_opts *opts, fl_ksp_stats *stats, bool from_guess = false)
+static bool mom_solve_poisons(const fl_ksp_opts *o, const fl_ksp_stats *st)
+{
+  return o->norm_type == FL_NORM_NONE || st->reason == FL_DIVERGED_NANORINF || st->reason == FL_DIVERGED_DTOL || !std::isfinite(st->rnorm);
+}
+
+static int momentum_cheb(fl_momentum *m, const double *b_dev, double *x_dev, const fl_ksp_opts *opts, fl_ksp_stats *stats, bool from_guess = false, const double **ans_out = nullptr)
 {
   if (opts->pc != FL_PC_JACOBI && opts->pc != FL_PC_NONE) return FL_ERR_SUP;
   if (opts->norm_type == FL_NORM_NATURAL) return FL_ERR_SUP;
@@ -701,7 +715,10 @@
   }
   FL_CHK(fl_cheb_begin(h, &o, emin, emax));
   const size_t bytes = sizeof(double) * 3 * h->padlen;
-  for (double *v : {X0, X1}) FL_HIP(hipMemsetAsync(v, 0, bytes, h->stream));
+  if (m->poisoned) {
+    for (double *v : {X0, X1}) FL_HIP(hipMemsetAsync(v, 0, bytes, h->stream));
+  } else if (!from_guess) FL_HIP(hipMemsetAsync(X0, 0, bytes, h->stream));
+  m->poisoned = true;
   for (int c = 0; c < 3; ++c) launch_pad_copy(h->stream, h->g, b_dev + (size_t)c * h->ncell, B + (size_t)c * h->padlen);
   if (from_guess)
     for (int c = 0; c < 3; ++c) launch_pad_copy(h->stream, h->g, x_dev + (size_t)c * h->ncell, X0 + (size_t)c * h->padlen);
@@ -735,7 +752,9 @@
   FL_CHK(fl_poll_scal(h));
   const double *ans = h->scal_host->cur ? X1 : X0;
   for (int c = 0; c < 3; ++c) launch_unpad_copy(h->stream, h->g, ans + (size_t)c * h->padlen, x_dev + (size_t)c * h->ncell, nullptr);
+  if (ans_out) *ans_out = ans;
   FL_CHK(fl_ksp_finish(h, &o, stats));
+  m->poisoned = mom_solve_poisons(&o, stats);
   if (watched && stats->reason == FL_DIVERGED_ITS) stats->reason = FL_CONVERGED_ITS;
   return 0;
 }
@@ -745,7 +764,8 @@
 namespace {
 void lincomb(fl_poisson *h, int64_t n, double a, const double *x, double b, const double *z, double *y);
 }
-static int momentum_solve_from_guess(fl_momentum *m, const double *b_dev, double *x_dev, const fl_ksp_opts *opts, fl_ksp_stats *stats)
+static int momentum_solve_core(fl_momentum *m, const double *b_dev, double *x_dev, const fl_ksp_opts *opts, fl_ksp_stats *stats, const double **ans_out);
+static int momentum_solve_from_guess(fl_momentum *m, const double *b_dev, double *x_dev, const fl_ksp_opts *opts, fl_ksp_stats *stats, const double **ans_out)
 {
   fl_poisson *h = m->p;
   FL_HIP(hipSetDevice(h->device));
@@ -765,7 +785,7 @@
     o.initial_guess_nonzero = 0;
     o.rtol = 0.;
     o.atol = std::max(opts->rtol * bnorm, opts->atol);
-    FL_CHK(momentum_cheb(m, b_dev, x_dev, &o, stats, true));
+    FL_CHK(momentum_cheb(m, b_dev, x_dev, &o, stats, true, ans_out));
     if (stats->reason == FL_CONVERGED_ATOL && !(stats->rnorm < opts->atol)) stats->reason = FL_CONVERGED_RTOL;
     stats->rnorm0 = bnorm;
     return FL_SUCCESS;
@@ -778,7 +798,8 @@
   o.initial_guess_nonzero = 0;
   o.rtol = 0.;
   o.atol = std::max(opts->rtol * bnorm, opts->atol);
-  FL_CHK(fl_momentum_solve(m, m->gr, m->gd, &o, stats));
+  const double *dpad = nullptr;
+  FL_CHK(momentum_solve_core(m, m->gr, m->gd, &o, stats, &dpad));
   lincomb(h, n3, 1., x_dev, 1., m->gd, x_dev);
   FL_HIP(hipGetLastError());
   if (stats->reason == FL_CONVERGED_ATOL && !(stats->rnorm < opts->atol)) stats->reason = FL_CONVERGED_RTOL;
@@ -786,13 +807,14 @@
   return FL_SUCCESS;
 }
 
-extern "C" int fl_momentum_solve(fl_momentum *m, const double *b_dev, double *x_dev, const fl_ksp_opts *opts, fl_ksp_stats *stats)
-{
+static int momentum_solve_core(fl_momentum *m, const double *b_dev, double *x_dev, const fl_ksp_opts *opts, fl_ksp_stats *stats, const double **ans_out)
+{
+  *ans_out = nullptr;
   if (!m || !b_dev || !x_dev || !opts || !stats) return FL_ERR_ARG_NULL;
   if (!m->have_state && m->mp.cC != 0.) return FL_ERR_ARG_WRONGSTATE;
-  if (opts->initial_guess_nonzero) return momentum_solve_from_guess(m, b_dev, x_dev, opts, stats);
+  if (opts->initial_guess_nonzero) return momentum_solve_from_guess(m, b_dev, x_dev, opts, stats, ans_out);
   if (opts->type == FL_KSP_GMRES) return momentum_gmres(m, b_dev, x_dev, opts, stats);
-  if (opts->type == FL_KSP_CHEBYSHEV) return momentum_cheb(m, b_dev, x_dev, opts, stats);
+  if (opts->type == FL_KSP_CHEBYSHEV) return momentum_cheb(m, b_dev, x_dev, opts, stats, false, ans_out);
   if (opts->type != FL_KSP_BCGS) return FL_ERR_SUP;
   if (opts->pc != FL_PC_JACOBI && opts->pc != FL_PC_NONE) return FL_ERR_SUP;
   if (opts->norm_type != FL_NORM_PRECONDITIONED) return FL_ERR_SUP;
@@ -838,24 +860,38 @@
   }
   if (h->scal_host->it == 0) FL_HIP(hipMemsetAsync(X, 0, bytes, h->stream));
   for (int c = 0; c < 3; ++c) launch_unpad_copy(h->stream, h->g, X + (size_t)c * h->padlen, x_dev + (size_t)c * h->ncell, nullptr);
-  return fl_ksp_finish(h, &o, stats);
+  *ans_out = X;
+  FL_CHK(fl_ksp_finish(h, &o, stats));
+  if (mom_solve_poisons(&o, stats)) m->poisoned = true;
+  return 0;
+}
+
+extern "C" int fl_momentum_solve(fl_momentum *m, const double *b_dev, double *x_dev, const fl_ksp_opts *opts, fl_ksp_stats *stats)
+{
+  const double *ans = nullptr;
+  return momentum_solve_core(m, b_dev, x_dev, opts, stats, &ans);
 }
 
 namespace {
-int face_interp(fl_momentum *m, double alpha, const double *v_dev, const double *const rhs_dev[3], double *const V_dev[3])
-{
-  fl_poisson *h = m->p;
-  FL_CHK(mom_vec(m, 7));
-  for (int c = 0; c < 3; ++c) launch_pad_copy(h->stream, h->g, v_dev + (size_t)c * h->ncell, m->vec[7] + (size_t)c * h->padlen);
-  FL_CHK(mom_ghosts(m, m->vec[7]));
+int face_interp_padded(fl_momentum *m, double alpha, double *vpad, const double *const rhs_dev[3], double *const V_dev[3])
+{
+  fl_poisson *h = m->p;
+  FL_CHK(mom_ghosts(m, vpad));
   for (int d = 0; d < 3; ++d) {
     if (!V_dev[d]) return FL_ERR_ARG_NULL;
     const int64_t n = h->nface[d];
     const int     nb = (int)std::min<int64_t>((n + 255) / 256, 8192);
-    hipLaunchKernelGGL(k_face_interp, dim3(std::max(nb, 1)), dim3(256), 0, h->stream, h->g, m->ft, 0, d, alpha, m->vec[7] + (size_t)d * h->padlen, rhs_dev ? rhs_dev[d] : nullptr, V_dev[d]);
+    hipLaunchKernelGGL(k_face_interp, dim3(std::max(nb, 1)), dim3(256), 0, h->stream, h->g, m->ft, 0, d, alpha, (const double *)vpad + (size_t)d * h->padlen, rhs_dev ? rhs_dev[d] : nullptr, V_dev[d]);
   }
   FL_HIP(hipGetLastError());
   return 0;
+}
+int face_interp(fl_momentum *m, double alpha, const double *v_dev, const double *const rhs_dev[3], double *const V_dev[3])
+{
+  fl_poisson *h = m->p;
+  FL_CHK(mom_vec(m, 7));
+  for (int c = 0; c < 3; ++c) launch_pad_copy(h->stream, h->g, v_dev + (size_t)c * h->ncell, m->vec[7] + (size_t)c * h->padlen);
+  return face_interp_padded(m, alpha, m->vec[7], rhs_dev, V_dev);
 }
 void lincomb(fl_poisson *h, int64_t n, double a, const double *x, double b, const double *z, double *y)
 {
@@ -876,6 +912,24 @@
   if (!m || !v_dev || !V_dev) return FL_ERR_ARG_NULL;
   FL_HIP(hipSetDevice(m->p->device));
   return face_interp(m, alpha, v_dev, rhs_dev, V_dev);
+}
+
+namespace {
+int mom_rhs_padded(fl_momentum *m, double dt, double rho, double mu, const double *v0pad, const double *p_dev, const double *vbc_dev, double *momrhs_dev)
+{
+  fl_poisson  *h = m->p;
+  const size_t N = (size_t)h->ncell;
+  MomP         co = m->mp;
+  co.cI   = 1.;
+  co.cC   = 0.;
+  co.cL   = 0.5 * mu * dt / rho;
+  FL_CHK(mom_scale_tables(m, 1, co));
+  mom_apply_t<0, false, 1>(m, v0pad, momrhs_dev, nullptr, nullptr, &co);
+  if (p_dev) FL_CHK(fl_poisson_project(h, p_dev, momrhs_dev, momrhs_dev + N, momrhs_dev + 2 * N, nullptr, nullptr, nullptr));
+  if (vbc_dev) lincomb(h, (int64_t)(3 * N), 1., momrhs_dev, 1., vbc_dev, momrhs_dev);
+  FL_HIP(hipGetLastError());
+  return FL_SUCCESS;
+}
 }
 
 extern "C" int fl_momentum_rhs(fl_momentum *m, double dt, double rho, double mu, const double *v0_dev, const double *p_dev, const double *vbc_dev, double *momrhs_dev)
@@ -888,19 +942,71 @@
   FL_CHK(mom_vec(m, 7));
   for (int c = 0; c < 3; ++c) launch_pad_copy(h->stream, h->g, v0_dev + c * N, m->vec[7] + (size_t)c * h->padlen);
   FL_CHK(mom_ghosts(m, m->vec[7]));
-  MomP co = m->mp;
-  co.cI   = 1.;
-  co.cC   = 0.;
-  co.cL   = 0.5 * mu * dt / rho;
-  FL_CHK(mom_scale_tables(m, 1, co));
-  mom_apply_t<0, false, 1>(m, m->vec[7], momrhs_dev, nullptr, nullptr, &co);
-  if (p_dev) FL_CHK(fl_poisson_project(h, p_dev, momrhs_dev, momrhs_dev + N, momrhs_dev + 2 * N, nullptr, nullptr, nullptr));
-  if (vbc_dev) lincomb(h, (int64_t)(3 * N), 1., momrhs_dev, 1., vbc_dev, momrhs_dev);
-  FL_HIP(hipGetLastError());
-  return FL_SUCCESS;
-}
-
-extern "C" int fl_momentum_interp_faces(fl_momentum *m, const double *v_dev, const double *const vbc_dev[9], double *const out_dev[9])
+  return mom_rhs_padded(m, dt, rho, mu, m->vec[7], p_dev, vbc_dev, momrhs_dev);
+}
+
+namespace {
+int interp_faces_padded(fl_momentum *m, const double *vpad, const double *const vbc_dev[9], double *const out_dev[9], bool ends);
+}
+
+extern "C" int fl_momentum_set_v0(fl_momentum *m, const double *v0_dev)
+{
+  if (!m || !v0_dev) return FL_ERR_ARG_NULL;
+  FL_HIP(hipSetDevice(m->p->device));
+  m->have_state = false;
+  m->gersh      = -1.;
+  FL_CHK(mom_pad_v0(m, v0_dev));
+  FL_HIP(hipGetLastError());
+  return FL_SUCCESS;
+}
+
+extern "C" int fl_momentum_interp_faces_ends_v0(fl_momentum *m, const double *const vbc_dev[9], double *const out_dev[9])
+{
+  if (!m || !out_dev) return FL_ERR_ARG_NULL;
+  if (!m->have_v0) return FL_ERR_ARG_WRONGSTATE;
+  FL_HIP(hipSetDevice(m->p->device));
+  return interp_faces_padded(m, m->v0p, vbc_dev, out_dev, true);
+}
+
+extern "C" int fl_momentum_rhs_v0(fl_momentum *m, double dt, double rho, double mu, const double *p_dev, const double *vbc_dev, double *momrhs_dev)
+{
+  if (!m || !momrhs_dev) return FL_ERR_ARG_NULL;
+  if (!(rho > 0.)) return FL_ERR_ARG_OUTOFRANGE;
+  if (!m->have_v0) return FL_ERR_ARG_WRONGSTATE;
+  FL_HIP(hipSetDevice(m->p->device));
+  return mom_rhs_padded(m, dt, rho, mu, m->v0p, p_dev, vbc_dev, momrhs_dev);
+}
+
+extern "C" int fl_momentum_set_state_shared_v0(fl_momentum *m, double dt, double rho, double mu, const double *const V0_dev[3], const double *const v0interp_dev[9])
+{
+  if (!m) return FL_ERR_ARG_NULL;
+  if (!m->have_v0) return FL_ERR_ARG_WRONGSTATE;
+  return mom_set_state(m, dt, rho, mu, V0_dev, v0interp_dev, nullptr, true);
+}
+
+namespace {
+int interp_faces_padded(fl_momentum *m, const double *vpad, const double *const vbc_dev[9], double *const out_dev[9], bool ends)
+{
+  fl_poisson  *h = m->p;
+  const GridP &g = h->g;
+  ends = ends && mom3_grid(g);
+  for (int c = 0; c < 3; ++c)
+    for (int d = 0; d < 3; ++d) {
+      if (!out_dev[c * 3 + d]) return FL_ERR_ARG_NULL;
+      if (ends) {
+        const int64_t n = 2 * h->nface[d] / std::max(d == 0 ? g.fx : (d == 1 ? g.fy : g.fz), 1);
+        const int     nb = (int)std::max<int64_t>(1, std::min<int64_t>((n + 255) / 256, 8192));
+        hipLaunchKernelGGL(k_face_interp_ends, dim3(nb), dim3(256), 0, h->stream, g, m->ft, c == d ? 1 : 2, d, vpad + (size_t)c * h->padlen, vbc_dev ? vbc_dev[c * 3 + d] : nullptr, out_dev[c * 3 + d]);
+      } else {
+        const int64_t n = h->nface[d];
+        const int     nb = (int)std::min<int64_t>((n + 255) / 256, 8192);
+        hipLaunchKernelGGL(k_face_interp, dim3(std::max(nb, 1)), dim3(256), 0, h->stream, g, m->ft, c == d ? 1 : 2, d, 1., vpad + (size_t)c * h->padlen, vbc_dev ? vbc_dev[c * 3 + d] : nullptr, out_dev[c * 3 + d]);
+      }
+    }
+  FL_HIP(hipGetLastError());
+  return FL_SUCCESS;
+}
+int interp_faces_caller(fl_momentum *m, const double *v_dev, const double *const vbc_dev[9], double *const out_dev[9], bool ends)
 {
   if (!m || !v_dev || !out_dev) return FL_ERR_ARG_NULL;
   fl_poisson *h = m->p;
@@ -908,37 +1014,18 @@
   FL_CHK(mom_vec(m, 7));
   for (int c = 0; c < 3; ++c) launch_pad_copy(h->stream, h->g, v_dev + (size_t)c * h->ncell, m->vec[7] + (size_t)c * h->padlen);
   FL_CHK(mom_ghosts(m, m->vec[7]));
-  for (int c = 0; c < 3; ++c)
-    for (int d = 0; d < 3; ++d) {
-      if (!out_dev[c * 3 + d]) return FL_ERR_ARG_NULL;
-      const int64_t n = h->nface[d];
-      const int     nb = (int)std::min<int64_t>((n + 255) / 256, 8192);
-      hipLaunchKernelGGL(k_face_interp, dim3(std::max(nb, 1)), dim3(256), 0, h->stream, h->g, m->ft, c == d ? 1 : 2, d, 1., m->vec[7] + (size_t)c * h->padlen, vbc_dev ? vbc_dev[c * 3 + d] : nullptr,
-                         out_dev[c * 3 + d]);
-    }
-  FL_HIP(hipGetLastError());
-  return FL_SUCCESS;
+  return interp_faces_padded(m, m->vec[7], vbc_dev, out_dev, ends);
+}
+}
+
+extern "C" int fl_momentum_interp_faces(fl_momentum *m, const double *v_dev, const double *const vbc_dev[9], double *const out_dev[9])
+{
+  return interp_faces_caller(m, v_dev, vbc_dev, out_dev, false);
 }
 
 extern "C" int fl_momentum_interp_faces_ends(fl_momentum *m, const double *v_dev, const double *const vbc_dev[9], double *const out_dev[9])
 {
-  if (!m || !v_dev || !out_dev) return FL_ERR_ARG_NULL;
-  fl_poisson *h = m->p;
-  const GridP &g = h->g;
-  if (!mom3_grid(g)) return fl_momentum_interp_faces(m, v_dev, vbc_dev, out_dev);
-  FL_HIP(hipSetDevice(h->device));
-  FL_CHK(mom_vec(m, 7));
-  for (int c = 0; c < 3; ++c) launch_pad_copy(h->stream, h->g, v_dev + (size_t)c * h->ncell, m->vec[7] + (size_t)c * h->padlen);
-  FL_CHK(mom_ghosts(m, m->vec[7]));
-  for (int c = 0; c < 3; ++c)
-    for (int d = 0; d < 3; ++d) {
-      if (!out_dev[c * 3 + d]) return FL_ERR_ARG_NULL;
-      const int64_t n = 2 * h->nface[d] / std::max(d == 0 ? g.fx : (d == 1 ? g.fy : g.fz), 1);
-      const int     nb = (int)std::max<int64_t>(1, std::min<int64_t>((n + 255) / 256, 8192));
-      hipLaunchKernelGGL(k_face_interp_ends, dim3(nb), dim3(256), 0, h->stream, g, m->ft, c == d ? 1 : 2, d, m->vec[7] + (size_t)c * h->padlen, vbc_dev ? vbc_dev[c * 3 + d] : nullptr, out_dev[c * 3 + d]);
-    }
-  FL_HIP(hipGetLastError());
-  return FL_SUCCESS;
+  return interp_faces_caller(m, v_dev, vbc_dev, out_dev, true);
 }
 
 extern "C" int fl_abf_jacobian_mult(fl_momentum *m, const double *v_dev, const double *const V_dev[3], const double *p_dev, double *fv_dev, double *const fV_dev[3], double *fp_dev)
@@ -1185,8 +1272,10 @@
   fl_poisson *h = m->p;
   FL_HIP(hipSetDevice(h->device));
   if (!m->srhs) FL_CHK(fl_dev_alloc(h, (void **)&m->srhs, sizeof(double) * (size_t)h->ncell, true));
-  FL_CHK(fl_momentum_solve(m, momrhs_dev, v_dev, momentum_opts, &stats[0]));
-  FL_CHK(fl_momentum_face_interp(m, v_dev, interprhs_dev, V_dev));
+  const double *vpad = nullptr;
+  FL_CHK(momentum_solve_core(m, momrhs_dev, v_dev, momentum_opts, &stats[0], &vpad));
+  if (vpad) FL_CHK(face_interp_padded(m, 1., const_cast<double *>(vpad), interprhs_dev, V_dev));
+  else FL_CHK(fl_momentum_face_interp(m, v_dev, interprhs_dev, V_dev));
   FL_CHK(fl_poisson_rhs(h, V_dev[0], V_dev[1], V_dev[2], contrhs_dev, m->srhs));
   const size_t N = (size_t)h->ncell;
   if (m->schur_ainv == FL_ABF_AINV_ID) FL_CHK(fl_poisson_solve(h, m->srhs, p_dev, schur_opts, &stats[1]));
diff --git a/fluca_amd/host/fluca_host.c b/fluca_amd/host/fluca_host.c
--- a/fluca_amd/host/fluca_host.c
+++ b/fluca_amd/host/fluca_host.c
@@ -1,4 +1,5 @@
 #include "../../include/fluca_host_impl.h"
+#include "../../include/fluca_hip_momentum_v0.h"
 
 #include <math.h>
 #include <pthread.h>
@@ -2472,7 +2473,8 @@
   fl_poisson   *h = ns->poisson;
   const int64_t N = c->sz[0];
   const double  dt = ns->dt, t = ns->t, cv = 0.5 * ns->mu * dt / ns->rho;
-  FLABI(fl_momentum_rhs(ns->momentum, dt, ns->rho, ns->mu, c->sol0_v, ns->step == 0 ? c->sol0_p : c->phalf, NULL, f->v));
+  if (c->v0_shared) FLABI(fl_momentum_rhs_v0(ns->momentum, dt, ns->rho, ns->mu, ns->step == 0 ? c->sol0_p : c->phalf, NULL, f->v));
+  else FLABI(fl_momentum_rhs(ns->momentum, dt, ns->rho, ns->mu, c->sol0_v, ns->step == 0 ? c->sol0_p : c->phalf, NULL, f->v));
   for (int d = 0; d < 3; ++d) FLABI(fl_vec_lincomb(h, c->sz[1 + d], 0., f->V[d], 0., NULL, f->V[d]));
   FLABI(fl_vec_lincomb(h, N, 0., f->p, 0., NULL, f->p));
   for (int b = 0; b < 6; ++b) {
@@ -2577,7 +2579,8 @@
     const double *V0[3] = {c->sol0_V[0], c->sol0_V[1], c->sol0_V[2]};
     const double *W[9];
     for (int q = 0; q < 9; ++q) W[q] = c->W[q];
-    FLABI(fl_momentum_set_state_v0(J, ns->dt, ns->rho, ns->mu, V0, W, c->sol0_v));
+    if (c->v0_shared && J == ns->momentum) FLABI(fl_momentum_set_state_shared_v0(J, ns->dt, ns->rho, ns->mu, V0, W));
+    else FLABI(fl_momentum_set_state_v0(J, ns->dt, ns->rho, ns->mu, V0, W, c->sol0_v));
   }
   return 0;
 }
@@ -2607,6 +2610,8 @@
   FLABI(fl_momentum_create(ns->poisson, &ns->momentum));
   return NSFormJacobian(ns, NULL, ns->momentum, NS_INIT_JACOBIAN);
 }
+
+static FlErrorCode cnl_step_solve(NS ns, int guess, double *xv, double **xV, int timing, double *tm);
 
 static FlErrorCode NSStep_CNLinear(NS ns)
 {
@@ -2621,14 +2626,29 @@
   double    tm[6] = {0., 0., 0., 0., 0., 0.};
   if (timing) tm[0] = step_clock(ns);
   const int guess = ns->ksp_type != 2 ? ns->mom_guess_previous : 0;
-  if (guess == 2 && c->have_sol0) FLABI(fl_vec_lincomb(h, 3 * N, 2., c->sol_v, -1., c->sol0_v, c->x_v));
-  else if (guess) FLABI(fl_vec_lincomb(h, 3 * N, 1., c->sol_v, 0., NULL, c->x_v));
+  const int extrapolate = guess == 2 && c->have_sol0;
+  const int inplace = ns->ksp_type == 1;
+  double   *xv = inplace && !extrapolate ? c->sol_v : c->x_v, **xV = inplace ? c->sol_V : c->x_V;
+  if (extrapolate) FLABI(fl_vec_lincomb(h, 3 * N, 2., c->sol_v, -1., c->sol0_v, c->x_v));
+  else if (guess && xv != c->sol_v) FLABI(fl_vec_lincomb(h, 3 * N, 1., c->sol_v, 0., NULL, c->x_v));
   FLABI(fl_vec_lincomb(h, 3 * N, 1., c->sol_v, 0., NULL, c->sol0_v));
-  FLABI(fl_vec_lincomb(h, N, 1., c->sol_p, 0., NULL, c->sol0_p));
+  if (ns->step == 0) FLABI(fl_vec_lincomb(h, N, 1., c->sol_p, 0., NULL, c->sol0_p));
   for (int d = 0; d < 3; ++d) FLABI(fl_vec_lincomb(h, c->sz[1 + d], 1., c->sol_V[d], 0., NULL, c->sol0_V[d]));
   c->have_sol0 = 1;
-
-  FLABI(fl_momentum_interp_faces_ends(ns->momentum, c->sol0_v, NULL, c->W));
+  c->v0_shared = 0;
+  FLABI(fl_momentum_set_v0(ns->momentum, c->sol0_v));
+  c->v0_shared = 1;
+  const FlErrorCode rc = cnl_step_solve(ns, guess, xv, xV, timing, tm);
+  c->v0_shared = 0;
+  return rc;
+}
+
+static FlErrorCode cnl_step_solve(NS ns, int guess, double *xv, double **xV, int timing, double *tm)
+{
+  NS_CNLinear  *c = (NS_CNLinear *)ns->data;
+  fl_poisson   *h = ns->poisson;
+  const int64_t N = c->sz[0];
+  FLABI(fl_momentum_interp_faces_ends_v0(ns->momentum, NULL, c->W));
   for (int b = 0; b < 6; ++b) {
     if (ns->bcs[b].type != NS_BC_VELOCITY || !cnl_touches(ns, b)) continue;
     const int        ax = b / 2, a1 = ax == 0 ? 1 : 0, a2 = ax == 2 ? 1 : 2;
@@ -2641,7 +2661,7 @@
       FLABI(fl_boundary_set_faces(h, b, 1., c->plane_dev, c->W[q * 3 + ax]));
     }
   }
-  NSVec x = {c->x_v, {c->x_V[0], c->x_V[1], c->x_V[2]}, c->x_p}, f = {c->f_v, {c->f_V[0], c->f_V[1], c->f_V[2]}, c->f_p};
+  NSVec x = {xv, {xV[0], xV[1], xV[2]}, c->x_p}, f = {c->f_v, {c->f_V[0], c->f_V[1], c->f_V[2]}, c->f_p};
   if (timing) tm[1] = step_clock(ns);
   FLCHK(NSFormFunction(ns, &x, &f));
   if (timing) tm[2] = step_clock(ns);
@@ -2656,7 +2676,7 @@
   } else {
     fl_ksp_opts mom1 = ns->mom;
     if (guess) mom1.initial_guess_nonzero = 1;
-    FLABI(fl_abf_apply(ns->momentum, &mom1, &ns->schur, c->f_v, fV, c->f_p, c->x_v, c->x_V, c->x_p, st));
+    FLABI(fl_abf_apply(ns->momentum, &mom1, &ns->schur, c->f_v, fV, c->f_p, xv, xV, c->x_p, st));
   }
   if (ns->ksp_type != 2) {
     ns->ksp_its   = 1;
@@ -2695,9 +2715,16 @@
     }
   }
   if (timing) tm[4] = step_clock(ns);
-  if (ns->reason < 0) return 0;
-  FLABI(fl_vec_lincomb(h, 3 * N, 1., c->x_v, 0., NULL, c->sol_v));
-  for (int d = 0; d < 3; ++d) FLABI(fl_vec_lincomb(h, c->sz[1 + d], 1., c->x_V[d], 0., NULL, c->sol_V[d]));
+  if (ns->reason < 0) {
+    if (xv == c->sol_v) FLABI(fl_vec_lincomb(h, 3 * N, 1., c->sol0_v, 0., NULL, c->sol_v));
+    if (xV == c->sol_V)
+      for (int d = 0; d < 3; ++d) FLABI(fl_vec_lincomb(h, c->sz[1 + d], 1., c->sol0_V[d], 0., NULL, c->sol_V[d]));
+    FLABI(fl_poisson_synchronize(h));
+    return 0;
+  }
+  if (xv != c->sol_v) FLABI(fl_vec_lincomb(h, 3 * N, 1., xv, 0., NULL, c->sol_v));
+  if (xV != c->sol_V)
+    for (int d = 0; d < 3; ++d) FLABI(fl_vec_lincomb(h, c->sz[1 + d], 1., xV[d], 0., NULL, c->sol_V[d]));
   FLABI(fl_pressure_update(h, ns->step == 0, c->x_p, c->sol0_p, c->phalf, c->sol_p));
   FLABI(fl_poisson_synchronize(h));
   if (timing) {
@@ -2731,9 +2758,10 @@
   if (!ns->setupcalled || !ns->data) return E_ARG_WRONGSTATE;
   NS_CNLinear *c = (NS_CNLinear *)ns->data;
   if (x) {
-    x->v = c->x_v;
+    const int inplace = ns->ksp_type == 1;
+    x->v = inplace ? c->sol_v : c->x_v;
     x->p = c->x_p;
-    for (int d = 0; d < 3; ++d) x->V[d] = c->x_V[d];
+    for (int d = 0; d < 3; ++d) x->V[d] = inplace ? c->sol_V[d] : c->x_V[d];
   }
   if (r) {
     r->v = c->f_v;
diff --git a/include/fluca_hip_momentum_v0.h b/include/fluca_hip_momentum_v0.h
--- /dev/null
+++ b/include/fluca_hip_momentum_v0.h
@@ -0,0 +1,19 @@
+#ifndef FLUCA_HIP_MOMENTUM_V0_H
+#define FLUCA_HIP_MOMENTUM_V0_H
+
+#include "fluca_hip.h"
+
+#ifdef __cplusplus
+extern "C" {
+#endif
+
+int fl_momentum_set_v0(fl_momentum *m, const double *v0_dev);
+int fl_momentum_interp_faces_ends_v0(fl_momentum *m, const double *const vbc_dev[9], double *const out_dev[9]);
+int fl_momentum_rhs_v0(fl_momentum *m, double dt, double rho, double mu, const double *p_dev, const double *vbc_dev, double *momrhs_dev);
+int fl_momentum_set_state_shared_v0(fl_momentum *m, double dt, double rho, double mu, const double *const V0_dev[3], const double *const v0interp_dev[9]);
+
+#ifdef __cplusplus
+}
+#endif
+
+#endif
diff --git a/include/fluca_host_impl.h b/include/fluca_host_impl.h
--- a/include/fluca_host_impl.h
+++ b/include/fluca_host_impl.h
@@ -152,6 +152,7 @@
   NSBoundaryConditionFunction bc_fn[6][2];
   NSVec gm_w, gm_t, *gm_V;
   int   gm_nalloc, gm_cap;
+  int   v0_shared;
 } NS_CNLinear;
 FlErrorCode NSCreate_CNLinear(NS ns);
 
```

Result: no change. 718.7 (-0.0%).
